# iris1997jiatong/I-DCCRN-VAE

Measured on AMD Instinct MI355X. Metric: 4s@16kHz utterances/sec fwd+SI-SNR, DCCRN-CL, 1/2/4/8 MI355X vs host CPU, higher is better.
Workload: dtype f32; 1 GPU; supervised DCCRN-CL forward(train=False) + final_ete_loss (weights 0/0/1); batch_per_gpu=64, utterance=4 s @ 16 kHz (64000 samples, 641 frames), parallelism=replicas x1, streams=1, input=resident in HBM

## Files before the change

i-dccrn-vae_amd/csrc/cgemm_tw.hip:

```cpp
#include <cstdint>
#include <cstdlib>
#include "cgemm.hpp"
#include "../../include/idccrn_hip.h"

namespace {

struct TwArgs {
    const float* x0;
    const float* x1;
    int C0, C1;
    int Fin, Fout;
    int J, Jp, Tp;
    const float* wfrag;
    int UP;
    const float* epi;
    int has_fold;
    const float* slope;
    float* out;
    int Cout, cotiles;
    int tshift, t_valid;
    double* stats;
    int stats_rep;
    const float* add;
    int add_div, add_Jp;
    int jtiles, ftiles;
    int xcd_split;
};

constexpr int TW_PACK_CI = 8;

template <int PH> __device__ __forceinline__ int tw_ra(int r) {
    if (PH == 0) return r == 0 ? 0 : (r == 2 ? 2 : 1);
    return r == 0 ? 1 : 2;
}
template <int PH> __device__ __forceinline__ int tw_rb(int r) {
    if (PH == 0) return r == 2 ? 1 : (r == 3 ? 3 : 2);
    return r == 0 ? 2 : 3;
}
template <int PH> __device__ __forceinline__ float tw_cb(int r) {
    if (PH == 0) return r == 1 ? 1.f : -1.f;
    return r == 1 ? 0.f : -1.f;
}
template <int PH> constexpr int tw_nr() { return PH == 0 ? 4 : 3; }
template <int PH> constexpr int tw_nt() { return tw_nr<PH>() * 9; }
template <int PH> constexpr int tw_ntp() { return PH == 0 ? 36 : 32; }
template <int PH> constexpr int tw_ntw() { return (tw_nt<PH>() + 3) / 4; }
__host__ __device__ inline int tw_tile(int ph, int w, int k) {
    if (ph == 0) return w * 9 + k;
    if (w < 3) return k < 6 ? w * 9 + k : w * 9 + 8;
    return k < 6 ? (k >> 1) * 9 + 6 + (k & 1) : -1;
}
template <int PH> constexpr int tw_wslots() { return PH == 0 ? 9 : 8; }

template <int PH, int CIK, bool LEFT, int DBG = 0, int RDW = 2, bool WVEC = true, bool STATS = false>
__global__ __launch_bounds__(256, 2) void cconv_tw_kernel(const TwArgs a) {
    constexpr int NR = tw_nr<PH>(), NT = tw_nt<PH>(), NTP = tw_ntp<PH>(), NTW = tw_ntw<PH>();
    constexpr int NRAW = PH == 0 ? 4 : 3, ROW0 = PH == 0 ? 0 : 1;
    constexpr int KS = CIK / 2;
    constexpr int RT = NRAW * 9 * 32;
    constexpr int NE = CIK * RT;
    constexpr int NBUF = 2;
    constexpr int NITEM = CIK * NRAW * 16;
    constexpr int NLD = (NITEM + 255) / 256;
    static_assert(KS % RDW == 0 && NLD <= 2, "weight ring slots are compile-time; at most two staging items per thread");
    static_assert(NT * 4 * 64 <= NBUF * NE, "the epilogue exchange fits the patch buffers");

    extern __shared__ __attribute__((aligned(16))) float smem[];

    const int tid = threadIdx.x;
    const int lane = tid & 63;
    const int wave = __builtin_amdgcn_readfirstlane(tid >> 6);
    const int half = lane >> 5, l31 = lane & 31;

    const int bid = blockIdx.x;
    const int xcd = bid & 7, slot = bid >> 3;
    int jt, ft, ct;
    if (a.xcd_split) {
        const int G = 8 / a.cotiles;
        ct = xcd % a.cotiles;
        jt = (slot / a.ftiles) * G + xcd / a.cotiles;
        ft = slot - (slot / a.ftiles) * a.ftiles;
    } else {
        const int per = a.cotiles * a.ftiles;
        jt = (slot / per) * 8 + xcd;
        const int rem = slot - (slot / per) * per;
        ft = rem / a.cotiles;
        ct = rem - ft * a.cotiles;
    }
    if (jt >= a.jtiles) return;
    const int j0 = jt * 64;
    const int m0 = 2 * ft;
    const int rbase = m0 - 1 + ROW0;

    const int Cin = a.C0 + a.C1;
    const int nchunk = (Cin + CIK - 1) / CIK;

    f32x16 acc[NTW];
#pragma unroll
    for (int k = 0; k < NTW; ++k)
#pragma unroll
        for (int r = 0; r < 16; ++r) acc[k][r] = 0.f;
    constexpr int NPAIR = (NTW - 1) / 2;
    constexpr bool UNI = PH == 0;
    int offA[UNI ? 1 : NPAIR + 1], offB[UNI ? 1 : NPAIR + 1];
    float cbj[UNI ? 1 : NPAIR + 1];
    if (UNI) {
        cbj[0] = tw_cb<PH>(wave);
        offA[0] = (tw_ra<PH>(wave) - ROW0) * 288;
        offB[0] = (tw_rb<PH>(wave) - ROW0) * 288;
    } else {
#pragma unroll
        for (int j = 0; j <= NPAIR; ++j) {
            int t = tw_tile(PH, wave, j < NPAIR ? 2 * j : NTW - 1);
            t = t < 0 ? 0 : t;
            const int r = t / 9, plane = t - r * 9;
            cbj[j] = tw_cb<PH>(r);
            const int po = plane == 8 ? 256 : (plane >> 1) * 64;
            offA[j] = (tw_ra<PH>(r) - ROW0) * 288 + po;
            offB[j] = cbj[j] != 0.f ? (tw_rb<PH>(r) - ROW0) * 288 + po : offA[j];
        }
    }

    f32x4 v_r[NLD], v_i[NLD];
    float e_r[NLD], e_i[NLD];
    unsigned off_v[NLD], off_e[NLD], ldsoff[NLD];
    unsigned okmask[NLD];
    int item_cl[NLD];
    bool interior[NLD];
#pragma unroll
    for (int i = 0; i < NLD; ++i) {
        const int e = tid + i * 256;
        const int c8 = e & 15;
        const int rl = (e >> 4) % NRAW, cl = e / (16 * NRAW);
        item_cl[i] = cl;
        const int f = rbase + rl;
        const int jc = j0 + 4 * c8;
        const int je = LEFT ? jc - 1 : jc + 4;
        const bool exists = e < NITEM;
        const bool okr = exists && f >= 0 && f < a.Fin;
        unsigned m = 0;
#pragma unroll
        for (int q = 0; q < 5; ++q) {
            const int c = jc + q + (LEFT ? -1 : 0);
            if (c >= 0 && c < a.J) m |= 1u << q;
        }
        if (okr) m |= 1u << 5;
        if (exists) m |= 1u << 7;
        const int jcv = jc + 3 < a.Jp ? jc : 0;
        const int jev = (je >= 0 && je < a.Jp) ? je : 0;
        off_v[i] = okr ? (unsigned)((cl * a.Fin + f) * a.Jp + jcv) : 0u;
        off_e[i] = okr ? (unsigned)((cl * a.Fin + f) * a.Jp + jev) : 0u;
        if (jc + 3 >= a.Jp) m &= ~0x1fu;
        if (!(je >= 0 && je < a.Jp)) m &= LEFT ? ~1u : ~(1u << 4);
        okmask[i] = m;
        interior[i] = __builtin_amdgcn_ballot_w64((m & 0xbfu) == 0xbfu) == ~0ull;
        ldsoff[i] = (unsigned)((cl * NRAW + rl) * 288 + 4 * c8);
    }
    auto stage_load = [&](int chunk, int i) {
        const int ci0 = chunk * CIK;
        const bool from0 = ci0 < a.C0;
        const float* br = from0 ? a.x0 + (size_t)ci0 * a.Fin * a.Jp : a.x1 + (size_t)(ci0 - a.C0) * a.Fin * a.Jp;
        const float* bi = from0 ? br + (size_t)a.C0 * a.Fin * a.Jp : br + (size_t)a.C1 * a.Fin * a.Jp;
        const int cvalid = (from0 ? a.C0 : Cin) - ci0;
        const bool dead = item_cl[i] >= cvalid;
        const unsigned ov = dead ? 0u : off_v[i], oe = dead ? 0u : off_e[i];
        v_r[i] = *(const f32x4*)(br + ov);
        v_i[i] = *(const f32x4*)(bi + ov);
        e_r[i] = br[oe];
        e_i[i] = bi[oe];
    };
    float fr[5], fi[5];
    auto stage_window = [&](int chunk, int i) {
        const int ci0s = chunk * CIK;
        const int cvalid = (ci0s < a.C0 ? a.C0 : Cin) - ci0s;
        constexpr bool left = LEFT;
        if (interior[i] && cvalid >= CIK) {
#pragma unroll
            for (int q = 0; q < 5; ++q) {
                fr[q] = left ? (q == 0 ? e_r[i] : v_r[i][q == 0 ? 0 : q - 1]) : (q == 4 ? e_r[i] : v_r[i][q == 4 ? 3 : q]);
                fi[q] = left ? (q == 0 ? e_i[i] : v_i[i][q == 0 ? 0 : q - 1]) : (q == 4 ? e_i[i] : v_i[i][q == 4 ? 3 : q]);
            }
            return;
        }
        unsigned m = okmask[i];
        if (item_cl[i] >= cvalid || !((m >> 5) & 1u)) m &= ~0x1fu;
#pragma unroll
        for (int q = 0; q < 5; ++q) {
            const float xr = left ? (q == 0 ? e_r[i] : v_r[i][q == 0 ? 0 : q - 1]) : (q == 4 ? e_r[i] : v_r[i][q == 4 ? 3 : q]);
            const float xi = left ? (q == 0 ? e_i[i] : v_i[i][q == 0 ? 0 : q - 1]) : (q == 4 ? e_i[i] : v_i[i][q == 4 ? 3 : q]);
            const bool cok = (m >> q) & 1u;
            fr[q] = cok ? xr : 0.f;
            fi[q] = cok ? xi : 0.f;
        }
    };
    auto plane_val = [&](int gt, int pr) -> float {
        const int g = gt / 3, tau = gt - g * 3;
        const int q0 = 2 * pr;
        const float xa_ = g == 0 ? fr[q0] + fi[q0] : (g == 1 ? fr[q0] : fi[q0]);
        const float xb_ = g == 0 ? fr[q0 + 1] + fi[q0 + 1] : (g == 1 ? fr[q0 + 1] : fi[q0 + 1]);
        const float xd_ = g == 0 ? fr[q0 + 2] + fi[q0 + 2] : (g == 1 ? fr[q0 + 2] : fi[q0 + 2]);
        return tau == 0 ? xa_ - xb_ : (tau == 1 ? xb_ : xb_ - xd_);
    };
    auto item_exists = [&](int i) -> bool { return NITEM >= (i + 1) * 256 || wave * 64 + i * 256 < NITEM; };
    auto stage_plane2 = [&](float* dst, int i, int j) {
        if (!item_exists(i)) return;
        if (j < 4) {
            f32x4 o = {plane_val(2 * j, 0), plane_val(2 * j + 1, 0), plane_val(2 * j, 1), plane_val(2 * j + 1, 1)};
            *(f32x4*)(dst + ldsoff[i] + j * 64) = o;
        } else {
            *(float2*)(dst + ldsoff[i] - 2 * (int)(tid & 15) + 256) = make_float2(plane_val(8, 0), plane_val(8, 1));
        }
    };
    auto stage_store = [&](float* dst, int chunk, int i) {
        stage_window(chunk, i);
#pragma unroll
        for (int j = 0; j < 5; ++j) stage_plane2(dst, i, j);
    };

    constexpr int WS = tw_wslots<PH>();
    const float* wbase = a.wfrag + ((size_t)(PH == 1 ? (size_t)a.cotiles * a.UP * tw_ntp<0>() : 0) + (size_t)ct * a.UP * NTP) * 64 +
                         (size_t)wave * WS * 64;
    const int total_ks = nchunk * KS;
    float a_w[RDW][NTW];
    auto load_w = [&](int g, float (&dst)[NTW]) {
        g = g < total_ks ? g : total_ks - 1;
        const float* ws = wbase + (size_t)g * NTP * 64;
        if (WVEC) {
            const f32x4 w0 = *(const f32x4*)(ws + lane * 4), w1 = *(const f32x4*)(ws + 256 + lane * 4);
#pragma unroll
            for (int k = 0; k < 4; ++k) {
                dst[k] = w0[k];
                if (4 + k < NTW) dst[4 + k] = w1[k];
            }
            if (NTW == 9) dst[NTW - 1] = ws[512 + lane];
        } else {
#pragma unroll
            for (int k = 0; k < NTW; ++k) dst[k] = ws[k * 64 + lane];
        }
    };
    float xa[NTW], xb[NTW];
    auto load_raw2 = [&](const float* base, int j) {
        if (j < NPAIR) {
            const int oa = UNI ? offA[0] + j * 64 : offA[UNI ? 0 : j], ob = UNI ? offB[0] + j * 64 : offB[UNI ? 0 : j];
            const float2 pa_ = *(const float2*)(base + oa + 2 * l31), pb_ = *(const float2*)(base + ob + 2 * l31);
            xa[2 * j] = pa_.x; xa[2 * j + 1] = pa_.y;
            xb[2 * j] = pb_.x; xb[2 * j + 1] = pb_.y;
        } else {
            xa[NTW - 1] = base[(UNI ? offA[0] + 256 : offA[UNI ? 0 : NPAIR]) + l31];
            xb[NTW - 1] = base[(UNI ? offB[0] + 256 : offB[UNI ? 0 : NPAIR]) + l31];
        }
    };
    auto load_raw_all = [&](const float* base) {
#pragma unroll
        for (int j = 0; j <= NPAIR; ++j) load_raw2(base, j);
    };

#pragma unroll
    for (int i = 0; i < NLD; ++i) stage_load(0, i);
#pragma unroll
    for (int u = 0; u < RDW; ++u) load_w(u, a_w[u]);
#pragma unroll
    for (int i = 0; i < NLD; ++i) stage_store(smem, 0, i);
#pragma unroll
    for (int i = 0; i < NLD; ++i) stage_load(nchunk > 1 ? 1 : 0, i);
    __syncthreads();

    load_raw_all(smem + (size_t)half * RT);
    for (int chunk = 0; chunk < nchunk; ++chunk) {
        const float* P = smem + (chunk & 1) * NE;
        float* Pn = smem + ((chunk + 1) & 1) * NE;
        const int nxt = chunk + 1 < nchunk ? chunk + 1 : chunk, nxt2 = chunk + 2 < nchunk ? chunk + 2 : nchunk - 1;
#pragma unroll
        for (int ul = 0; ul < KS; ++ul) {
            const float* bnext = ul + 1 < KS ? P + (size_t)(2 * (ul + 1) + half) * RT : Pn + (size_t)half * RT;
            const int si = ul - 1;
            const bool staging = !(DBG & 1) && si >= 0 && si < NLD;
#pragma unroll
            for (int k = 0; k < NTW; ++k) {
                const float b = xa[k] + cbj[UNI ? 0 : (k >> 1 < NPAIR ? k >> 1 : NPAIR)] * xb[k];
                acc[k] = __builtin_amdgcn_mfma_f32_32x32x2f32(a_w[ul % RDW][k], b, acc[k], 0, 0, 0);
                if (ul == KS - 1 && k == 0) {
                    __builtin_amdgcn_sched_barrier(0);
                    __syncthreads();
                }
                if ((k & 1) && (k >> 1) < NPAIR) load_raw2(bnext, k >> 1);
                if (k == NTW - 1) load_raw2(bnext, NPAIR);
                if (staging) {
                    if (k == 0) stage_window(nxt, si);
                    if ((k & 1) && k < 6) stage_plane2(Pn, si, k >> 1);
                    if (k == (NTW == 9 ? 7 : 6)) stage_plane2(Pn, si, 3);
                    if (k == NTW - 1) stage_plane2(Pn, si, 4);
                    if (k == NTW - 1) stage_load(nxt2, si);
                }
                __builtin_amdgcn_sched_barrier(0);
            }
            if (!(DBG & 2)) load_w(chunk * KS + ul + RDW, a_w[ul % RDW]);
        }
    }
    __syncthreads();

    const float slope = a.slope ? *a.slope : 1.0f;
    const bool has_act = a.slope != nullptr;
    float* E = smem;
    const int jA = j0 + 2 * l31;
    bool keep[2], inb[2];
    int ja[2];
#pragma unroll
    for (int q = 0; q < 2; ++q) {
        const int j = jA + q;
        const int bj = j / a.Tp, tp = j - bj * a.Tp;
        inb[q] = j < a.J;
        keep[q] = inb[q] && tp >= 1 && tp <= a.t_valid;
        ja[q] = j - (bj - bj / a.add_div) * a.Tp;
    }
#pragma unroll
    for (int s = 0; s < ((DBG & 4) ? 1 : 4); ++s) {
        if (s > 0) __syncthreads();
#pragma unroll
        for (int k = 0; k < NTW; ++k) {
            const int t = tw_tile(PH, wave, k);
            if (t >= 0) {
#pragma unroll
                for (int rr = 0; rr < 4; ++rr) E[(t * 4 + rr) * 64 + lane] = acc[k][4 * s + rr];
            }
        }
        __syncthreads();
        float v[NT];
#pragma unroll
        for (int t = 0; t < NT; ++t) v[t] = E[(t * 4 + wave) * 64 + lane];
        float pr[NR][2], pi[NR][2];
#pragma unroll
        for (int r = 0; r < NR; ++r) {
            float y[3][2];
#pragma unroll
            for (int g = 0; g < 3; ++g) {
                const float m1 = v[r * 9 + g * 3], m2 = v[r * 9 + g * 3 + 1], m3 = v[r * 9 + g * 3 + 2];
                y[g][0] = m1 + m2;
                y[g][1] = m2 - m3;
            }
#pragma unroll
            for (int q = 0; q < 2; ++q) {
                pr[r][q] = y[0][q] - y[2][q];
                pi[r][q] = y[0][q] + y[1][q];
            }
        }
        const int rg = 4 * s + wave;
        const int co = ct * 32 + (rg & 3) + 8 * (rg >> 2) + 4 * half;
        const bool cok = co < a.Cout;
        const f32x4 e0 = *(const f32x4*)(a.epi + (size_t)co * 8);
        const float e4 = a.epi[(size_t)co * 8 + 4], e5 = a.epi[(size_t)co * 8 + 5];
        float st[5] = {0.f, 0.f, 0.f, 0.f, 0.f};
#pragma unroll
        for (int rt = 0; rt < 2; ++rt) {
            const int fo = 2 * m0 + PH + 2 * rt;
            if (fo >= a.Fout) continue;
            float yr[2], yi[2];
#pragma unroll
            for (int q = 0; q < 2; ++q) {
                float re, im;
                if (PH == 0) {
                    re = rt == 0 ? pr[0][q] + pr[1][q] + pr[2][q] : pr[1][q] - pr[2][q] - pr[NR - 1][q];
                    im = rt == 0 ? pi[0][q] + pi[1][q] + pi[2][q] : pi[1][q] - pi[2][q] - pi[NR - 1][q];
                } else {
                    re = rt == 0 ? pr[0][q] + pr[1][q] : pr[1][q] - pr[2][q];
                    im = rt == 0 ? pi[0][q] + pi[1][q] : pi[1][q] - pi[2][q];
                }
                if (a.add && cok && inb[q]) {
                    re += a.add[((size_t)co * a.Fout + fo) * a.add_Jp + ja[q]];
                    im += a.add[((size_t)(a.Cout + co) * a.Fout + fo) * a.add_Jp + ja[q]];
                }
                float r_, i_;
                if (a.has_fold) {
                    r_ = e0[0] * re + e0[1] * im + e4;
                    i_ = e0[2] * re + e0[3] * im + e5;
                } else {
                    r_ = re + e4;
                    i_ = im + e5;
                }
                if (has_act) {
                    r_ = r_ >= 0.f ? r_ : slope * r_;
                    i_ = i_ >= 0.f ? i_ : slope * i_;
                }
                yr[q] = keep[q] ? r_ : 0.f;
                yi[q] = keep[q] ? i_ : 0.f;
                if (STATS && keep[q]) {
                    st[0] += yr[q];
                    st[1] += yi[q];
                    st[2] += yr[q] * yr[q];
                    st[3] += yi[q] * yi[q];
                    st[4] += yr[q] * yi[q];
                }
            }
            if (cok) {
                float* o_r = a.out + ((size_t)co * a.Fout + fo) * a.Jp + jA;
                float* o_i = a.out + ((size_t)(a.Cout + co) * a.Fout + fo) * a.Jp + jA;
                if (inb[1]) {
                    *(float2*)o_r = make_float2(yr[0], yr[1]);
                    *(float2*)o_i = make_float2(yi[0], yi[1]);
                } else if (inb[0]) {
                    o_r[0] = yr[0];
                    o_i[0] = yi[0];
                }
            }
        }
        if (STATS) {
#pragma unroll
            for (int q = 0; q < 5; ++q) {
                float tsum = st[q];
#pragma unroll
                for (int o = 16; o > 0; o >>= 1) tsum += __shfl_xor(tsum, o, 64);
                if (l31 == 0 && cok)
                    atomicAdd(&a.stats[((size_t)(a.stats_rep > 1 ? (blockIdx.x & (a.stats_rep - 1)) : 0) * a.Cout + co) * 5 + q], (double)tsum);
            }
        }
    }
}

__global__ void pack_cconv_tw_kernel(const float* __restrict__ wino, int cotiles, int UN, int UP, int vec, float* __restrict__ out) {
    const long long n0 = (long long)cotiles * UP * tw_ntp<0>() * 64, n1 = (long long)cotiles * UP * tw_ntp<1>() * 64;
    for (long long idx = blockIdx.x * (long long)blockDim.x + threadIdx.x; idx < n0 + n1; idx += (long long)gridDim.x * blockDim.x) {
        const int ph = idx >= n0;
        const long long i = ph ? idx - n0 : idx;
        const int ntp = ph ? tw_ntp<1>() : tw_ntp<0>(), nt = ph ? tw_nt<1>() : tw_nt<0>();
        const int lane = (int)(i & 63);
        long long t_ = i >> 6;
        const int t = (int)(t_ % ntp); t_ /= ntp;
        const int u = (int)(t_ % UP);
        const int ct = (int)(t_ / UP);
        float val = 0.f;
        const int ws_ = ph ? tw_wslots<1>() : tw_wslots<0>();
        const int pos = t * 64 + lane, w = pos / (ws_ * 64), q = pos % (ws_ * 64);
        const bool vec_ = (vec >> ph) & 1;
        const int k = !vec_ ? q >> 6 : (q < 512 ? (q >> 8) * 4 + (q & 3) : 8);
        const int ln = !vec_ ? q & 63 : (q < 512 ? (q & 255) >> 2 : q - 512);
        const int tt = k < (ph ? 7 : 9) ? tw_tile(ph, w, k) : -1;
        const int ci = 2 * u + (ln >> 5), co = ln & 31;
        if (tt >= 0 && ci * 3 < UN) {
            const int r = tt / 9, g = (tt % 9) / 3, tau = tt % 3;
            const float* src = wino + ((((size_t)ph * cotiles + ct) * UN + (size_t)ci * 3 + g) * 4 + r) * 64;
            const float w0 = src[co], w1 = src[32 + co];
            val = tau == 0 ? w0 : (tau == 1 ? w0 + w1 : w1);
        }
        out[idx] = val;
    }
}

template <int PH, int CIK, bool LEFT, int DBG, int RDW, bool WVEC = true, bool STATS = false>
int launch_tw_ph_l(const TwArgs& a, hipStream_t st);
inline int tw_wvec_mask() {
    static const int v = [] { const char* e = getenv("IDV_TW_WVEC"); return e ? atoi(e) : 1; }();
    return v;
}
template <int PH, int CIK, int DBG = 0, int RDW = 2>
int launch_tw_ph(const TwArgs& a, hipStream_t st) {
    const bool wv = (tw_wvec_mask() >> PH) & 1;
    if (DBG == 0 && RDW == 2 && a.stats) {
        constexpr bool WV = PH == 0;
        if (wv != WV) return IDV_EINVAL;
        return a.tshift ? launch_tw_ph_l<PH, CIK, true, 0, 2, WV, true>(a, st) : launch_tw_ph_l<PH, CIK, false, 0, 2, WV, true>(a, st);
    }
    if (DBG == 0 && RDW == 2 && !wv)
        return a.tshift ? launch_tw_ph_l<PH, CIK, true, 0, 2, false>(a, st) : launch_tw_ph_l<PH, CIK, false, 0, 2, false>(a, st);
    return a.tshift ? launch_tw_ph_l<PH, CIK, true, DBG, RDW>(a, st) : launch_tw_ph_l<PH, CIK, false, DBG, RDW>(a, st);
}
template <int PH, int CIK, bool LEFT, int DBG, int RDW, bool WVEC, bool STATS>
int launch_tw_ph_l(const TwArgs& a, hipStream_t st) {
    constexpr int NE = CIK * (PH == 0 ? 4 : 3) * 9 * 32;
    constexpr size_t smem = 2 * NE * sizeof(float);
    static_assert(smem * 2 <= 160 * 1024, "the patch buffers of two workgroups must fit the 160 KB of LDS");
    TwArgs b = a;
    b.jtiles = (a.J + 63) / 64;
    b.ftiles = PH == 1 ? a.Fin / 2 : (a.Fin + 1) / 2;
    if (b.ftiles == 0) return IDV_OK;
    static const int xsplit = [] { const char* e = getenv("IDV_TW_XCD_SPLIT"); return e ? atoi(e) : 1; }();
    b.xcd_split = (xsplit && (b.cotiles == 2 || b.cotiles == 4 || b.cotiles == 8)) ? 1 : 0;
    long long nblk = (long long)((b.jtiles + 7) / 8) * 8 * b.ftiles * b.cotiles;
    if (b.xcd_split) {
        const int G = 8 / b.cotiles;
        nblk = (long long)((b.jtiles + G - 1) / G) * b.ftiles * 8;
    }
    if (nblk > 0x7fffffffLL) return IDV_EINVAL;
    auto k = cconv_tw_kernel<PH, CIK, LEFT, DBG, RDW, WVEC, STATS>;
    static bool attr_set[64] = {};
    int dev = 0;
    if (hipGetDevice(&dev) != hipSuccess || dev < 0 || dev >= 64) return IDV_ELAUNCH;
    if (smem > 64 * 1024 && !attr_set[dev]) {
        if (hipFuncSetAttribute((const void*)k, hipFuncAttributeMaxDynamicSharedMemorySize, (int)smem) != hipSuccess) return IDV_ELAUNCH;
        attr_set[dev] = true;
    }
    hipLaunchKernelGGL(k, dim3((unsigned)nblk), dim3(256), smem, st, b);
    return idv_launch_status();
}

}

extern "C" int idv_cconv_tw_supported(int C0, int C1, int Cout, int Fin) {
    static const int min_cout = [] { const char* e = getenv("IDV_TW_MIN_COUT"); return e ? atoi(e) : 32; }();
    if (Cout < min_cout || Fin < 2) return 0;
    if (!idv_cconv_gauss_supported(C0, C1, Cout)) return 0;
    return (C1 == 0 || C0 % 8 == 0) ? 1 : 0;
}

extern "C" long long idv_cconv_tw_wfrag_floats(int Cout, int cin_used) {
    const long long cotiles = (Cout + 31) / 32, cpad = (cin_used + TW_PACK_CI - 1) / TW_PACK_CI * TW_PACK_CI;
    return cotiles * (cpad / 2) * (36 + 32) * 64;
}

extern "C" int idv_pack_cconv_tw(const float* wino_frag, int Cout, int cin_used, float* tw_frag, void* stream) {
    if (!wino_frag || !tw_frag || Cout <= 0 || cin_used <= 0) return IDV_EINVAL;
    const int cotiles = (Cout + 31) / 32;
    const int cpad = (cin_used + TW_PACK_CI - 1) / TW_PACK_CI * TW_PACK_CI;
    const long long n = idv_cconv_tw_wfrag_floats(Cout, cin_used);
    const unsigned blocks = (unsigned)((n + 255) / 256 > 4096 ? 4096 : (n + 255) / 256);
    hipLaunchKernelGGL(pack_cconv_tw_kernel, dim3(blocks), dim3(256), 0, (hipStream_t)stream, wino_frag, cotiles, cpad * 3, cpad / 2,
                       tw_wvec_mask(), tw_frag);
    return idv_launch_status();
}

extern "C" int idv_ctconv2d_tw_fwd(const float* x0, int C0, const float* x1, int C1, const float* wfrag, const float* epi, int has_fold,
                                   const float* prelu_slope, float* out, double* stats, double* stats_work, int stats_rep, int tshift,
                                   int Cout, int Fin, int B, int Tp, int Jp, int t_valid_out, const float* addend, int addend_div,
                                   int addend_Jp, void* stream) {
    if (!x0 || !wfrag || !epi || !out || C0 <= 0 || Cout <= 0 || Fin <= 0 || B <= 0 || Tp <= 1) return IDV_EINVAL;
    if (stats && stats_work && (stats_rep < 2 || (stats_rep & (stats_rep - 1)))) return IDV_EINVAL;
    if (addend && (addend_div < 1 || B % addend_div || addend_Jp < (B / addend_div) * Tp)) return IDV_EINVAL;
    if (C1 > 0 && !x1) return IDV_EINVAL;
    if (tshift != 0 && tshift != -1) return IDV_EINVAL;
    if (!idv_cconv_tw_supported(C0, C1, Cout, Fin)) return IDV_EINVAL;
    if ((Jp & 3) || (reinterpret_cast<uintptr_t>(x0) & 15) || (C1 > 0 && (reinterpret_cast<uintptr_t>(x1) & 15)) ||
        (reinterpret_cast<uintptr_t>(out) & 7))
        return IDV_EINVAL;
    TwArgs a{};
    a.x0 = x0; a.x1 = x1; a.C0 = C0; a.C1 = C1;
    a.Fin = Fin; a.Fout = 2 * Fin - 1;
    a.J = B * Tp; a.Jp = Jp; a.Tp = Tp;
    a.wfrag = wfrag; a.UP = (C0 + C1 + TW_PACK_CI - 1) / TW_PACK_CI * TW_PACK_CI / 2;
    a.epi = epi; a.has_fold = has_fold; a.slope = prelu_slope; a.out = out;
    a.Cout = Cout; a.cotiles = (Cout + 31) / 32;
    a.tshift = tshift; a.t_valid = t_valid_out;
    a.add = addend; a.add_div = addend ? addend_div : 1; a.add_Jp = addend_Jp;
    if (Jp < a.J) return IDV_EINVAL;
    if ((long long)8 * Fin * (long long)Jp >= 0xffffffffLL) return IDV_EINVAL;
    hipStream_t st = (hipStream_t)stream;
    a.stats = stats;
    if (stats && stats_work) { a.stats = stats_work; a.stats_rep = stats_rep; }
    int rc = 0;
#ifdef IDV_TW_EXPERIMENTS
    static const int dbg = [] { const char* e = getenv("IDV_TW_DBG"); return e ? atoi(e) : 0; }();
    static const int only = [] { const char* e = getenv("IDV_TW_ONLY"); return e ? atoi(e) : 0; }();
    if (dbg && !stats) {
        if (only != 2) rc = dbg == 1 ? launch_tw_ph<0, 8, 1>(a, st) : (dbg == 2 ? launch_tw_ph<0, 8, 2>(a, st) : launch_tw_ph<0, 8, 3>(a, st));
        if (rc) return rc;
        if (only != 1) rc = dbg == 1 ? launch_tw_ph<1, 8, 1>(a, st) : (dbg == 2 ? launch_tw_ph<1, 8, 2>(a, st) : launch_tw_ph<1, 8, 3>(a, st));
        return rc;
    }
    if (only) return only == 1 ? launch_tw_ph<0, 8>(a, st) : launch_tw_ph<1, 8>(a, st);
#endif
    rc = launch_tw_ph<0, 8>(a, st);
    if (!rc) rc = launch_tw_ph<1, 8>(a, st);
    if (rc || !(stats && stats_work)) return rc;
    return idv_launch_stats_collapse(stats_work, stats_rep, Cout * 5, stats, st);
}
```

i-dccrn-vae_amd/csrc/cgemm_tw2.hip:

```cpp
#include <cstdint>
#include <cstdlib>
#include <type_traits>
#include "cgemm.hpp"
#include "../../include/idccrn_hip.h"

namespace {

struct Tw2Args {
    const float* x0;
    int Cin;
    int Fin, Fout;
    int J, Jp, Tp;
    const float* wfrag;
    int UP;
    const float* epi;
    int has_fold;
    const float* slope;
    float* out;
    int Cout, cotiles;
    int tshift, t_valid;
    double* stats;
    int stats_rep;
    int jtiles, ftiles;
    int xcd_split;
};

constexpr int TW2_PACK_CI = 8;

__host__ __device__ constexpr int tw2_ra(int q) { return q == 0 ? 0 : (q == 1 ? 2 : (q == 2 ? 4 : (q == 3 ? 2 : (q == 4 ? 1 : 3)))); }
__host__ __device__ constexpr int tw2_rb(int q) { return q == 0 ? 4 : (q == 1 ? 4 : (q == 2 ? 2 : (q == 3 ? 6 : (q == 4 ? 3 : (q == 5 ? 3 : 5))))); }
__host__ __device__ constexpr float tw2_cb(int q) { return q == 1 ? 1.f : (q == 5 ? 0.f : -1.f); }
__host__ __device__ constexpr int tw2_qx(int a) { return a == 0 ? 0 : (a == 1 ? 1 : 3); }
__host__ __device__ constexpr int tw2_qy(int a) { return a == 0 ? 4 : (a == 1 ? 5 : 6); }
__host__ __device__ constexpr int tw2_main_acc(int w) { return w == 2 ? 3 : w; }
__host__ __device__ inline void tw2_slot(int w, int k, int& q, int& plane) {
    if (w < 3) {
        if (k < 14) { q = (k & 1) ? tw2_qy(tw2_main_acc(w)) : tw2_qx(tw2_main_acc(w)); plane = k >> 1; }
        else { q = 2; plane = 2 * w + (k - 14); }
    } else {
        if (k < 12) { const int a = tw2_main_acc(k >> 2); q = (k & 1) ? tw2_qy(a) : tw2_qx(a); plane = 7 + ((k >> 1) & 1); }
        else if (k < 15) { q = 2; plane = 6 + (k - 12); }
        else { q = -1; plane = 0; }
    }
}
__host__ __device__ inline int tw2_acc_tile(int w, int i) {
    if (w < 3) return i < 7 ? tw2_main_acc(w) * 9 + i : 2 * 9 + 2 * w + (i - 7);
    return i < 6 ? tw2_main_acc(i >> 1) * 9 + 7 + (i & 1) : 2 * 9 + 6 + (i - 6);
}

__device__ __forceinline__ int tw2_poff(int p, int l31) { return p < 8 ? (p >> 1) * 64 + 2 * l31 + (p & 1) : 256 + l31; }

template <bool LEFT, bool STATS, int DBG = 0>
__global__ __launch_bounds__(256, 2) void cconv_tw2_kernel(const Tw2Args a) {
    constexpr int NT = 36, NACC = 9, NSLOT = 16;
    constexpr int NRAW = 7, CIK = 4, KS = 2;
    constexpr int RT = NRAW * 288;
    constexpr int NE = CIK * RT;
    constexpr int NITEM = CIK * NRAW * 16;
    constexpr int NLD = 2;
    static_assert(NT * 4 * 64 <= 2 * NE, "the epilogue exchange fits the patch buffers");

    extern __shared__ __attribute__((aligned(16))) float smem[];

    const int tid = threadIdx.x;
    const int lane = tid & 63;
    const int wave = __builtin_amdgcn_readfirstlane(tid >> 6);
    const int half = lane >> 5, l31 = lane & 31;

    const int bid = blockIdx.x;
    const int xcd = bid & 7, slot = bid >> 3;
    int jt, ft, ct;
    if (a.xcd_split) {
        const int G = 8 / a.cotiles;
        ct = xcd % a.cotiles;
        jt = (slot / a.ftiles) * G + xcd / a.cotiles;
        ft = slot - (slot / a.ftiles) * a.ftiles;
    } else {
        const int per = a.cotiles * a.ftiles;
        jt = (slot / per) * 8 + xcd;
        const int rem = slot - (slot / per) * per;
        ft = rem / a.cotiles;
        ct = rem - ft * a.cotiles;
    }
    if (jt >= a.jtiles) return;
    const int j0 = jt * 64;
    const int m0 = 2 * ft;
    const int rbase = 2 * m0 - 2;

    const int Cin = a.Cin;
    const int nchunk = (Cin + CIK - 1) / CIK;

    f32x16 acc[NACC];
#pragma unroll
    for (int k = 0; k < NACC; ++k)
#pragma unroll
        for (int r = 0; r < 16; ++r) acc[k][r] = 0.f;

    f32x4 v_r[NLD], v_i[NLD];
    float e_r[NLD], e_i[NLD];
    unsigned off_v[NLD], ldsoff[NLD];
    unsigned okmask[NLD];
    bool interior[NLD];
    auto item_cl = [&](int i) -> int { return (tid + i * 256) / (16 * NRAW); };
#pragma unroll
    for (int i = 0; i < NLD; ++i) {
        const int e = tid + i * 256;
        const int c8 = e & 15;
        const int rl = (e >> 4) % NRAW, cl = e / (16 * NRAW);
        const int f = rbase + rl;
        const int jc = j0 + 4 * c8;
        const int je = LEFT ? jc - 1 : jc + 4;
        const bool exists = e < NITEM;
        const bool okr = exists && f >= 0 && f < a.Fin;
        unsigned m = 0;
#pragma unroll
        for (int q = 0; q < 5; ++q) {
            const int c = jc + q + (LEFT ? -1 : 0);
            if (c >= 0 && c < a.J) m |= 1u << q;
        }
        if (okr) m |= 1u << 5;
        const int jcv = jc + 3 < a.Jp ? jc : 0;
        off_v[i] = okr ? (unsigned)((cl * a.Fin + f) * a.Jp + jcv) : 4u;
        if (jc + 3 >= a.Jp) m &= ~0x1fu;
        if (!(je >= 0 && je < a.Jp)) m &= LEFT ? ~1u : ~(1u << 4);
        okmask[i] = m;
        interior[i] = __builtin_amdgcn_ballot_w64((m & 0x3fu) == 0x3fu) == ~0ull;
        ldsoff[i] = (unsigned)((cl * NRAW + rl) * 288 + 4 * c8);
    }
    auto item_exists = [&](int i) -> bool { return i == 0 || wave * 64 + 256 < NITEM; };
    auto stage_load = [&](int chunk, int i) {
        if (!item_exists(i)) return;
        const int ci0 = chunk * CIK;
        const float* br = a.x0 + (size_t)ci0 * a.Fin * a.Jp;
        const float* bi = br + (size_t)Cin * a.Fin * a.Jp;
        const bool dead = item_cl(i) >= Cin - ci0;
        const unsigned ov = dead ? 4u : off_v[i];
        v_r[i] = *(const f32x4*)(br + ov);
        v_i[i] = *(const f32x4*)(bi + ov);
        e_r[i] = (br + ov)[LEFT ? -1 : 4];
        e_i[i] = (bi + ov)[LEFT ? -1 : 4];
    };
    float fr[5], fi[5];
    auto stage_window = [&](int chunk, int i) {
        if (!item_exists(i)) return;
        const int cvalid = Cin - chunk * CIK;
        constexpr bool left = LEFT;
        if (interior[i] && cvalid >= CIK) {
#pragma unroll
            for (int q = 0; q < 5; ++q) {
                fr[q] = left ? (q == 0 ? e_r[i] : v_r[i][q == 0 ? 0 : q - 1]) : (q == 4 ? e_r[i] : v_r[i][q == 4 ? 3 : q]);
                fi[q] = left ? (q == 0 ? e_i[i] : v_i[i][q == 0 ? 0 : q - 1]) : (q == 4 ? e_i[i] : v_i[i][q == 4 ? 3 : q]);
            }
            return;
        }
        unsigned m = okmask[i];
        if (item_cl(i) >= cvalid || !((m >> 5) & 1u)) m &= ~0x1fu;
#pragma unroll
        for (int q = 0; q < 5; ++q) {
            const float xr = left ? (q == 0 ? e_r[i] : v_r[i][q == 0 ? 0 : q - 1]) : (q == 4 ? e_r[i] : v_r[i][q == 4 ? 3 : q]);
            const float xi = left ? (q == 0 ? e_i[i] : v_i[i][q == 0 ? 0 : q - 1]) : (q == 4 ? e_i[i] : v_i[i][q == 4 ? 3 : q]);
            const bool cok = (m >> q) & 1u;
            fr[q] = cok ? xr : 0.f;
            fi[q] = cok ? xi : 0.f;
        }
    };
    auto plane_val = [&](int gt, int pr) -> float {
        const int g = gt / 3, tau = gt - g * 3;
        const int q0 = 2 * pr;
        const float xa_ = g == 0 ? fr[q0] + fi[q0] : (g == 1 ? fr[q0] : fi[q0]);
        const float xb_ = g == 0 ? fr[q0 + 1] + fi[q0 + 1] : (g == 1 ? fr[q0 + 1] : fi[q0 + 1]);
        const float xd_ = g == 0 ? fr[q0 + 2] + fi[q0 + 2] : (g == 1 ? fr[q0 + 2] : fi[q0 + 2]);
        return tau == 0 ? xa_ - xb_ : (tau == 1 ? xb_ : xb_ - xd_);
    };
    auto stage_plane2 = [&](float* dst, int i, int j) {
        if (!item_exists(i)) return;
        if (j < 4) {
            f32x4 o = {plane_val(2 * j, 0), plane_val(2 * j + 1, 0), plane_val(2 * j, 1), plane_val(2 * j + 1, 1)};
            *(f32x4*)(dst + ldsoff[i] + j * 64) = o;
        } else {
            *(float2*)(dst + ldsoff[i] - 2 * (int)(tid & 15) + 256) = make_float2(plane_val(8, 0), plane_val(8, 1));
        }
    };
    auto stage_store = [&](float* dst, int chunk, int i) {
        stage_window(chunk, i);
#pragma unroll
        for (int j = 0; j < 5; ++j) stage_plane2(dst, i, j);
    };

    const float* wbase = a.wfrag + (((size_t)ct * a.UP) * 4 + wave) * 1024 + lane * 4;
    const int total_ks = nchunk * KS;
    float a_w[NSLOT];
    auto load_wg = [&](int g, int grp) {
        g = g < total_ks ? g : total_ks - 1;
        const f32x4 w4 = *(const f32x4*)(wbase + (size_t)g * 4096 + grp * 256);
#pragma unroll
        for (int k = 0; k < 4; ++k) a_w[grp * 4 + k] = w4[k];
    };

    const int am = tw2_main_acc(wave < 3 ? wave : 0);
    const int qxm = tw2_qx(am), qym = tw2_qy(am);
    const int rxa = tw2_ra(qxm) * 288, rxb = tw2_rb(qxm) * 288, rya = tw2_ra(qym) * 288, ryb = tw2_rb(qym) * 288;
    const float cbx = tw2_cb(qxm), cby = tw2_cb(qym);
    const int r2a = tw2_ra(2) * 288 + wave * 64, r2b = tw2_rb(2) * 288 + wave * 64;
    float xa[2][4], xb[2][4];
    auto load_grp_a = [&](const float* base, int g, float (&oa)[4], float (&ob)[4]) {
        if (g < 3) {
            const float2 xa_ = *(const float2*)(base + rxa + g * 64 + 2 * l31), xb_ = *(const float2*)(base + rxb + g * 64 + 2 * l31);
            const float2 ya_ = *(const float2*)(base + rya + g * 64 + 2 * l31), yb_ = *(const float2*)(base + ryb + g * 64 + 2 * l31);
            oa[0] = xa_.x; oa[2] = xa_.y; ob[0] = xb_.x; ob[2] = xb_.y;
            oa[1] = ya_.x; oa[3] = ya_.y; ob[1] = yb_.x; ob[3] = yb_.y;
        } else {
            oa[0] = base[rxa + 3 * 64 + 2 * l31]; ob[0] = base[rxb + 3 * 64 + 2 * l31];
            oa[1] = base[rya + 3 * 64 + 2 * l31]; ob[1] = base[ryb + 3 * 64 + 2 * l31];
            const float2 pa_ = *(const float2*)(base + r2a + 2 * l31), pb_ = *(const float2*)(base + r2b + 2 * l31);
            oa[2] = pa_.x; oa[3] = pa_.y; ob[2] = pb_.x; ob[3] = pb_.y;
        }
    };
    auto load_grp_b = [&](const float* base, int g, float (&oa)[4], float (&ob)[4]) {
#pragma unroll
        for (int s4 = 0; s4 < 4; ++s4) {
            int q, plane;
            tw2_slot(3, 4 * g + s4, q, plane);
            if (q < 0) continue;
            oa[s4] = base[tw2_ra(q) * 288 + tw2_poff(plane, l31)];
            ob[s4] = base[tw2_rb(q) * 288 + tw2_poff(plane, l31)];
        }
    };

#pragma unroll
    for (int i = 0; i < NLD; ++i) stage_load(0, i);
#pragma unroll
    for (int grp = 0; grp < 4; ++grp) load_wg(0, grp);
#pragma unroll
    for (int i = 0; i < NLD; ++i) stage_store(smem, 0, i);
#pragma unroll
    for (int i = 0; i < NLD; ++i) stage_load(nchunk > 1 ? 1 : 0, i);
    __syncthreads();
    if (wave < 3)
        load_grp_a(smem + (size_t)half * RT, 0, xa[0], xb[0]);
    else
        load_grp_b(smem + (size_t)half * RT, 0, xa[0], xb[0]);

    auto run = [&](auto role) {
        constexpr bool ROLE_B = decltype(role)::value;
        for (int chunk = 0; chunk < nchunk; ++chunk) {
            const float* P = smem + (chunk & 1) * NE;
            float* Pn = smem + ((chunk + 1) & 1) * NE;
            const int nxt = chunk + 1 < nchunk ? chunk + 1 : chunk, nxt2 = chunk + 2 < nchunk ? chunk + 2 : nchunk - 1;
#pragma unroll
            for (int ul = 0; ul < KS; ++ul) {
                const float* bnext = ul + 1 < KS ? P + (size_t)(2 * (ul + 1) + half) * RT : Pn + (size_t)half * RT;
                const bool staging = !(DBG & 1) && ul == 0;
#pragma unroll
                for (int k = 0; k < (ROLE_B ? NSLOT - 1 : NSLOT); ++k) {
                    const int g = k >> 2, s4 = k & 3;
                    float cb;
                    int ai;
                    if (ROLE_B) {
                        int q, plane;
                        tw2_slot(3, k, q, plane);
                        cb = tw2_cb(q);
                        ai = k < 12 ? k >> 1 : 6 + (k - 12);
                    } else {
                        cb = k < 14 ? ((k & 1) ? cby : cbx) : -1.f;
                        ai = k < 14 ? k >> 1 : 7 + (k - 14);
                    }
                    if (s4 == 0) {
                        const float* src = g < 3 ? P + (size_t)(2 * ul + half) * RT : bnext;
                        if (!(ul == KS - 1 && g == 3)) {
                            if (ROLE_B) load_grp_b(src, (g + 1) & 3, xa[(g + 1) & 1], xb[(g + 1) & 1]);
                            else load_grp_a(src, (g + 1) & 3, xa[(g + 1) & 1], xb[(g + 1) & 1]);
                        }
                    }
                    const float b = xa[g & 1][s4] + cb * xb[g & 1][s4];
                    acc[ai] = __builtin_amdgcn_mfma_f32_32x32x2f32(a_w[k], b, acc[ai], 0, 0, 0);
                    if (ul == KS - 1 && k == 0) {
                        __builtin_amdgcn_sched_barrier(0);
                        __syncthreads();
                    }
                    if (ul == KS - 1 && k == 12) {
                        if (ROLE_B) load_grp_b(bnext, 0, xa[0], xb[0]);
                        else load_grp_a(bnext, 0, xa[0], xb[0]);
                    }
                    if (((k & 3) == 3 || (ROLE_B && k == NSLOT - 2)) && !(DBG & 2)) load_wg(chunk * KS + ul + 1, k >> 2);
                    if (staging) {
                        if (k == 0) stage_window(nxt, 0);
                        if (k >= 1 && k <= 5) stage_plane2(Pn, 0, k - 1);
                        if (k == 5) stage_load(nxt2, 0);
                        if (!ROLE_B) {
                            if (k == 8) stage_window(nxt, 1);
                            if (k >= 9 && k <= 13) stage_plane2(Pn, 1, k - 9);
                            if (k == 13) stage_load(nxt2, 1);
                        }
                    }
                    __builtin_amdgcn_sched_barrier(0);
                }
            }
        }
    };
    if (wave < 3)
        run(std::false_type{});
    else
        run(std::true_type{});
    __syncthreads();

    const float slope = a.slope ? *a.slope : 1.0f;
    const bool has_act = a.slope != nullptr;
    float* E = smem;
    const int jA = j0 + 2 * l31;
    bool keep[2], inb[2];
#pragma unroll
    for (int q = 0; q < 2; ++q) {
        const int j = jA + q;
        const int tp = j % a.Tp;
        inb[q] = j < a.J;
        keep[q] = inb[q] && tp >= 1 && tp <= a.t_valid;
    }
#pragma unroll
    for (int s = 0; s < 4; ++s) {
        if (s > 0) __syncthreads();
#pragma unroll
        for (int k = 0; k < NACC; ++k) {
            const int t = tw2_acc_tile(wave, k);
#pragma unroll
            for (int rr = 0; rr < 4; ++rr) E[(t * 4 + rr) * 64 + lane] = acc[k][4 * s + rr];
        }
        __syncthreads();
        float v[NT];
#pragma unroll
        for (int t = 0; t < NT; ++t) v[t] = E[(t * 4 + wave) * 64 + lane];
        float pr[4][2], pi[4][2];
#pragma unroll
        for (int r = 0; r < 4; ++r) {
            float y[3][2];
#pragma unroll
            for (int g = 0; g < 3; ++g) {
                const float m1 = v[r * 9 + g * 3], m2 = v[r * 9 + g * 3 + 1], m3 = v[r * 9 + g * 3 + 2];
                y[g][0] = m1 + m2;
                y[g][1] = m2 - m3;
            }
#pragma unroll
            for (int q = 0; q < 2; ++q) {
                pr[r][q] = y[0][q] - y[2][q];
                pi[r][q] = y[0][q] + y[1][q];
            }
        }
        const int rg = 4 * s + wave;
        const int co = ct * 32 + (rg & 3) + 8 * (rg >> 2) + 4 * half;
        const bool cok = co < a.Cout;
        const f32x4 e0 = *(const f32x4*)(a.epi + (size_t)co * 8);
        const float e4 = a.epi[(size_t)co * 8 + 4], e5 = a.epi[(size_t)co * 8 + 5];
        float st[5] = {0.f, 0.f, 0.f, 0.f, 0.f};
#pragma unroll
        for (int rt = 0; rt < 2; ++rt) {
            const int fo = m0 + rt;
            if (fo >= a.Fout) continue;
            float yr[2], yi[2];
#pragma unroll
            for (int q = 0; q < 2; ++q) {
                const float re = rt == 0 ? pr[0][q] + pr[1][q] + pr[2][q] : pr[1][q] - pr[2][q] - pr[3][q];
                const float im = rt == 0 ? pi[0][q] + pi[1][q] + pi[2][q] : pi[1][q] - pi[2][q] - pi[3][q];
                float r_, i_;
                if (a.has_fold) {
                    r_ = e0[0] * re + e0[1] * im + e4;
                    i_ = e0[2] * re + e0[3] * im + e5;
                } else {
                    r_ = re + e4;
                    i_ = im + e5;
                }
                if (has_act) {
                    r_ = r_ >= 0.f ? r_ : slope * r_;
                    i_ = i_ >= 0.f ? i_ : slope * i_;
                }
                yr[q] = keep[q] ? r_ : 0.f;
                yi[q] = keep[q] ? i_ : 0.f;
                if (STATS && keep[q]) {
                    st[0] += yr[q];
                    st[1] += yi[q];
                    st[2] += yr[q] * yr[q];
                    st[3] += yi[q] * yi[q];
                    st[4] += yr[q] * yi[q];
                }
            }
            if (cok) {
                float* o_r = a.out + ((size_t)co * a.Fout + fo) * a.Jp + jA;
                float* o_i = a.out + ((size_t)(a.Cout + co) * a.Fout + fo) * a.Jp + jA;
                if (inb[1]) {
                    *(float2*)o_r = make_float2(yr[0], yr[1]);
                    *(float2*)o_i = make_float2(yi[0], yi[1]);
                } else if (inb[0]) {
                    o_r[0] = yr[0];
                    o_i[0] = yi[0];
                }
            }
        }
        if (STATS) {
#pragma unroll
            for (int q = 0; q < 5; ++q) {
                float tsum = st[q];
#pragma unroll
                for (int o = 16; o > 0; o >>= 1) tsum += __shfl_xor(tsum, o, 64);
                if (l31 == 0 && cok)
                    atomicAdd(&a.stats[((size_t)(a.stats_rep > 1 ? (blockIdx.x & (a.stats_rep - 1)) : 0) * a.Cout + co) * 5 + q], (double)tsum);
            }
        }
    }
}

__global__ void pack_cconv_tw2_kernel(const float* __restrict__ wino, int cotiles, int UN, int UP, float* __restrict__ out) {
    const long long n = (long long)cotiles * UP * 4096;
    for (long long idx = blockIdx.x * (long long)blockDim.x + threadIdx.x; idx < n; idx += (long long)gridDim.x * blockDim.x) {
        const int kk = (int)(idx & 3), ln = (int)((idx >> 2) & 63), grp = (int)((idx >> 8) & 3), w = (int)((idx >> 10) & 3);
        const long long t_ = idx >> 12;
        const int u = (int)(t_ % UP), ct = (int)(t_ / UP);
        int q, plane;
        tw2_slot(w, grp * 4 + kk, q, plane);
        float val = 0.f;
        const int ci = 2 * u + (ln >> 5), co = ln & 31;
        if (q >= 0 && ci * 3 < UN) {
            const int g = plane / 3, tau = plane % 3;
            const float* src = wino + ((((size_t)ct * UN + (size_t)ci * 3 + g) * 8 + q)) * 64;
            const float w0 = src[co], w1 = src[32 + co];
            val = tau == 0 ? w0 : (tau == 1 ? w0 + w1 : w1);
        }
        out[idx] = val;
    }
}

template <bool LEFT, bool STATS, int DBG>
int launch_tw2(const Tw2Args& a, hipStream_t st) {
    constexpr size_t smem = 2 * 4 * 7 * 288 * sizeof(float);
    static_assert(smem * 2 <= 160 * 1024, "the patch buffers of two workgroups must fit the 160 KB of LDS");
    Tw2Args b = a;
    b.jtiles = (a.J + 63) / 64;
    b.ftiles = (a.Fout + 1) / 2;
    static const int xsplit = [] { const char* e = getenv("IDV_TW_XCD_SPLIT"); return e ? atoi(e) : 1; }();
    b.xcd_split = (xsplit && (b.cotiles == 2 || b.cotiles == 4 || b.cotiles == 8)) ? 1 : 0;
    long long nblk = (long long)((b.jtiles + 7) / 8) * 8 * b.ftiles * b.cotiles;
    if (b.xcd_split) {
        const int G = 8 / b.cotiles;
        nblk = (long long)((b.jtiles + G - 1) / G) * b.ftiles * 8;
    }
    if (nblk > 0x7fffffffLL) return IDV_EINVAL;
    auto k = cconv_tw2_kernel<LEFT, STATS, DBG>;
    static bool attr_set[64] = {};
    int dev = 0;
    if (hipGetDevice(&dev) != hipSuccess || dev < 0 || dev >= 64) return IDV_ELAUNCH;
    if (smem > 64 * 1024 && !attr_set[dev]) {
        if (hipFuncSetAttribute((const void*)k, hipFuncAttributeMaxDynamicSharedMemorySize, (int)smem) != hipSuccess) return IDV_ELAUNCH;
        attr_set[dev] = true;
    }
    hipLaunchKernelGGL(k, dim3((unsigned)nblk), dim3(256), smem, st, b);
    return idv_launch_status();
}

}

extern "C" int idv_cconv_tw2_supported(int Cin, int Cout, int Fin) {
    static const int min_cout = [] { const char* e = getenv("IDV_TW2_MIN_COUT"); return e ? atoi(e) : 32; }();
    static const int min_cin = [] { const char* e = getenv("IDV_TW2_MIN_CIN"); return e ? atoi(e) : 64; }();
    if (Cout < min_cout || Cin < min_cin || (Fin - 1) / 2 + 1 < 2) return 0;
    return idv_cconv_gauss_supported(Cin, 0, Cout);
}

extern "C" long long idv_cconv_tw2_wfrag_floats(int Cout, int cin_used) {
    const long long cotiles = (Cout + 31) / 32, cpad = (cin_used + TW2_PACK_CI - 1) / TW2_PACK_CI * TW2_PACK_CI;
    return cotiles * (cpad / 2) * 4096;
}

extern "C" int idv_pack_cconv_tw2(const float* wino_frag, int Cout, int cin_used, float* tw_frag, void* stream) {
    if (!wino_frag || !tw_frag || Cout <= 0 || cin_used <= 0) return IDV_EINVAL;
    const int cotiles = (Cout + 31) / 32;
    const int cpad = (cin_used + TW2_PACK_CI - 1) / TW2_PACK_CI * TW2_PACK_CI;
    const long long n = idv_cconv_tw2_wfrag_floats(Cout, cin_used);
    const unsigned blocks = (unsigned)((n + 255) / 256 > 4096 ? 4096 : (n + 255) / 256);
    hipLaunchKernelGGL(pack_cconv_tw2_kernel, dim3(blocks), dim3(256), 0, (hipStream_t)stream, wino_frag, cotiles, cpad * 3, cpad / 2,
                       tw_frag);
    return idv_launch_status();
}

extern "C" int idv_cconv2d_tw_fwd(const float* x0, int Cin, const float* wfrag, const float* epi, int has_fold, const float* prelu_slope,
                                  float* out, double* stats, double* stats_work, int stats_rep, int tshift, int Cout, int Fin, int B, int Tp,
                                  int Jp, int t_valid_out, void* stream) {
    if (!x0 || !wfrag || !epi || !out || Cin <= 0 || Cout <= 0 || Fin <= 0 || B <= 0 || Tp <= 1) return IDV_EINVAL;
    if (stats && stats_work && (stats_rep < 2 || (stats_rep & (stats_rep - 1)))) return IDV_EINVAL;
    if (tshift != 0 && tshift != -1) return IDV_EINVAL;
    if (!idv_cconv_tw2_supported(Cin, Cout, Fin)) return IDV_EINVAL;
    if ((Jp & 3) || (reinterpret_cast<uintptr_t>(x0) & 15) || (reinterpret_cast<uintptr_t>(out) & 7)) return IDV_EINVAL;
    Tw2Args a{};
    a.x0 = x0; a.Cin = Cin;
    a.Fin = Fin; a.Fout = (Fin - 1) / 2 + 1;
    a.J = B * Tp; a.Jp = Jp; a.Tp = Tp;
    a.wfrag = wfrag; a.UP = (Cin + TW2_PACK_CI - 1) / TW2_PACK_CI * TW2_PACK_CI / 2;
    a.epi = epi; a.has_fold = has_fold; a.slope = prelu_slope; a.out = out;
    a.Cout = Cout; a.cotiles = (Cout + 31) / 32;
    a.tshift = tshift; a.t_valid = t_valid_out;
    if (Jp < a.J) return IDV_EINVAL;
    if ((long long)4 * Fin * (long long)Jp >= 0xffffffffLL) return IDV_EINVAL;
    hipStream_t st = (hipStream_t)stream;
    a.stats = stats;
    if (stats && stats_work) { a.stats = stats_work; a.stats_rep = stats_rep; }
    int rc;
#ifdef IDV_TW_EXPERIMENTS
    static const int dbg = [] { const char* e = getenv("IDV_TW_DBG"); return e ? atoi(e) : 0; }();
    if (!stats && dbg == 1) return tshift ? launch_tw2<true, false, 1>(a, st) : launch_tw2<false, false, 1>(a, st);
    if (!stats && dbg == 2) return tshift ? launch_tw2<true, false, 2>(a, st) : launch_tw2<false, false, 2>(a, st);
    if (!stats && dbg == 3) return tshift ? launch_tw2<true, false, 3>(a, st) : launch_tw2<false, false, 3>(a, st);
#endif
    if (stats)
        rc = tshift ? launch_tw2<true, true, 0>(a, st) : launch_tw2<false, true, 0>(a, st);
    else
        rc = tshift ? launch_tw2<true, false, 0>(a, st) : launch_tw2<false, false, 0>(a, st);
    if (rc || !(stats && stats_work)) return rc;
    return idv_launch_stats_collapse(stats_work, stats_rep, Cout * 5, stats, st);
}
```

i-dccrn-vae_amd/csrc/cgemm_wino.hip:

```cpp
#include <cstdlib>
#include "cgemm.hpp"
#include "../../include/idccrn_hip.h"

namespace {

struct WinoArgs {
    const float* x0;
    const float* x1;
    int C0, C1;
    int Fin, Fout;
    int J, Jp, Tp;
    const float* wfrag;
    int UN;
    const float* epi;
    int has_fold;
    const float* slope;
    float* out;
    int Cout, cotiles;
    int tshift, t_valid;
    double* stats;
    int stats_rep;
    const float* add;
    int add_div, add_Jp;
    int jtiles, ftiles, mblocks;
    int xcd_split;
};

constexpr int WCIK = 8;
template <int PH> __device__ __forceinline__ int wino_ra(int tq) {
    if (PH == 0) return tq == 0 ? 0 : (tq == 2 ? 2 : 1);
    if (PH == 1) return tq == 0 ? 1 : 2;
    return tq == 0 ? 0 : (tq == 1 ? 2 : (tq == 2 ? 4 : (tq == 3 ? 2 : (tq == 4 ? 1 : 3))));
}
template <int PH> __device__ __forceinline__ int wino_rb(int tq) {
    if (PH == 0) return tq == 2 ? 1 : (tq == 3 ? 3 : 2);
    if (PH == 1) return tq == 0 ? 2 : 3;
    return tq == 0 ? 4 : (tq == 1 ? 4 : (tq == 2 ? 2 : (tq == 3 ? 6 : (tq == 4 ? 3 : 5))));
}
template <int PH> __device__ __forceinline__ float wino_cb(int tq) {
    if (PH == 0) return tq == 1 ? 1.f : -1.f;
    if (PH == 1) return tq == 1 ? 0.f : -1.f;
    return tq == 1 ? 1.f : (tq == 5 ? 0.f : -1.f);
}
template <int PH> constexpr int wino_tr() { return PH == 0 ? 4 : (PH == 1 ? 3 : 7); }
template <int PH> constexpr int wino_nacc() { return PH == 1 ? 3 : 4; }
template <int PH> constexpr int wino_slots() { return PH == 2 ? 8 : 4; }
constexpr int wino_acc2(int q) { return q < 4 ? q : (q == 4 ? 0 : (q == 5 ? 1 : 3)); }

template <int PH, int WM, int WN, int CIK, int NBUF, bool STATS, int OCC = 1, int RDP = 0>
__global__ __launch_bounds__(WM* WN * 64, OCC) void cconv_wino_kernel(const WinoArgs a) {
    constexpr int NT = WM * WN * 64;
    constexpr int TR = wino_tr<PH>();
    constexpr int NP = TR, NACC = wino_nacc<PH>(), SL = wino_slots<PH>();
    constexpr int JT = 32 * WN;
    constexpr int PS = JT + 8;
    constexpr int COL0 = 4;
    constexpr int PS4 = PS / 4;
    constexpr int NS = CIK * TR * PS4;
    constexpr int NLD = (NS + NT - 1) / NT;
    constexpr int NE = CIK * 3 * TR * PS;
    constexpr int UNITS = CIK * 3;
    static_assert(NLD <= 8, "staging registers");

    extern __shared__ __attribute__((aligned(16))) float smem[];

    const int tid = threadIdx.x;
    const int lane = tid & 63;
    const int wave = __builtin_amdgcn_readfirstlane(tid >> 6);
    const int wm = wave / WN, wn = wave % WN;

    const int MB = a.mblocks, FTn = a.ftiles;
    const int bid = blockIdx.x;
    int jt, ft, mblk;
    if (a.xcd_split) {
        const int xcd = bid & 7, slot = bid >> 3;
        const int G = 8 / MB;
        mblk = xcd % MB;
        jt = (slot / FTn) * G + xcd / MB;
        ft = slot - (slot / FTn) * FTn;
    } else {
        const int per = 8 * MB * FTn;
        const int sg = bid / per, rem = bid - sg * per;
        const int v = rem >> 3;
        jt = sg * 8 + (rem & 7);
        ft = v / MB;
        mblk = v - (v / MB) * MB;
    }
    if (jt >= a.jtiles) return;
    const int j0 = jt * JT;
    const int ct = mblk * WM + wm;
    const bool ct_ok = ct < a.cotiles;
    const int m0 = 2 * ft;
    const int rbase = PH == 2 ? 2 * m0 - 2 : m0 - 1;
    const bool half_tile = PH != 1 && m0 + 1 >= (PH == 2 ? a.Fout : a.Fin);

    const int Cin = a.C0 + a.C1;
    const int nchunk = (Cin + CIK - 1) / CIK;

    f32x16 acc[NACC][3];
#pragma unroll
    for (int w = 0; w < NACC; ++w)
#pragma unroll
        for (int p3 = 0; p3 < 3; ++p3)
#pragma unroll
            for (int r = 0; r < 16; ++r) acc[w][p3][r] = 0.f;

    f32x4 sar[NLD], sai[NLD], sbr[NLD], sbi[NLD];
    unsigned voffa[NLD], voffb[NLD];
    unsigned long long okbits = 0;
    unsigned ldsoff[NLD];
    float cbv[NLD];
#pragma unroll
    for (int i = 0; i < NLD; ++i) {
        const int e = tid + i * NT;
        const int row = e / PS4, c4 = e - row * PS4;
        const int cil = row / TR, tq = row - cil * TR;
        const int fa = rbase + wino_ra<PH>(tq), fb = rbase + wino_rb<PH>(tq);
        const int jv = j0 - 4 + 4 * c4;
        const bool oka = (e < NS) && fa >= 0 && fa < a.Fin;
        const bool okb = (e < NS) && wino_cb<PH>(tq) != 0.f && fb >= 0 && fb < a.Fin;
        unsigned ba = 0, bb = 0;
#pragma unroll
        for (int q = 0; q < 4; ++q) {
            const bool cok = jv + q >= 0 && jv + q < a.J;
            if (oka && cok) ba |= 1u << q;
            if (okb && cok) bb |= 1u << q;
        }
        okbits |= (unsigned long long)(ba | (bb << 4)) << (8 * i);
        voffa[i] = ba ? (unsigned)((cil * a.Fin + fa) * a.Jp + jv) : 0u;
        voffb[i] = bb ? (unsigned)((cil * a.Fin + fb) * a.Jp + jv) : 0u;
        cbv[i] = wino_cb<PH>(tq);
        ldsoff[i] = (unsigned)(((cil * 3) * TR + tq) * PS + 4 * c4);
    }
    auto stage_load = [&](int chunk) {
        const int ci0 = chunk * CIK;
        const bool from0 = ci0 < a.C0;
        const float* br = from0 ? a.x0 + (size_t)ci0 * a.Fin * a.Jp : a.x1 + (size_t)(ci0 - a.C0) * a.Fin * a.Jp;
        const float* bi = from0 ? br + (size_t)a.C0 * a.Fin * a.Jp : br + (size_t)a.C1 * a.Fin * a.Jp;
        const int cvalid = (from0 ? a.C0 : Cin) - ci0;
#pragma unroll
        for (int i = 0; i < NLD; ++i) {
            const bool dead = (tid + i * NT) / (TR * PS4) >= cvalid;
            const unsigned oa = dead ? 0u : voffa[i], ob = dead ? 0u : voffb[i];
            sar[i] = *(const f32x4*)(br + oa);
            sai[i] = *(const f32x4*)(bi + oa);
            sbr[i] = *(const f32x4*)(br + ob);
            sbi[i] = *(const f32x4*)(bi + ob);
        }
    };
    auto stage_store = [&](float* dst, int chunk) {
        const int ci0s = chunk * CIK;
        const int cvalid = (ci0s < a.C0 ? a.C0 : Cin) - ci0s;
#pragma unroll
        for (int i = 0; i < NLD; ++i) asm volatile("" ::"v"(sar[i]), "v"(sai[i]), "v"(sbr[i]), "v"(sbi[i]));
#pragma unroll
        for (int i = 0; i < NLD; ++i) {
            const int e = tid + i * NT;
            unsigned bits = (unsigned)(okbits >> (8 * i)) & 255u;
            if (e / (TR * PS4) >= cvalid) bits = 0u;
            f32x4 vr, vi, vs;
#pragma unroll
            for (int q = 0; q < 4; ++q) {
                const float ar = (bits >> q) & 1u ? sar[i][q] : 0.f, ai = (bits >> q) & 1u ? sai[i][q] : 0.f;
                const float br_ = (bits >> (4 + q)) & 1u ? sbr[i][q] : 0.f, bi_ = (bits >> (4 + q)) & 1u ? sbi[i][q] : 0.f;
                vr[q] = ar + cbv[i] * br_;
                vi[q] = ai + cbv[i] * bi_;
                vs[q] = vr[q] + vi[q];
            }
            if (e < NS) {
                float* d = dst + ldsoff[i];
                *(f32x4*)d = vs;
                *(f32x4*)(d + TR * PS) = vr;
                *(f32x4*)(d + 2 * TR * PS) = vi;
            }
        }
    };

    constexpr int RD = RDP ? RDP : UNITS;
    static_assert(UNITS % RD == 0, "ring slots are compile-time");
    const float* wbase = a.wfrag + (((size_t)(PH == 1 ? a.cotiles : 0) + (ct_ok ? ct : 0)) * a.UN) * SL * 64 + lane;
    const int total_units = nchunk * UNITS;
    float a_w[RD][NP];

    const int bcol = wn * 32 + (lane & 31) + (lane >> 5) + COL0 + a.tshift;
    auto load_b = [&](const float* P, int u, float (&dst)[TR]) {
#pragma unroll
        for (int tq = 0; tq < TR; ++tq) dst[tq] = P[(u * TR + tq) * PS + bcol];
    };

    stage_load(0);
#pragma unroll
    for (int u = 0; u < RD; ++u)
#pragma unroll
        for (int q = 0; q < NP; ++q) a_w[u][q] = wbase[(size_t)(u * SL + q) * 64];
    stage_store(smem, 0);
#pragma unroll
    for (int u = 0; u < RD; ++u)
#pragma unroll
        for (int q = 0; q < NP; ++q) asm volatile("" : "+v"(a_w[u][q]));
    __syncthreads();

    constexpr int UMID = UNITS / 2;
    float b_cur[TR], b_nxt[TR];
    int ibuf = 0;
    if (NBUF == 3) load_b(smem, 0, b_cur);
    for (int chunk = 0; chunk < nchunk; ++chunk) {
        const float* P = smem + ibuf * NE;
        const int inext = (ibuf + 1 == NBUF) ? 0 : ibuf + 1;
        float* Pn = smem + inext * NE;
        const int nxt = (chunk + 1 < nchunk) ? chunk + 1 : chunk;
        if (NBUF == 2) load_b(P, 0, b_cur);
#pragma unroll
        for (int u = 0; u < UNITS; ++u) {
            const int p3 = u % 3;
            acc[0][p3] = __builtin_amdgcn_mfma_f32_32x32x2f32(a_w[u % RD][0], b_cur[0], acc[0][p3], 0, 0, 0);
            __builtin_amdgcn_sched_barrier(0);
            if (NBUF == 3 && u == UNITS - 1) __syncthreads();
            if (u + 1 < UNITS)
                load_b(P, u + 1, b_nxt);
            else if (NBUF == 3)
                load_b(Pn, 0, b_nxt);
            __builtin_amdgcn_sched_barrier(0);
            if (u == 0) stage_load(nxt);
            if (u == (NBUF == 3 ? UMID : UNITS - 1)) stage_store(Pn, nxt);
#pragma unroll
            for (int q = 1; q < NP; ++q) {
                constexpr int dummy = 0;
                (void)dummy;
                const int ai = PH == 2 ? wino_acc2(q) : q;
                if (ai == 3 && half_tile) continue;
                acc[ai][p3] = __builtin_amdgcn_mfma_f32_32x32x2f32(a_w[u % RD][q], b_cur[q], acc[ai][p3], 0, 0, 0);
            }
            __builtin_amdgcn_sched_barrier(0);
            {
                int gl = chunk * UNITS + u - 1 + RD;
                gl = gl < total_units ? gl : total_units - 1;
                const float* ws = wbase + (size_t)gl * SL * 64;
#pragma unroll
                for (int q = 0; q < NP; ++q) a_w[(u + RD - 1) % RD][q] = ws[q * 64];
            }
            if (u + 1 < UNITS || NBUF == 3) {
#pragma unroll
                for (int tq = 0; tq < TR; ++tq) b_cur[tq] = b_nxt[tq];
            }
        }
        if (NBUF == 2) __syncthreads();
        ibuf = inext;
    }

    if (!ct_ok) return;
    const float slope = a.slope ? *a.slope : 1.0f;
    const bool has_act = a.slope != nullptr;
    const int half = lane >> 5, l31 = lane & 31;
    const int j = j0 + wn * 32 + l31;
    const int bj = j / a.Tp, tp = j - bj * a.Tp;
    const bool keep = (tp >= 1) && (tp <= a.t_valid);
    const bool inb = j < a.J;
    const int ja = j - (bj - bj / a.add_div) * a.Tp;
#pragma unroll
    for (int r = 0; r < 16; ++r) {
        const int co = ct * 32 + (r & 3) + 8 * (r >> 2) + 4 * half;
        const f32x4 e0 = *(const f32x4*)(a.epi + (size_t)co * 8);
        const float e4 = a.epi[(size_t)co * 8 + 4], e5 = a.epi[(size_t)co * 8 + 5];
        const bool cok = co < a.Cout;
        float st[5] = {0.f, 0.f, 0.f, 0.f, 0.f};
        float t[2][3];
#pragma unroll
        for (int p3 = 0; p3 < 3; ++p3) {
            if (PH != 1) {
                const float M1 = acc[0][p3][r], M2 = acc[1][p3][r], M3 = acc[2][p3][r], M4 = acc[NACC - 1][p3][r];
                t[0][p3] = M1 + M2 + M3;
                t[1][p3] = M2 - M3 - M4;
            } else {
                const float N1 = acc[0][p3][r], N2 = acc[1][p3][r], N3 = acc[2][p3][r];
                t[0][p3] = N1 + N2;
                t[1][p3] = N2 - N3;
            }
        }
#pragma unroll
        for (int rt = 0; rt < 2; ++rt) {
            const int fo = PH == 2 ? m0 + rt : 2 * m0 + PH + 2 * rt;
            if (fo >= a.Fout) continue;
            float re = t[rt][0] - t[rt][2], im = t[rt][0] + t[rt][1];
            if (a.add && cok && inb) {
                re += a.add[((size_t)co * a.Fout + fo) * a.add_Jp + ja];
                im += a.add[((size_t)(a.Cout + co) * a.Fout + fo) * a.add_Jp + ja];
            }
            float yr, yi;
            if (a.has_fold) {
                yr = e0[0] * re + e0[1] * im + e4;
                yi = e0[2] * re + e0[3] * im + e5;
            } else {
                yr = re + e4;
                yi = im + e5;
            }
            if (has_act) {
                yr = yr >= 0.f ? yr : slope * yr;
                yi = yi >= 0.f ? yi : slope * yi;
            }
            yr = keep ? yr : 0.f;
            yi = keep ? yi : 0.f;
            if (cok && inb) {
                a.out[((size_t)co * a.Fout + fo) * a.Jp + j] = yr;
                a.out[((size_t)(a.Cout + co) * a.Fout + fo) * a.Jp + j] = yi;
            }
            if (STATS && inb && keep) {
                st[0] += yr;
                st[1] += yi;
                st[2] += yr * yr;
                st[3] += yi * yi;
                st[4] += yr * yi;
            }
        }
        if (STATS) {
#pragma unroll
            for (int q = 0; q < 5; ++q) {
                float tsum = st[q];
#pragma unroll
                for (int o = 16; o > 0; o >>= 1) tsum += __shfl_xor(tsum, o, 64);
                if (l31 == 0 && cok)
                    atomicAdd(&a.stats[((size_t)(a.stats_rep > 1 ? (blockIdx.x & (a.stats_rep - 1)) : 0) * a.Cout + co) * 5 + q], (double)tsum);
            }
        }
    }
}

__global__ void pack_cconv_wino_kernel(const float* __restrict__ w_re, const float* __restrict__ w_im, int Cout, int Cin_total,
                                       int Cin_used, int transposed, int conj, int UN, int cotiles, float* __restrict__ wfrag) {
    const long long n = 2LL * cotiles * UN * 64;
    for (long long idx = blockIdx.x * (long long)blockDim.x + threadIdx.x; idx < n; idx += (long long)gridDim.x * blockDim.x) {
        const int lane = (int)(idx & 63);
        long long t = idx >> 6;
        int unit, ct, hf;
        if (transposed) {
            unit = (int)(t % UN); t /= UN;
            ct = (int)(t % cotiles);
            hf = (int)(t / cotiles);
        } else {
            hf = (int)(t & 1); t >>= 1;
            unit = (int)(t % UN);
            ct = (int)(t / UN);
        }
        const int h = lane >> 5, co = ct * 32 + (lane & 31);
        const int ci = unit / 3, p3 = unit % 3;
        float W[5] = {0.f, 0.f, 0.f, 0.f, 0.f};
        if (co < Cout && ci < Cin_used) {
            const int kt = transposed ? 1 - h : h;
#pragma unroll
            for (int kf = 0; kf < 5; ++kf) {
                const size_t off = transposed ? (((size_t)ci * Cout + co) * 5 + kf) * 2 + kt
                                              : (((size_t)co * Cin_total + ci) * 5 + kf) * 2 + kt;
                const float wr = w_re[off], wi = conj ? -w_im[off] : w_im[off];
                W[kf] = p3 == 0 ? wr : (p3 == 1 ? wi - wr : wr + wi);
            }
        }
        float o[4];
        if (transposed) {
            if (hf == 0) {
                o[0] = W[4]; o[1] = 0.5f * (W[4] + W[2] + W[0]); o[2] = 0.5f * (W[4] - W[2] + W[0]); o[3] = W[0];
            } else {
                o[0] = W[3]; o[1] = W[3] + W[1]; o[2] = W[1]; o[3] = 0.f;
            }
        } else {
            if (hf == 0) {
                o[0] = W[0]; o[1] = 0.5f * (W[0] + W[2] + W[4]); o[2] = 0.5f * (W[0] - W[2] + W[4]); o[3] = W[4];
            } else {
                o[0] = W[1]; o[1] = W[1] + W[3]; o[2] = W[3]; o[3] = 0.f;
            }
        }
        float* dst = wfrag + ((idx >> 6) * 4) * 64 + lane;
#pragma unroll
        for (int q = 0; q < 4; ++q) dst[q * 64] = o[q];
    }
}

template <int PH, int WM, int WN, int CIK, bool STATS, int OCC = 1, int RD = 0>
int launch_wino_ph(const WinoArgs& a, hipStream_t st) {
    static_assert(WCIK % CIK == 0, "a K chunk never straddles the pack granularity (nor, with it, the two sources)");
    constexpr int TR = wino_tr<PH>();
    constexpr int JT = 32 * WN;
    constexpr int NE = CIK * 3 * TR * (JT + 8);
    constexpr int NBUF = (3 * NE * sizeof(float) * OCC <= 156 * 1024) ? 3 : 2;
    constexpr size_t smem = NBUF * NE * sizeof(float);
    static_assert(smem * OCC <= 160 * 1024, "the patch buffers of OCC workgroups must fit the 160 KB of LDS");
    WinoArgs b = a;
    b.jtiles = (a.J + JT - 1) / JT;
    b.ftiles = PH == 2 ? (a.Fout + 1) / 2 : (PH == 1 ? a.Fin / 2 : (a.Fin + 1) / 2);
    b.mblocks = (a.cotiles + WM - 1) / WM;
    if (b.ftiles == 0) return IDV_OK;
    static const int xsplit = [] { const char* e = getenv("IDV_WINO_XCD_SPLIT"); return e ? atoi(e) : 1; }();
    b.xcd_split = (xsplit && (b.mblocks == 2 || b.mblocks == 4 || b.mblocks == 8)) ? 1 : 0;
    long long nblk = (long long)((b.jtiles + 7) / 8) * 8 * b.ftiles * b.mblocks;
    if (b.xcd_split) {
        const int G = 8 / b.mblocks;
        nblk = (long long)((b.jtiles + G - 1) / G) * b.ftiles * 8;
    }
    if (nblk > 0x7fffffffLL) return IDV_EINVAL;
    auto k = cconv_wino_kernel<PH, WM, WN, CIK, NBUF, STATS, OCC, RD>;
    const size_t smem_req = OCC == 1 ? (smem > 84 * 1024 ? smem : 84 * 1024) : smem;
    if (smem_req > 64 * 1024 &&
        hipFuncSetAttribute((const void*)k, hipFuncAttributeMaxDynamicSharedMemorySize, (int)smem_req) != hipSuccess) return IDV_ELAUNCH;
    hipLaunchKernelGGL(k, dim3((unsigned)nblk), dim3(WM * WN * 64), smem_req, st, b);
    return idv_launch_status();
}

template <int WM, int WN, int CIK, bool STATS>
int launch_wino_s(const WinoArgs& a, int transposed, hipStream_t st) {
    if (!transposed) {
        if constexpr (CIK == 2) return launch_wino_ph<2, WM, WN, 2, STATS, 2, 3>(a, st);
        else return launch_wino_ph<2, WM, WN, CIK, STATS, 1, (CIK * 3) / 2>(a, st);
    }
    if constexpr (CIK == 2) return IDV_EINVAL;
    else {
    static const int ph1 = [] { const char* e = getenv("IDV_WINO_PH1"); return e ? atoi(e) : 1; }();
    static const int ph0 = [] { const char* e = getenv("IDV_WINO_PH0"); return e ? atoi(e) : 2; }();
    if (ph0 == 2 && WM == 4 && WN == 1) {
        if (int rc = launch_wino_ph<0, 4, 1, 4, STATS, 2, 4>(a, st)) return rc;
    } else if (ph0 == 2 && WM == 2 && WN == 2) {
        if (int rc = launch_wino_ph<0, 2, 2, 2, STATS, 2, 3>(a, st)) return rc;
    } else if (ph0 == 2 && WM == 1 && WN == 4) {
        if (int rc = launch_wino_ph<0, 1, 4, 2, STATS, 2, 3>(a, st)) return rc;
    } else if (int rc = launch_wino_ph<0, WM, WN, CIK, STATS>(a, st)) return rc;
    if (ph1 == 0) return launch_wino_ph<1, WM, WN, CIK, STATS>(a, st);
    return launch_wino_ph<1, WM, WN, CIK, STATS, 2, (CIK * 3) % 8 == 0 ? 8 : 6>(a, st);
    }
}
template <int WM, int WN, int CIK>
int launch_wino(const WinoArgs& a, int transposed, hipStream_t st) {
    return a.stats ? launch_wino_s<WM, WN, CIK, true>(a, transposed, st) : launch_wino_s<WM, WN, CIK, false>(a, transposed, st);
}

const bool USE_WINO = [] { const char* e = getenv("IDV_WINO"); return !e || e[0] != '0'; }();
const bool USE_WINO_CONV = [] { const char* e = getenv("IDV_WINO_CONV"); return !e || e[0] != '0'; }();

}

extern "C" int idv_cconv_wino_supported(int transposed, int C0, int C1, int Cout, int Fin) {
    static const int min_cout = [] { const char* e = getenv("IDV_WINO_MIN_COUT"); return e ? atoi(e) : 33; }();
    static const int conv_min = [] { const char* e = getenv("IDV_WINO_CONV_MINC"); return e ? atoi(e) : 32; }();
    if (!USE_WINO || (!transposed && !USE_WINO_CONV) || Cout < min_cout) return 0;
    static const int conv_mincout = [] { const char* e = getenv("IDV_WINO_CONV_MINCOUT"); return e ? atoi(e) : 64; }();
    if (transposed ? Fin < 2 : ((Fin - 1) / 2 + 1 < 2 || Cout < conv_mincout || C0 + C1 < conv_min)) return 0;
    return idv_cconv_gauss_supported(C0, C1, Cout);
}

extern "C" long long idv_cconv_wino_wfrag_floats(int transposed, int Cout, int cin_used) {
    (void)transposed;
    const long long cotiles = (Cout + 31) / 32, cpad = (cin_used + WCIK - 1) / WCIK * WCIK;
    return cotiles * cpad * 3 * 8 * 64;
}

extern "C" int idv_cconv_wino_config(int transposed, int Cin, int Cout) {
    (void)Cin;
    if (!transposed) return Cout >= 128 ? 412 : 222;
    return Cout >= 128 ? 418 : (Cout > 32 ? 228 : 144);
}

extern "C" int idv_pack_cconv_wino(const float* w_re, const float* w_im, int Cout, int Cin_total, int Cin_used, int transposed,
                                   int conj, float* wfrag, void* stream) {
    if (!w_re || !w_im || !wfrag || Cout <= 0 || Cin_used <= 0 || Cin_used > Cin_total) return IDV_EINVAL;
    const int cotiles = (Cout + 31) / 32;
    const int UN = (Cin_used + WCIK - 1) / WCIK * WCIK * 3;
    const long long n = 2LL * cotiles * UN * 64;
    const unsigned blocks = (unsigned)((n + 255) / 256 > 4096 ? 4096 : (n + 255) / 256);
    hipLaunchKernelGGL(pack_cconv_wino_kernel, dim3(blocks), dim3(256), 0, (hipStream_t)stream, w_re, w_im, Cout, Cin_total, Cin_used,
                       transposed, conj, UN, cotiles, wfrag);
    return idv_launch_status();
}

extern "C" int idv_cconv2d_wino_fwd(const float* x0, int C0, const float* x1, int C1, const float* wfrag, const float* epi, int has_fold,
                                    const float* prelu_slope, float* out, double* stats, double* stats_work, int stats_rep,
                                    int transposed, int tshift, int Cout, int Fin, int B, int Tp, int Jp, int t_valid_out,
                                    const float* addend, int addend_div, int addend_Jp, void* stream) {
    if (!x0 || !wfrag || !epi || !out || C0 <= 0 || Cout <= 0 || Fin <= 0 || B <= 0 || Tp <= 1) return IDV_EINVAL;
    if (stats && stats_work && (stats_rep < 2 || (stats_rep & (stats_rep - 1)))) return IDV_EINVAL;
    if (addend && (addend_div < 1 || B % addend_div || addend_Jp < (B / addend_div) * Tp)) return IDV_EINVAL;
    if (C1 > 0 && !x1) return IDV_EINVAL;
    if (tshift != 0 && tshift != -1) return IDV_EINVAL;
    if (!idv_cconv_wino_supported(transposed, C0, C1, Cout, Fin)) return IDV_EINVAL;
    if ((Jp & 3) || (reinterpret_cast<uintptr_t>(x0) & 15) || (C1 > 0 && (reinterpret_cast<uintptr_t>(x1) & 15))) return IDV_EINVAL;
    WinoArgs a{};
    a.x0 = x0; a.x1 = x1; a.C0 = C0; a.C1 = C1;
    a.Fin = Fin; a.Fout = transposed ? 2 * Fin - 1 : (Fin - 1) / 2 + 1;
    a.J = B * Tp; a.Jp = Jp; a.Tp = Tp;
    a.wfrag = wfrag; a.UN = (C0 + C1 + WCIK - 1) / WCIK * WCIK * 3; a.epi = epi; a.has_fold = has_fold; a.slope = prelu_slope; a.out = out;
    a.Cout = Cout; a.cotiles = (Cout + 31) / 32;
    a.tshift = tshift; a.t_valid = t_valid_out;
    a.add = addend; a.add_div = addend ? addend_div : 1; a.add_Jp = addend_Jp;
    if (Jp < a.J) return IDV_EINVAL;
    if ((long long)WCIK * Fin * (long long)Jp >= 0xffffffffLL) return IDV_EINVAL;
    hipStream_t st = (hipStream_t)stream;
    a.stats = stats;
    if (stats && stats_work) { a.stats = stats_work; a.stats_rep = stats_rep; }
    int rc;
    static const int xcfg = [] { const char* e = getenv("IDV_WINO_CFG"); return e ? atoi(e) : 0; }();
    static const int xccfg = [] { const char* e = getenv("IDV_WINO_CCFG"); return e ? atoi(e) : 0; }();
    int cfg = transposed ? xcfg : xccfg;
    if (!cfg) cfg = idv_cconv_wino_config(transposed, C0 + C1, Cout);
    if (C1 > 0 && C0 % (cfg % 10)) cfg = cfg / 10 * 10 + 4;
    if (transposed && cfg % 10 == 2) return IDV_EINVAL;
    switch (cfg) {
        case 412: rc = launch_wino<4, 1, 2>(a, transposed, st); break;
        case 414: rc = launch_wino<4, 1, 4>(a, transposed, st); break;
        case 418: rc = launch_wino<4, 1, 8>(a, transposed, st); break;
        case 222: rc = launch_wino<2, 2, 2>(a, transposed, st); break;
        case 224: rc = launch_wino<2, 2, 4>(a, transposed, st); break;
        case 228: rc = launch_wino<2, 2, 8>(a, transposed, st); break;
        case 144: rc = launch_wino<1, 4, 4>(a, transposed, st); break;
        default: return IDV_EINVAL;
    }
    if (rc || !(stats && stats_work)) return rc;
    return idv_launch_stats_collapse(stats_work, stats_rep, Cout * 5, stats, st);
}
```

i-dccrn-vae_amd/csrc/common.hpp:

```cpp
#pragma once
#include <hip/hip_runtime.h>
#include <stdint.h>

#define IDV_SLACK 256

typedef float f32x16 __attribute__((ext_vector_type(16)));
typedef float f32x4 __attribute__((ext_vector_type(4)));

#define IDV_OK 0
#define IDV_EINVAL (-1)
#define IDV_ELAUNCH (-2)

static inline int idv_launch_status() {
    hipError_t e = hipGetLastError();
    return e == hipSuccess ? IDV_OK : IDV_ELAUNCH;
}

__device__ __forceinline__ float wave_sum(float v) {
#pragma unroll
    for (int o = 32; o > 0; o >>= 1) v += __shfl_xor(v, o, 64);
    return v;
}
__device__ __forceinline__ double wave_sum_d(double v) {
#pragma unroll
    for (int o = 32; o > 0; o >>= 1) v += __shfl_xor(v, o, 64);
    return v;
}

__device__ __forceinline__ float sigmoidf_(float x) {
    return __builtin_amdgcn_rcpf(1.0f + __builtin_amdgcn_exp2f(-1.44269504088896341f * x));
}
__device__ __forceinline__ float tanhf_(float x) {
    return 2.0f * __builtin_amdgcn_rcpf(1.0f + __builtin_amdgcn_exp2f(-2.88539008177792681f * x)) - 1.0f;
}

int idv_launch_stats_collapse(const double* work, int rep, int n, double* stats, hipStream_t st);
```

i-dccrn-vae_amd/ops.py:

```python
from __future__ import annotations

import os
from typing import Optional, Sequence

import torch

from . import _lib as L
from ._lib import call, p, i, f, d, ll, stream_ptr

SLACK = 256

PRECISION = os.environ.get("IDV_PRECISION", "fp32")


def set_precision(mode: str):
    global PRECISION
    if mode not in ("fp32", "bf16x3"):
        raise ValueError("precision must be 'fp32' or 'bf16x3'")
    PRECISION = mode


def bucket(n: int) -> int:
    if n <= 4096:
        return n
    step = 1 << (n.bit_length() - 4)
    return (n + step - 1) // step * step


class Planar:

    __slots__ = ("buf", "C", "F", "B", "T", "Tp", "Jp", "lengths")

    def __init__(self, buf, C, F, B, T, Tp, Jp, lengths=None):
        self.buf, self.C, self.F, self.B, self.T, self.Tp, self.Jp, self.lengths = buf, C, F, B, T, Tp, Jp, lengths

    @staticmethod
    def jp_for(B: int, Tp: int) -> int:
        return (B * Tp + 3) // 4 * 4

    @classmethod
    def empty(cls, C, F, B, T, Tp, device, zero=False):
        Jp = cls.jp_for(B, Tp)
        n = bucket(2 * C * F * Jp + 2 * SLACK)
        buf = (torch.zeros if zero else torch.empty)(n, dtype=torch.float32, device=device)
        return cls(buf, C, F, B, T, Tp, Jp)

    @property
    def data(self) -> torch.Tensor:
        return self.buf[SLACK:SLACK + 2 * self.C * self.F * self.Jp]

    def ptr(self, plane_offset: int = 0):
        return L._P(self.buf.data_ptr() + 4 * (SLACK + plane_offset * self.F * self.Jp))

    def planes(self) -> torch.Tensor:
        return torch.as_strided(self.buf, (2, self.C, self.F, self.B, self.Tp),
                                (self.C * self.F * self.Jp, self.F * self.Jp, self.Jp, self.Tp, 1), SLACK)

    def tensor5(self) -> torch.Tensor:
        return self.planes()[..., 1:1 + self.T].permute(3, 1, 2, 4, 0)

    def tensor4(self) -> torch.Tensor:
        return self.tensor5()[:, 0]

    def channel_slice(self, c0: int, c1: int) -> torch.Tensor:
        assert self.F == 1
        return self.planes()[:, c0:c1, 0, :, 1:1 + self.T].permute(2, 3, 1, 0)

    @classmethod
    def from_tensor5(cls, x: torch.Tensor, Tp: Optional[int] = None):
        B, C, F, T, _ = x.shape
        Tp = Tp or T + 1
        out = cls.empty(C, F, B, T, Tp, x.device, zero=True)
        out.tensor5().copy_(x)
        return out


IMG_SLACK = 4096
IMAGE_PATH = os.environ.get("IDV_IMAGE_PATH", "1") != "0"
IMAGE_TRAIN = os.environ.get("IDV_IMAGE_TRAIN", "1") != "0"


class Image:

    __slots__ = ("buf", "C", "F", "B", "T", "Tp", "Jp", "lo_off")

    def __init__(self, buf, C, F, B, T, Tp, Jp, lo_off):
        self.buf, self.C, self.F, self.B, self.T, self.Tp, self.Jp, self.lo_off = buf, C, F, B, T, Tp, Jp, lo_off

    @classmethod
    def empty(cls, C, F, B, T, Tp, device):
        Jp = Planar.jp_for(B, Tp)
        plane = (2 * C + 7) // 8 * F * Jp * 8
        lo_off = plane + IMG_SLACK
        buf = torch.empty(bucket(2 * IMG_SLACK + lo_off + plane), dtype=torch.int16, device=device)
        return cls(buf, C, F, B, T, Tp, Jp, lo_off)

    def ptr(self):
        return L._P(self.buf.data_ptr() + 2 * IMG_SLACK)

    @property
    def lo_slots(self) -> int:
        return self.lo_off // 8


def to_image(x: Planar) -> Image:
    out = Image.empty(x.C, x.F, x.B, x.T, x.Tp, x.buf.device)
    call("idv_planar_to_image", x.ptr(), i(x.C), i(x.F), i(x.B * x.Tp), i(x.Jp), out.ptr(), ll(out.lo_off), stream_ptr())
    return out


def to_image_repeat(x: Planar, n: int) -> Image:
    out = Image.empty(x.C, x.F, x.B * n, x.T, x.Tp, x.buf.device)
    call("idv_planar_to_image_repeat", x.ptr(), i(x.C), i(x.F), i(x.B), i(x.Tp), i(x.Jp), i(n), out.ptr(), ll(out.lo_off),
         i(out.Jp), stream_ptr())
    return out


def to_planar(x: Image) -> Planar:
    out = Planar.empty(x.C, x.F, x.B, x.T, x.Tp, x.buf.device)
    call("idv_image_to_planar", x.ptr(), ll(x.lo_off), i(x.C), i(x.F), i(x.B * x.Tp), i(x.Jp), out.ptr(), stream_ptr())
    return out


class KImage:

    __slots__ = ("buf", "nplanes", "Jp", "lo_off")

    def __init__(self, nplanes: int, Jp: int, device):
        assert nplanes % 8 == 0
        plane = nplanes // 8 * Jp * 8
        self.nplanes, self.Jp, self.lo_off = nplanes, Jp, plane + IMG_SLACK
        self.buf = torch.empty(bucket(2 * IMG_SLACK + self.lo_off + plane), dtype=torch.int16, device=device)

    def ptr(self, octet: int = 0):
        return L._P(self.buf.data_ptr() + 2 * IMG_SLACK + 16 * octet * self.Jp)

    @property
    def lo_slots(self) -> int:
        return self.lo_off // 8

    @classmethod
    def from_planes(cls, x_ptr, nvalid: int, J: int, Jp: int, device, pad_to: int = 8):
        nplanes = (nvalid + pad_to - 1) // pad_to * pad_to
        out = cls(nplanes, Jp, device)
        call("idv_planar_to_kimage", x_ptr, i(nvalid), i(nplanes), i(J), i(Jp), out.ptr(), ll(out.lo_off), stream_ptr())
        return out


def pack_pw_bf16(w):
    M, K = w.shape
    L.lib().idv_pw_bf16_wfrag_bytes.restype = L._L
    wf = torch.empty(int(L.lib().idv_pw_bf16_wfrag_bytes(i(M), i(K))), dtype=torch.uint8, device=w.device)
    call("idv_pack_pw_bf16", p(w.contiguous()), i(M), i(K), p(wf), stream_ptr())
    return wf


def pw_bf16x3(kimg: KImage, octet0: int, K: int, wfrag16, bias, M: int, B: int, Tp: int, t_valid: int, out_ptr):
    call("idv_pw_bf16x3", kimg.ptr(octet0), ll(kimg.lo_slots), i(K), p(wfrag16), p(bias), out_ptr, i(M), i(B), i(Tp), i(kimg.Jp),
         i(t_valid), stream_ptr())


def pw_bf16x3_rows(kimg: KImage, K: int, wfrag16, bias, M: int, ldo: int, B: int, T: int, Tp: int, out_ptr):
    call("idv_pw_bf16x3_rows", kimg.ptr(), ll(kimg.lo_slots), i(K), p(wfrag16), p(bias), out_ptr, i(M), i(ldo), i(B), i(T), i(Tp),
         i(kimg.Jp), stream_ptr())


def _dev_scratch(n: int, device, dtype=torch.float32, zero=False):
    return (torch.zeros if zero else torch.empty)(n, dtype=dtype, device=device)


def mtiles_alloc(M: int) -> int:
    return (M + 127) // 128 * 4


def cbn_fold(moments, g_rr, g_ri, g_ii, b_r, b_i):
    C = g_rr.numel()
    fold = torch.empty(C, 6, dtype=torch.float32, device=g_rr.device)
    call("idv_cbn_fold", p(moments), p(g_rr), p(g_ri), p(g_ii), p(b_r), p(b_i), i(C), p(fold), stream_ptr())
    return fold


def pack_cconv(w_re, w_im, b_re, b_im, fold, cin_used: Optional[int] = None, transposed=False):
    if transposed:
        cin_total, cout = w_re.shape[0], w_re.shape[1]
    else:
        cout, cin_total = w_re.shape[0], w_re.shape[1]
    cin_used = cin_total if cin_used is None else cin_used
    cck = L.lib().idv_cconv_cck(cin_used)
    ccp = (2 * cin_used + cck - 1) // cck * cck
    mt = mtiles_alloc(2 * cout)
    wfrag = torch.empty(mt * ccp * 5 * 64, dtype=torch.float32, device=w_re.device)
    bias = torch.empty(mt * 32, dtype=torch.float32, device=w_re.device)
    call("idv_pack_cconv", p(w_re.contiguous()), p(w_im.contiguous()), p(b_re.contiguous()), p(b_im.contiguous()),
         p(fold), i(cout), i(cin_total), i(cin_used), i(1 if transposed else 0), p(wfrag), p(bias), stream_ptr())
    return wfrag, bias


SKIP_ONCE = os.environ.get("IDV_SKIP_ONCE", "1") != "0"
GAUSS_FWD = os.environ.get("IDV_GAUSS_FWD", "1") != "0"
GAUSS_BWD = os.environ.get("IDV_GAUSS_BWD", "1") != "0"


def gauss_supported(c0: int, c1: int, cout: int, bwd: bool = False) -> bool:
    if not (GAUSS_BWD if bwd else GAUSS_FWD):
        return False
    return bool(L.lib().idv_cconv_gauss_supported(i(c0), i(c1), i(cout)))


def pack_cconv_gauss(w_re, w_im, b_re, b_im, fold, cin_used: Optional[int] = None, transposed=False, *, adjoint_of=None):
    if adjoint_of is not None:
        cout, cin_total, cin_used, transposed = adjoint_of
    else:
        if transposed:
            cin_total, cout = w_re.shape[0], w_re.shape[1]
        else:
            cout, cin_total = w_re.shape[0], w_re.shape[1]
        cin_used = cin_total if cin_used is None else cin_used
    lib = L.lib()
    lib.idv_cconv_gauss_wfrag_floats.restype = L._L
    wfrag = torch.empty(int(lib.idv_cconv_gauss_wfrag_floats(i(cout), i(cin_used))), dtype=torch.float32, device=w_re.device)
    epi = torch.empty(int(lib.idv_cconv_gauss_epi_rows(i(cout))) * 8, dtype=torch.float32, device=w_re.device)
    if adjoint_of is not None:
        call("idv_pack_cconv_gauss", p(w_re), p(w_im), p(None), p(None), p(None), i(cout), i(cin_total), i(cin_used),
             i(1 if transposed else 0), i(1), p(wfrag), p(epi), stream_ptr())
        return (wfrag, epi, 0) + _pack_wino_tw(w_re, w_im, cout, cin_total, cin_used, transposed, 1)
    w_re, w_im = w_re.contiguous(), w_im.contiguous()
    call("idv_pack_cconv_gauss", p(w_re), p(w_im), p(b_re.contiguous()), p(b_im.contiguous()), p(fold),
         i(cout), i(cin_total), i(cin_used), i(1 if transposed else 0), i(0), p(wfrag), p(epi), stream_ptr())
    return (wfrag, epi, (1 if fold is not None else 0)) + _pack_wino_tw(w_re, w_im, cout, cin_total, cin_used, transposed, 0)


WINO = os.environ.get("IDV_WINO", "1") != "0"
WINO_CFG = 4000000


def _pack_wino(w_re, w_im, cout: int, cin_total: int, cin_used: int, transposed: bool, conj: int):
    if not WINO:
        return None
    n = int(_ll_fn("idv_cconv_wino_wfrag_floats")(i(1 if transposed else 0), i(cout), i(cin_used)))
    wf = torch.empty(n, dtype=torch.float32, device=w_re.device)
    call("idv_pack_cconv_wino", p(w_re), p(w_im), i(cout), i(cin_total), i(cin_used), i(1 if transposed else 0), i(conj), p(wf),
         stream_ptr())
    return wf


TW = os.environ.get("IDV_TW", "1") != "0"
TW_CONV = os.environ.get("IDV_TW_CONV", "1") != "0"
TW_CFG = 5000000


def _pack_wino_tw(w_re, w_im, cout: int, cin_total: int, cin_used: int, transposed: bool, conj: int):
    wf = _pack_wino(w_re, w_im, cout, cin_total, cin_used, transposed, conj)
    if wf is None or not TW or (not transposed and not TW_CONV):
        return wf, None
    if transposed:
        tw = torch.empty(int(_ll_fn("idv_cconv_tw_wfrag_floats")(i(cout), i(cin_used))), dtype=torch.float32, device=w_re.device)
        call("idv_pack_cconv_tw", p(wf), i(cout), i(cin_used), p(tw), stream_ptr())
    else:
        tw = torch.empty(int(_ll_fn("idv_cconv_tw2_wfrag_floats")(i(cout), i(cin_used))), dtype=torch.float32, device=w_re.device)
        call("idv_pack_cconv_tw2", p(wf), i(cout), i(cin_used), p(tw), stream_ptr())
    return wf, tw


def _tw2_ok(gauss, x: Planar, c1: int, cout: int) -> bool:
    return (gauss is not None and TW and TW_CONV and WINO and c1 == 0 and len(gauss) > 4 and gauss[4] is not None and x.Jp % 4 == 0
            and bool(L.lib().idv_cconv_tw2_supported(i(x.C), i(cout), i(x.F))))


def _tw_ok(gauss, x: Planar, c1: int, cout: int, skip_jp: Optional[int]) -> bool:
    return (gauss is not None and TW and WINO and len(gauss) > 4 and gauss[4] is not None and x.Jp % 4 == 0
            and (skip_jp is None or skip_jp == x.Jp) and bool(L.lib().idv_cconv_tw_supported(i(x.C), i(c1), i(cout), i(x.F))))


def _wino_ok(gauss, transposed: bool, x: Planar, c1: int, cout: int, skip_jp: Optional[int]) -> bool:
    return (gauss is not None and WINO and len(gauss) > 3 and gauss[3] is not None and x.Jp % 4 == 0
            and (skip_jp is None or skip_jp == x.Jp)
            and bool(L.lib().idv_cconv_wino_supported(i(1 if transposed else 0), i(x.C), i(c1), i(cout), i(x.F))))


def pack_cconv_gauss_skip_part(w_re, w_im, c0: int):
    wr, wi = w_re[c0:].contiguous(), w_im[c0:].contiguous()
    cin, cout = wr.shape[0], wr.shape[1]
    lib = L.lib()
    lib.idv_cconv_gauss_wfrag_floats.restype = L._L
    wfrag = torch.empty(int(lib.idv_cconv_gauss_wfrag_floats(i(cout), i(cin))), dtype=torch.float32, device=wr.device)
    epi = torch.empty(int(lib.idv_cconv_gauss_epi_rows(i(cout))) * 8, dtype=torch.float32, device=wr.device)
    call("idv_pack_cconv_gauss", p(wr), p(wi), p(None), p(None), p(None), i(cout), i(cin), i(cin), i(1), i(0), p(wfrag), p(epi),
         stream_ptr())
    return (wfrag, epi, 0) + _pack_wino_tw(wr, wi, cout, cin, cin, True, 0)


def bf16_supported(transposed: bool, c0: int, c1: int, skip_div: int, cout: int) -> bool:
    return bool(L.lib().idv_cconv_bf16_supported(i(1 if transposed else 0), i(c0), i(c1), i(skip_div), i(cout)))


def pack_cconv_bf16(w_re, w_im, fold, cin_used: Optional[int] = None, transposed=False):
    if transposed:
        cin_total, cout = w_re.shape[0], w_re.shape[1]
    else:
        cout, cin_total = w_re.shape[0], w_re.shape[1]
    cin_used = cin_total if cin_used is None else cin_used
    L.lib().idv_cconv_bf16_wfrag_bytes.restype = L._L
    nbytes = L.lib().idv_cconv_bf16_wfrag_bytes(i(cout), i(cin_used))
    wfrag = torch.empty(int(nbytes), dtype=torch.uint8, device=w_re.device)
    call("idv_pack_cconv_bf16", p(w_re.contiguous()), p(w_im.contiguous()), p(fold), i(cout), i(cin_total), i(cin_used),
         i(1 if transposed else 0), p(wfrag), stream_ptr())
    return wfrag


def pack_ctconv_c1(w_re, w_im, fold, cin_used: Optional[int] = None):
    cin_total = w_re.shape[0]
    cin_used = cin_total if cin_used is None else cin_used
    L.lib().idv_ctconv_c1_wfrag_bytes.restype = L._L
    wfrag = torch.empty(int(L.lib().idv_ctconv_c1_wfrag_bytes(i(cin_used))), dtype=torch.uint8, device=w_re.device)
    call("idv_pack_ctconv_c1_bf16", p(w_re.contiguous()), p(w_im.contiguous()), p(fold), i(cin_total), i(cin_used), p(wfrag),
         stream_ptr())
    return wfrag


def ctconv_c1(x, wfrag_c1, bias, *, slope=None, skip=None) -> Planar:
    out = Planar.empty(1, 2 * x.F - 1, x.B, x.T, x.Tp, x.buf.device)
    c1 = skip.C if skip is not None else 0
    if LAUNCH_LOG is not None:
        macs = 4 * (x.C + c1) * 10 * x.B * x.T * x.F
        ev0, ev1 = torch.cuda.Event(enable_timing=True), torch.cuda.Event(enable_timing=True)
        ev0.record()
    if isinstance(x, Image):
        if skip is not None and not isinstance(skip, Image):
            raise RuntimeError("ctconv_c1: x and skip must have the same format")
        call("idv_ctconv_c1_img_fwd", x.ptr(), ll(x.lo_slots), i(x.C), skip.ptr() if skip is not None else p(None),
             ll(skip.lo_slots if skip is not None else 0), i(c1), p(wfrag_c1), p(bias), p(slope), out.ptr(), i(x.F), i(x.B),
             i(x.Tp), i(x.Jp), i(x.T), stream_ptr())
    else:
        call("idv_ctconv_c1_bf16x3_fwd", x.ptr(), i(x.C), skip.ptr() if skip is not None else p(None), i(c1),
             i(skip.Jp if skip is not None else 0), p(wfrag_c1), p(bias), p(slope), out.ptr(), i(x.F), i(x.B), i(x.Tp), i(x.Jp),
             i(x.T), stream_ptr())
    if LAUNCH_LOG is not None:
        ev1.record()
        LAUNCH_LOG.append((-98 if isinstance(x, Image) else -99, macs, ev0, ev1))
    return out


def pack_pw(w, bias):
    M, K = w.shape
    mt = mtiles_alloc(M)
    ks = (K + 7) // 8 * 4
    wfrag = torch.empty(mt * ks * 64, dtype=torch.float32, device=w.device)
    bout = torch.empty(mt * 32, dtype=torch.float32, device=w.device)
    call("idv_pack_pw", p(w.contiguous()), p(None if bias is None else bias.contiguous()), i(M), i(K), p(wfrag),
         p(bout), stream_ptr())
    return wfrag, bout


LAUNCH_LOG = None

STREAM_SPLIT = int(os.environ.get("IDV_STREAM_SPLIT", "1"))
CONCURRENT = os.environ.get("IDV_CONCURRENT", "0") != "0"
STREAM_STAGGER = os.environ.get("IDV_STREAM_STAGGER", "1") != "0"
STREAM_STAGGER_BELOW = 1 << 30
STREAM_SPLIT_MIN_BATCH = 16
_SIDE_STREAMS = {}


def stream_split(batch: int) -> int:
    n = max(1, STREAM_SPLIT)
    while n > 1 and batch < n * STREAM_SPLIT_MIN_BATCH:
        n -= 1
    return n


def side_streams(n: int, device):
    key = (torch.device(device).index or 0)
    pool = _SIDE_STREAMS.setdefault(key, [])
    while len(pool) < n:
        pool.append(torch.cuda.Stream(device=device))
    return pool[:n]


def repeat_batch(x: Planar, n: int) -> Planar:
    out = Planar.empty(x.C, x.F, x.B * n, x.T, x.Tp, x.buf.device)
    dst = torch.as_strided(out.buf, (2, x.C, x.F, x.B, n, x.Tp),
                           (x.C * x.F * out.Jp, x.F * out.Jp, out.Jp, n * x.Tp, x.Tp, 1), SLACK)
    dst.copy_(x.planes().unsqueeze(4).expand(2, x.C, x.F, x.B, n, x.Tp))
    return out


def concurrent(fns, device=None):
    if not CONCURRENT:
        return [fn() for fn in fns]
    device = torch.device("cuda", torch.cuda.current_device()) if device is None else device
    main = torch.cuda.current_stream(device)
    streams = side_streams(len(fns), device)
    ready = torch.cuda.Event()
    ready.record(main)
    outs = []
    for fn, st in zip(fns, streams):
        st.wait_event(ready)
        with torch.cuda.stream(st):
            outs.append(fn())
    for st in streams:
        main.wait_stream(st)
    hand_over(outs, main)
    return outs


def hand_over(obj, stream):
    if isinstance(obj, torch.Tensor):
        if obj.is_cuda:
            obj.record_stream(stream)
        pl = getattr(obj, "_idv", None)
        if pl is not None and isinstance(getattr(pl, "buf", None), torch.Tensor) and pl.buf.is_cuda:
            pl.buf.record_stream(stream)
    elif isinstance(obj, (Planar, Image)):
        obj.buf.record_stream(stream)
    elif isinstance(obj, (tuple, list)):
        for o in obj:
            hand_over(o, stream)


class CoopTimeout(RuntimeError):
    """A cooperative (spin-synchronised) recurrence ran into its spin bound: its outputs are NaN-poisoned."""


def coop_check(sync: bool = True, clear: bool = True) -> None:
    if sync:
        torch.cuda.current_stream().synchronize()
    if L.lib().idv_coop_last_status(1 if clear else 0) != 0:
        raise CoopTimeout("a cooperative LSTM recurrence timed out on this device (a sibling workgroup never became resident, e.g. "
                          "a CU-masked or shared GPU): results computed since the last check are NaN-poisoned"
                          + ("" if clear else "; cooperative launches are refused until ops.coop_clear()"))


def coop_clear() -> bool:
    return L.lib().idv_coop_last_status(1) != 0


STATS_REP = int(os.environ.get("IDV_STATS_REP", "32"))


def _stats_work(stats, cout: int):
    if stats is None or STATS_REP < 2:
        return None
    return torch.zeros(STATS_REP, cout, 5, dtype=torch.float64, device=stats.device)


def cconv2d(x: Planar, wfrag, bias, cout: int, *, transposed=False, causal=True, slope=None, skip: Optional[Planar] = None,
            skip_div: int = 1, stats: Optional[torch.Tensor] = None, out: Optional[Planar] = None,
            wfrag_bf16: Optional[torch.Tensor] = None, image: str = "", adjoint_time: bool = False, gauss=None,
            addend: Optional[Planar] = None, addend_div: int = 1):
    Fout = 2 * x.F - 1 if transposed else (x.F - 1) // 2 + 1
    if causal:
        t_out = x.T
    else:
        t_out = x.T + 1 if transposed else x.T - 1
    tshift = -1 if (causal or transposed) else 0
    if adjoint_time:
        assert transposed and causal
        tshift = 0
    if out is None and image != "only":
        out = Planar.empty(cout, Fout, x.B, t_out, x.Tp, x.buf.device)
    c1 = skip.C if skip is not None else 0
    if image:
        assert stats is None and skip_div == 1 and wfrag_bf16 is None
        img = Image.empty(cout, Fout, x.B, t_out, x.Tp, x.buf.device)
        call("idv_cconv2d_fwd_img", x.ptr(), i(x.C), skip.ptr() if skip is not None else p(None), i(c1),
             i(skip.Jp if skip is not None else 0), p(wfrag), p(bias), p(slope), out.ptr() if out is not None else p(None),
             img.ptr(), ll(img.lo_off), i(1 if transposed else 0), i(tshift), i(cout), i(x.F), i(x.B), i(x.Tp), i(x.Jp),
             i(t_out), stream_ptr())
        return out, img
    if LAUNCH_LOG is not None:
        cfg = L.lib().idv_cconv_config(i(1 if transposed else 0), i(x.C + c1), i(cout), i(x.F))
        pos = x.B * x.T * (x.F if transposed else Fout)
        macs = 4 * (x.C + c1) * cout * 10 * pos
        ev0, ev1 = torch.cuda.Event(enable_timing=True), torch.cuda.Event(enable_timing=True)
        ev0.record()
    if wfrag_bf16 is not None:
        if LAUNCH_LOG is not None:
            cfg = -(1000000 + L.lib().idv_cconv_bf16_config(i(1 if transposed else 0), i(cout), i(x.F)))
        swork = _stats_work(stats, cout)
        call("idv_cconv2d_bf16x3_fwd", x.ptr(), i(x.C), skip.ptr() if skip is not None else p(None), i(c1),
             i(skip.Jp if skip is not None else 0), i(skip_div), p(wfrag_bf16), p(bias), p(slope), out.ptr(), p(stats), p(swork),
             i(STATS_REP), i(1 if transposed else 0), i(tshift), i(cout), i(x.F), i(x.B), i(x.Tp), i(x.Jp), i(t_out), stream_ptr())
        if LAUNCH_LOG is not None:
            ev1.record()
            LAUNCH_LOG.append((cfg, macs, ev0, ev1))
        return out
    if transposed and skip_div == 1 and _tw_ok(gauss, x, c1, cout, skip.Jp if skip is not None else None):
        if LAUNCH_LOG is not None:
            cfg = TW_CFG + (1 if tshift else 0)
        swork = _stats_work(stats, cout)
        call("idv_ctconv2d_tw_fwd", x.ptr(), i(x.C), skip.ptr() if skip is not None else p(None), i(c1), p(gauss[4]), p(gauss[1]),
             i(gauss[2]), p(slope), out.ptr(), p(stats), p(swork), i(STATS_REP), i(tshift), i(cout), i(x.F), i(x.B), i(x.Tp), i(x.Jp),
             i(t_out), addend.ptr() if addend is not None else p(None), i(addend_div), i(addend.Jp if addend is not None else 0),
             stream_ptr())
    elif not transposed and addend is None and _tw2_ok(gauss, x, c1, cout):
        if LAUNCH_LOG is not None:
            cfg = TW_CFG + 2 + (1 if tshift else 0)
        swork = _stats_work(stats, cout)
        call("idv_cconv2d_tw_fwd", x.ptr(), i(x.C), p(gauss[4]), p(gauss[1]), i(gauss[2]), p(slope), out.ptr(), p(stats), p(swork),
             i(STATS_REP), i(tshift), i(cout), i(x.F), i(x.B), i(x.Tp), i(x.Jp), i(t_out), stream_ptr())
    elif skip_div == 1 and _wino_ok(gauss, transposed, x, c1, cout, skip.Jp if skip is not None else None):
        if LAUNCH_LOG is not None:
            cfg = WINO_CFG + (1000 if transposed else 0) + L.lib().idv_cconv_wino_config(i(1 if transposed else 0), i(x.C + c1), i(cout))
        swork = _stats_work(stats, cout)
        call("idv_cconv2d_wino_fwd", x.ptr(), i(x.C), skip.ptr() if skip is not None else p(None), i(c1), p(gauss[3]), p(gauss[1]),
             i(gauss[2]), p(slope), out.ptr(), p(stats), p(swork), i(STATS_REP), i(1 if transposed else 0), i(tshift), i(cout), i(x.F),
             i(x.B), i(x.Tp), i(x.Jp), i(t_out), addend.ptr() if addend is not None else p(None), i(addend_div),
             i(addend.Jp if addend is not None else 0), stream_ptr())
    elif gauss is not None:
        if LAUNCH_LOG is not None:
            cfg = L.lib().idv_cconv_gauss_config(i(1 if transposed else 0), i(x.C + c1), i(cout), i(x.F))
        swork = _stats_work(stats, cout)
        call("idv_cconv2d_gauss_fwd", x.ptr(), i(x.C), skip.ptr() if skip is not None else p(None), i(c1),
             i(skip.Jp if skip is not None else 0), i(skip_div), p(gauss[0]), p(gauss[1]), i(gauss[2]), p(slope), out.ptr(),
             p(stats), p(swork), i(STATS_REP), i(1 if transposed else 0), i(tshift), i(cout), i(x.F), i(x.B), i(x.Tp), i(x.Jp), i(t_out),
             addend.ptr() if addend is not None else p(None), i(addend_div), i(addend.Jp if addend is not None else 0), stream_ptr())
    else:
        swork = _stats_work(stats, cout)
        call("idv_cconv2d_fwd", x.ptr(), i(x.C), skip.ptr() if skip is not None else p(None), i(c1),
             i(skip.Jp if skip is not None else 0), i(skip_div), p(wfrag), p(bias), p(slope), out.ptr(), p(stats), p(swork),
             i(STATS_REP), i(1 if transposed else 0), i(tshift), i(cout), i(x.F), i(x.B), i(x.Tp), i(x.Jp), i(t_out), stream_ptr())
    if LAUNCH_LOG is not None:
        ev1.record()
        LAUNCH_LOG.append((cfg, macs, ev0, ev1))
    return out


def cconv2d_img(x, wfrag_bf16, bias, cout: int, *, transposed=False, causal=True, slope=None, skip=None,
                want_planar=False, want_image=True, adjoint=False):
    src_img = isinstance(x, Image)
    if skip is not None and isinstance(skip, Image) != src_img:
        raise RuntimeError("cconv2d_img: x and skip must have the same format")
    Fout = 2 * x.F - 1 if transposed else (x.F - 1) // 2 + 1
    t_out = x.T if causal else (x.T + 1 if transposed else x.T - 1)
    tshift = -1 if (causal or transposed) else 0
    if adjoint:
        assert causal
        tshift, t_out = 0, x.T
    dev = x.buf.device
    outp = Planar.empty(cout, Fout, x.B, t_out, x.Tp, dev) if want_planar else None
    outi = Image.empty(cout, Fout, x.B, t_out, x.Tp, dev) if want_image else None
    c1 = skip.C if skip is not None else 0
    if LAUNCH_LOG is not None:
        cfg = -(100000000 + L.lib().idv_cconv_img_config(i(1 if src_img else 0), i(1 if transposed else 0), i(x.C + c1),
                                                          i(cout), i(x.F)))
        pos = x.B * x.T * (x.F if transposed else Fout)
        macs = 4 * (x.C + c1) * cout * 10 * pos
        ev0, ev1 = torch.cuda.Event(enable_timing=True), torch.cuda.Event(enable_timing=True)
        ev0.record()
    call("idv_cconv2d_img_fwd", i(1 if src_img else 0), x.ptr(), ll(x.lo_slots if src_img else 0), i(x.C),
         skip.ptr() if skip is not None else p(None), ll(skip.lo_slots if (skip is not None and src_img) else 0), i(c1),
         p(wfrag_bf16), p(bias), p(slope), outp.ptr() if outp is not None else p(None),
         outi.ptr() if outi is not None else p(None), ll(outi.lo_off if outi is not None else 0),
         i(1 if transposed else 0), i(tshift), i(cout), i(x.F), i(x.B), i(x.Tp), i(x.Jp), i(t_out), stream_ptr())
    if LAUNCH_LOG is not None:
        ev1.record()
        LAUNCH_LOG.append((cfg, macs, ev0, ev1))
    return outp, outi


def cconv2d_img_train(x: Image, wfrag_bf16, bias, cout: int, stats, *, transposed=False, skip: Optional[Image] = None) -> Planar:
    Fout = 2 * x.F - 1 if transposed else (x.F - 1) // 2 + 1
    out = Planar.empty(cout, Fout, x.B, x.T, x.Tp, x.buf.device)
    c1 = skip.C if skip is not None else 0
    if LAUNCH_LOG is not None:
        cfg = -(100000000 + L.lib().idv_cconv_img_config(i(1), i(1 if transposed else 0), i(x.C + c1), i(cout), i(x.F)))
        macs = 4 * (x.C + c1) * cout * 10 * x.B * x.T * (x.F if transposed else Fout)
        ev0, ev1 = torch.cuda.Event(enable_timing=True), torch.cuda.Event(enable_timing=True)
        ev0.record()
    swork = _stats_work(stats, cout)
    call("idv_cconv2d_img_train_fwd", x.ptr(), ll(x.lo_slots), i(x.C), skip.ptr() if skip is not None else p(None),
         ll(skip.lo_slots if skip is not None else 0), i(c1), p(wfrag_bf16), p(bias), out.ptr(), p(stats), p(swork), i(STATS_REP),
         i(1 if transposed else 0), i(cout), i(x.F), i(x.B), i(x.Tp), i(x.Jp), i(x.T), stream_ptr())
    if LAUNCH_LOG is not None:
        ev1.record()
        LAUNCH_LOG.append((cfg, macs, ev0, ev1))
    return out


def pw_gemm(x_ptr, K: int, wfrag, bias, M: int, B: int, Tp: int, Jp: int, t_valid: int, out_ptr, *, slope=None,
            swap=False, ldo=0):
    call("idv_pw_gemm", x_ptr, i(K), p(wfrag), p(bias), p(slope), out_ptr, i(M), i(B), i(Tp), i(Jp), i(t_valid),
         i(1 if swap else 0), i(ldo), stream_ptr())


def pack_lstm(sd_get, H: int, K: int, layer: int, device):
    g = lambda n: sd_get(n).contiguous()
    l = layer
    M = 8 * H
    mt = mtiles_alloc(M)
    ks = (K + 7) // 8 * 4
    wih = torch.empty(mt * ks * 64, dtype=torch.float32, device=device)
    bih = torch.empty(mt * 32, dtype=torch.float32, device=device)
    call("idv_pack_lstm_ih", p(g(f"lstm_re.weight_ih_l{l}")), p(g(f"lstm_re.bias_ih_l{l}")), p(g(f"lstm_re.bias_hh_l{l}")),
         p(g(f"lstm_im.weight_ih_l{l}")), p(g(f"lstm_im.bias_ih_l{l}")), p(g(f"lstm_im.bias_hh_l{l}")), i(H), i(K),
         p(wih), p(bih), stream_ptr())
    whh = torch.empty(4 * 4 * H * H, dtype=torch.float32, device=device)
    call("idv_pack_lstm_hh", p(g(f"lstm_re.weight_hh_l{l}")), p(g(f"lstm_im.weight_hh_l{l}")), i(H), p(whh), stream_ptr())
    wih16 = None
    if L.lib().idv_lstm_proj_bf16_supported(i(H), i(K)) and (layer == 0 or (4 * H) % 256 == 0):
        L.lib().idv_lstm_ih_bf16_bytes.restype = L._L
        wih16 = torch.empty(int(L.lib().idv_lstm_ih_bf16_bytes(i(H), i(K))), dtype=torch.uint8, device=device)
        call("idv_pack_lstm_ih_bf16", p(g(f"lstm_re.weight_ih_l{l}")), p(g(f"lstm_im.weight_ih_l{l}")), i(H), i(K), p(wih16),
             stream_ptr())
    wih_hh = None
    if layer == 1 and K == H and H == 128:
        wih_hh = torch.empty(4 * 4 * H * H, dtype=torch.float32, device=device)
        call("idv_pack_lstm_hh", p(g(f"lstm_re.weight_ih_l{l}")), p(g(f"lstm_im.weight_ih_l{l}")), i(H), p(wih_hh), stream_ptr())
    return wih, bih, whh, wih16, wih_hh


LSTM_PERSISTENT = os.environ.get("IDV_LSTM_PERSISTENT", "1") != "0"
LSTM_STACK2 = os.environ.get("IDV_LSTM_STACK2", "1") != "0"


def clstm(x: Planar, packed0, packed1, H: int) -> Planar:
    K = x.C * x.F
    out = Planar.empty(H, 1, x.B, x.T, x.Tp, x.buf.device)
    nwork = L.lib().idv_clstm_work_floats(i(H), i(x.B), i(x.T), i(x.Jp))
    work = torch.empty(bucket(int(nwork)), dtype=torch.float32, device=x.buf.device)
    flags = 1 if PRECISION == "bf16x3" else 0
    if not LSTM_PERSISTENT:
        flags |= 8
    if (flags & 1) and packed0[3] is not None:
        kimg = KImage.from_planes(x.ptr(), 2 * K, x.B * x.Tp, x.Jp, x.buf.device)
        call("idv_lstm_proj_bf16x3", kimg.ptr(), ll(kimg.lo_slots), i(K), p(packed0[3]), p(packed0[1]), p(work), i(H), i(x.B),
             i(x.T), i(x.Tp), i(x.Jp), stream_ptr())
        flags |= 2
    call("idv_clstm_fwd2", x.ptr(), i(K), p(packed0[0]), p(packed0[1]), p(packed0[2]), p(packed1[0]), p(packed1[1]),
         p(packed1[2]), p(packed1[4] if (LSTM_STACK2 and len(packed1) > 4) else None), i(H), i(x.B), i(x.T), i(x.Tp), i(x.Jp), p(work), out.ptr(),
         i(flags), p(packed1[3] if (flags & 1) else None), stream_ptr())
    return out


def cdense(x: Planar, packed_r, packed_i, M: int, C_out: int, F_out: int) -> Planar:
    K = x.C * x.F
    out = Planar.empty(C_out, F_out, x.B, x.T, x.Tp, x.buf.device)
    if PRECISION == "bf16x3" and K % 64 == 0 and len(packed_r) > 2 and packed_r[2] is not None:
        kimg = KImage.from_planes(x.ptr(), 2 * K, x.B * x.Tp, x.Jp, x.buf.device)
        for ri, pk in enumerate((packed_r, packed_i)):
            pw_bf16x3(kimg, ri * K // 8, K, pk[2], pk[1], M, x.B, x.Tp, x.T, out.ptr(ri * C_out))
        return out
    for ri, pk in enumerate((packed_r, packed_i)):
        pw_gemm(x.ptr(ri * x.C), K, pk[0], pk[1], M, x.B, x.Tp, x.Jp, x.T, out.ptr(ri * C_out))
    return out


class DftPlan:

    def __init__(self, n_fft, win, hop, T, device):
        self.n_fft, self.win, self.hop, self.T = n_fft, win, hop, T
        self.F = n_fft // 2 + 1
        F = self.F
        w_fwd = torch.empty(2 * F, win, dtype=torch.float32, device=device)
        w_inv = torch.empty(win, 2 * F, dtype=torch.float32, device=device)
        self.env_inv = torch.empty(n_fft + hop * (T - 1), dtype=torch.float32, device=device)
        call("idv_make_dft", i(n_fft), i(win), i(hop), i(T), p(w_fwd), p(w_inv), p(self.env_inv), stream_ptr())
        self.fwd = pack_pw(w_fwd, None)
        self.inv = pack_pw(w_inv, None)
        self.fwd16 = pack_pw_bf16(w_fwd)
        self.inv16 = pack_pw_bf16(w_inv)
        self._w_fwd, self._w_inv = w_fwd, w_inv
        self._fwd_T = self._inv_T = None

    def fwd_T(self):
        if self._fwd_T is None:
            self._fwd_T = pack_pw(self._w_fwd.t().contiguous(), None)
        return self._fwd_T

    def inv_T(self):
        if self._inv_T is None:
            self._inv_T = pack_pw(self._w_inv.t().contiguous(), None)
        return self._inv_T


def check_lengths(lengths, B: int, L: int, n_fft: Optional[int]) -> list:
    if isinstance(lengths, Lengths):
        lengths = lengths.host
    if isinstance(lengths, torch.Tensor):
        if lengths.is_cuda:
            raise ValueError("lengths must be a python sequence or a CPU integer tensor: they size the batch on the host, and "
                             "a GPU tensor would have to be fetched with a synchronisation")
        if lengths.dim() != 1 or lengths.is_floating_point() or lengths.is_complex() or lengths.dtype == torch.bool:
            raise ValueError("lengths must be a 1-D integer tensor")
        lengths = lengths.tolist()
    elif isinstance(lengths, (str, bytes)) or not isinstance(lengths, Sequence):
        raise ValueError("lengths must be a python sequence or a CPU integer tensor")
    if any(isinstance(v, bool) or not isinstance(v, int) for v in lengths):
        raise ValueError("lengths must be integers (sample counts)")
    if len(lengths) != B:
        raise ValueError(f"{len(lengths)} lengths for a batch of {B} utterances")
    for b, v in enumerate(lengths):
        if n_fft is None and v <= 0:
            raise ValueError(f"lengths[{b}] = {v}: a length must be positive")
        if n_fft is not None and v <= n_fft // 2:
            raise ValueError(f"lengths[{b}] = {v}: torch.stft's reflect padding needs more than n_fft/2 = {n_fft // 2} samples")
        if v > L:
            raise ValueError(f"lengths[{b}] = {v} exceeds the {L} samples per row of the padded batch")
    return list(lengths)


class Lengths:

    __slots__ = ("host", "dev")

    def __init__(self, host, device, dev=None):
        self.host = list(host)
        self.dev = torch.tensor(self.host, dtype=torch.int32, device=device) if dev is None else dev

    def __len__(self):
        return len(self.host)

    def part(self, b0: int, b1: int) -> "Lengths":
        return Lengths(self.host[b0:b1], None, self.dev[b0:b1])

    def outputs(self, hop: int) -> "Lengths":
        return Lengths([hop * (v // hop) for v in self.host], self.dev.device)


def _ragged_rows(x: torch.Tensor) -> torch.Tensor:
    if x.dtype != torch.float32 or x.stride(1) != 1 or x.stride(0) < x.shape[1]:
        x = x.float().contiguous()
    return x


def stft(x: torch.Tensor, plan: DftPlan, Tp: Optional[int] = None, lengths=None) -> Planar:
    if lengths is not None:
        return _stft_ragged(x, plan, Tp, lengths)
    B, Lx = x.shape
    T = 1 + Lx // plan.hop
    assert T == plan.T, "DftPlan built for another length"
    Tp = Tp or T + 1
    x = x.contiguous()
    if PRECISION == "bf16x3":
        Jp = Planar.jp_for(B, Tp)
        kimg = KImage((plan.win + 63) // 64 * 64, Jp, x.device)
        call("idv_stft_frames_kimage", p(x), i(B), i(Lx), i(plan.n_fft), i(plan.win), i(plan.hop), i(T), kimg.ptr(),
             ll(kimg.lo_off), i(Tp), i(Jp), stream_ptr())
        out = Planar.empty(1, plan.F, B, T, Tp, x.device)
        pw_bf16x3(kimg, 0, plan.win, plan.fwd16, None, 2 * plan.F, B, Tp, T, out.ptr())
        return out
    fr = Planar.empty(1, plan.win // 2, B, T, Tp, x.device)
    assert plan.win % 2 == 0
    call("idv_stft_frames", p(x), i(B), i(Lx), i(plan.n_fft), i(plan.win), i(plan.hop), i(T), fr.ptr(), i(Tp), i(fr.Jp),
         stream_ptr())
    out = Planar.empty(1, plan.F, B, T, Tp, x.device)
    pw_gemm(fr.ptr(), plan.win, plan.fwd[0], plan.fwd[1], 2 * plan.F, B, Tp, fr.Jp, T, out.ptr())
    return out


def _stft_ragged(x: torch.Tensor, plan: DftPlan, Tp: Optional[int], lengths) -> Planar:
    B, Lx = x.shape
    T = 1 + Lx // plan.hop
    assert T == plan.T, "DftPlan built for another length"
    host = check_lengths(lengths, B, Lx, plan.n_fft)
    if not isinstance(lengths, Lengths):
        lengths = Lengths(host, x.device)
    Tp = Tp or T + 1
    x = _ragged_rows(x)
    assert plan.win % 2 == 0
    out = Planar.empty(1, plan.F, B, T, Tp, x.device)
    out.lengths = lengths
    if PRECISION == "bf16x3":
        kimg = KImage((plan.win + 63) // 64 * 64, out.Jp, x.device)
        call("idv_stft_frames_kimage_ragged", p(x), ll(x.stride(0)), p(lengths.dev), i(B), i(plan.n_fft), i(plan.win), i(plan.hop),
             i(T), kimg.ptr(), ll(kimg.lo_off), i(Tp), i(out.Jp), stream_ptr())
        pw_bf16x3(kimg, 0, plan.win, plan.fwd16, None, 2 * plan.F, B, Tp, T, out.ptr())
        return out
    fr = Planar.empty(1, plan.win // 2, B, T, Tp, x.device)
    call("idv_stft_frames_ragged", p(x), ll(x.stride(0)), p(lengths.dev), i(B), i(plan.n_fft), i(plan.win), i(plan.hop), i(T),
         fr.ptr(), i(Tp), i(fr.Jp), stream_ptr())
    pw_gemm(fr.ptr(), plan.win, plan.fwd[0], plan.fwd[1], 2 * plan.F, B, Tp, fr.Jp, T, out.ptr())
    return out


def istft(spec: Planar, plan: DftPlan, lengths=None) -> torch.Tensor:
    B, T = spec.B, spec.T
    if lengths is not None:
        nl = len(lengths)
        if nl < 1 or B % nl:
            raise ValueError(f"{nl} lengths for {B} rows: the row count must be a multiple of the number of lengths")
        if not isinstance(lengths, Lengths):
            lengths = Lengths(check_lengths(lengths, nl, plan.hop * T + plan.hop - 1, plan.n_fft), spec.buf.device)
        if max(lengths.host) // plan.hop + 1 > T:
            raise ValueError("a length needs more frames than the spectrum holds")
    fr = Planar.empty(1, plan.win // 2, B, T, spec.Tp, spec.buf.device)
    if PRECISION == "bf16x3":
        kimg = KImage.from_planes(spec.ptr(), 2 * plan.F, B * spec.Tp, spec.Jp, spec.buf.device, pad_to=64)
        pw_bf16x3(kimg, 0, 2 * plan.F, plan.inv16, None, plan.win, B, spec.Tp, T, fr.ptr())
    else:
        pw_gemm(spec.ptr(), 2 * plan.F, plan.inv[0], plan.inv[1], plan.win, B, spec.Tp, spec.Jp, T, fr.ptr())
    y = torch.empty(B, plan.hop * (T - 1), dtype=torch.float32, device=spec.buf.device)
    if lengths is not None:
        call("idv_istft_ola_ragged", fr.ptr(), p(lengths.dev), i(B // len(lengths)), i(B), i(plan.n_fft), i(plan.win), i(plan.hop),
             i(T), i(spec.Tp), i(fr.Jp), p(y), ll(y.stride(0)), stream_ptr())
        return y
    call("idv_istft_ola", fr.ptr(), p(plan.env_inv), i(B), i(plan.n_fft), i(plan.win), i(plan.hop), i(T), i(spec.Tp),
         i(fr.Jp), p(y), stream_ptr())
    return y


def mask_apply(mask: Planar, X: Planar, x_div: int = 1):
    B, F, T = mask.B, mask.F, mask.T
    pred = Planar.empty(1, F, B, T, mask.Tp, mask.buf.device)
    pc = torch.empty(B, F, T, 2, dtype=torch.float32, device=mask.buf.device)
    call("idv_mask_apply", mask.ptr(), X.ptr(), i(x_div), i(X.Jp), pred.ptr(), p(pc), i(F), i(B), i(T), i(mask.Tp),
         i(mask.Jp), stream_ptr())
    return pred, torch.view_as_complex(pc)


def msd(a: Planar, ca0: int, b: Planar, cb0: int, C: int) -> torch.Tensor:
    work = torch.empty(3, dtype=torch.float64, device=a.buf.device)
    out = torch.empty(1, dtype=torch.float32, device=a.buf.device)
    call("idv_msd", a.ptr(), i(a.C), i(ca0), i(a.Jp), b.ptr(), i(b.C), i(cb0), i(b.Jp), i(C), i(a.F), i(a.B), i(a.Tp), i(a.T),
         p(work), p(out), stream_ptr())
    return out[0]


def planar_to_complex(act: Planar) -> torch.Tensor:
    pc = torch.empty(act.B, act.F, act.T, 2, dtype=torch.float32, device=act.buf.device)
    call("idv_planar_to_complex", act.ptr(), p(pc), i(act.F), i(act.B), i(act.T), i(act.Tp), i(act.Jp), stream_ptr())
    return torch.view_as_complex(pc)


def cbn_train(act: Planar, stats: torch.Tensor, bn, slope, first_call: bool, momentum: float = 0.9):
    C = act.C
    dev = act.buf.device
    moments = torch.empty(5, C, dtype=torch.float32, device=dev)
    fold = torch.empty(C, 6, dtype=torch.float32, device=dev)
    count = float(act.B) * act.F * act.T
    if BN_SYNC is not None:
        count = count * BN_SYNC(stats)
    call("idv_cbn_finalize", p(stats), d(count), p(bn.gamma_rr), p(bn.gamma_ri), p(bn.gamma_ii), p(bn.beta_r), p(bn.beta_i),
         i(C), i(1 if first_call else 0), f(momentum), p(bn.running_mean_real), p(bn.running_mean_imag), p(bn.Vrr), p(bn.Vri),
         p(bn.Vii), p(moments), p(fold), stream_ptr())
    call("idv_cbn_apply_prelu", act.ptr(), p(fold), p(slope), i(C), i(act.F), i(act.B), i(act.Tp), i(act.Jp), i(act.T),
         stream_ptr())
    return moments


def reparam(lat: Planar, off, zdim: int, eps_r, eps_i, ns: int) -> Planar:
    B, T = lat.B, lat.T
    z = Planar.empty(zdim, 1, B * ns, T, lat.Tp, lat.buf.device)
    call("idv_reparam", lat.ptr(), i(lat.C), i(off[0]), i(off[1]), i(off[2]), i(zdim), p(eps_r.contiguous()),
         p(eps_i.contiguous()), i(ns), i(B), i(T), i(lat.Tp), i(lat.Jp), z.ptr(), i(z.Jp), stream_ptr())
    return z


def check_dev_f32(t: torch.Tensor, name: str, device=None):
    if not isinstance(t, torch.Tensor) or not t.is_cuda:
        raise L.IdvError(f"{name}: expected a CUDA (ROCm) tensor, got {type(t).__name__} on "
                         f"{getattr(t, 'device', '?')}; the HIP hot path has no CPU fallback")
    if device is not None and t.device != torch.device(device):
        raise L.IdvError(f"{name}: on {t.device}, expected {device}")


def sisnr(source: torch.Tensor, est: torch.Tensor, src_div: int = 1) -> torch.Tensor:
    B, Ln = est.shape
    check_dev_f32(source, "source", est.device)
    if source.dtype != torch.float32 or est.dtype != torch.float32 or source.shape[-1] < Ln:
        raise L.IdvError("sisnr: float32 tensors with source length >= estimate length expected")
    assert source.stride(-1) == 1 and est.stride(-1) == 1
    work = torch.empty(3 * B, dtype=torch.float64, device=est.device)
    out = torch.empty(1, dtype=torch.float32, device=est.device)
    call("idv_sisnr", p(source), i(source.stride(0)), i(src_div), p(est), i(est.stride(0)), i(B), i(Ln), p(work), p(out),
         stream_ptr())
    return out[0]


def recon_loss(pred_c: torch.Tensor, ori: torch.Tensor, ori_div: int = 1):
    pr = torch.view_as_real(pred_c)
    assert pr.is_contiguous()
    check_dev_f32(ori, "ori_cpx_stft", pr.device)
    if ori.dtype != torch.float32:
        raise L.IdvError("recon_loss: float32 STFT expected")
    B, F, T, _ = pr.shape
    if tuple(ori.shape[1:]) != (F, T, 2):
        raise L.IdvError(f"recon_loss: STFT shape {tuple(ori.shape)} does not match the prediction {tuple(pr.shape)}")
    work = torch.empty(3, dtype=torch.float64, device=pr.device)
    out = torch.empty(2, dtype=torch.float32, device=pr.device)
    sb, sf, st, sr = ori.stride()
    call("idv_recon_loss", p(pr), p(ori), ll(sb), ll(sf), ll(st), ll(sr), i(ori_div), i(B), i(F), i(T), p(work), p(out),
         stream_ptr())
    return out[0], out[1]


def ckl(q1: Planar, off1, q2: Optional[Planar], off2, zdim: int, eps: float) -> torch.Tensor:
    work = torch.empty(3, dtype=torch.float64, device=q1.buf.device)
    out = torch.empty(1, dtype=torch.float32, device=q1.buf.device)
    o2 = off2 if q2 is not None else (0, 0, 0)
    call("idv_ckl", q1.ptr(), i(q1.C), i(q1.Jp), i(off1[0]), i(off1[1]), i(off1[2]),
         q2.ptr() if q2 is not None else p(None), i(q2.C if q2 is not None else 0), i(q2.Jp if q2 is not None else 0),
         i(o2[0]), i(o2[1]), i(o2[2]), i(zdim), f(eps), i(q1.B), i(q1.T), i(q1.Tp), p(work), p(out), stream_ptr())
    return out[0]


def mi_estimate(lat: Planar, off, z: Planar, zdim: int, ns: int, eps: float):
    lib = L.lib()
    lib.idv_mi_work_floats.restype = L._L
    if (z.C, z.B, z.T, z.Tp) != (zdim, lat.B * ns, lat.T, lat.Tp):
        raise ValueError(f"mutual_information: samples {(z.C, z.B, z.T)} do not belong to a posterior {(zdim, lat.B, lat.T)} x {ns}")
    work = torch.empty(int(lib.idv_mi_work_floats(i(lat.B), i(ns), i(lat.T), i(zdim))), dtype=torch.float32, device=lat.buf.device)
    acc = torch.empty(1, dtype=torch.float64, device=lat.buf.device)
    out = torch.empty(1, dtype=torch.float32, device=lat.buf.device)
    call("idv_mi_fwd", lat.ptr(), i(lat.C), i(lat.Jp), i(off[0]), i(off[1]), i(off[2]), z.ptr(), i(z.Jp), i(zdim), i(ns), i(lat.B),
         i(lat.T), i(lat.Tp), f(eps), p(work), p(acc), p(out), stream_ptr())
    return out[0], work


def mi_bwd(lat: Planar, off, z: Planar, zdim: int, ns: int, eps: float, work, gout, dlat: Optional[Planar], dz: Optional[Planar]):
    call("idv_mi_bwd", lat.ptr(), i(lat.C), i(lat.Jp), i(off[0]), i(off[1]), i(off[2]), z.ptr(), i(z.Jp), i(zdim), i(ns), i(lat.B),
         i(lat.T), i(lat.Tp), f(eps), p(work), p(gout), dlat.ptr() if dlat is not None else p(None),
         dz.ptr() if dz is not None else p(None), stream_ptr())


def miu_dist(q1: Planar, off1: int, q2: Planar, off2: int, zdim: int) -> torch.Tensor:
    work = torch.empty(3 * 2 * zdim, dtype=torch.float64, device=q1.buf.device)
    out = torch.empty(1, dtype=torch.float32, device=q1.buf.device)
    call("idv_miu_dist", q1.ptr(), i(q1.C), i(q1.Jp), i(off1), q2.ptr(), i(q2.C), i(q2.Jp), i(off2), i(zdim), i(q1.B), i(q1.T),
         i(q1.Tp), p(work), p(out), stream_ptr())
    return out[0]


def cbn_stats(act: Planar) -> torch.Tensor:
    stats = torch.zeros(act.C, 5, dtype=torch.float64, device=act.buf.device)
    call("idv_cbn_stats", act.ptr(), i(act.C), i(act.F), i(act.B), i(act.Tp), i(act.Jp), i(act.T), p(stats), stream_ptr())
    return stats


def cbn_apply(act: Planar, fold: torch.Tensor, slope=None):
    call("idv_cbn_apply_prelu", act.ptr(), p(fold), p(slope), i(act.C), i(act.F), i(act.B), i(act.Tp), i(act.Jp), i(act.T),
         stream_ptr())
    return act


_LL = L._L


def _ll_fn(name):
    fn = getattr(L.lib(), name)
    fn.restype = _LL
    return fn


def like(x: Planar, C: Optional[int] = None, F: Optional[int] = None, zero=False) -> Planar:
    return Planar.empty(x.C if C is None else C, x.F if F is None else F, x.B, x.T, x.Tp, x.buf.device, zero=zero)


def rewrap(buf: torch.Tensor, x: Planar, C: Optional[int] = None, F: Optional[int] = None) -> Planar:
    return Planar(buf, x.C if C is None else C, x.F if F is None else F, x.B, x.T, x.Tp, x.Jp)


def pack_cconv_adjoint(w_re, w_im, cout: int, cin_total: int, cin_used: int, transposed: bool):
    cck = L.lib().idv_cconv_cck(cin_used)
    ccp = (2 * cin_used + cck - 1) // cck * cck
    mt = mtiles_alloc(2 * cout)
    wfrag = torch.empty(mt * ccp * 5 * 64, dtype=torch.float32, device=w_re.device)
    bias = torch.empty(mt * 32, dtype=torch.float32, device=w_re.device)
    call("idv_pack_cconv_adjoint", p(w_re), p(w_im), i(cout), i(cin_total), i(cin_used), i(1 if transposed else 0), p(wfrag),
         p(bias), stream_ptr())
    return wfrag, bias


def pack_cconv_bf16_adjoint(w_re, w_im, cout: int, cin_total: int, cin_used: int, transposed: bool):
    L.lib().idv_cconv_bf16_wfrag_bytes.restype = L._L
    wfrag = torch.empty(int(L.lib().idv_cconv_bf16_wfrag_bytes(i(cout), i(cin_used))), dtype=torch.uint8, device=w_re.device)
    call("idv_pack_cconv_bf16_adjoint", p(w_re), p(w_im), i(cout), i(cin_total), i(cin_used), i(1 if transposed else 0),
         p(wfrag), stream_ptr())
    return wfrag


_ZBIAS = {}


def zero_bias(cout: int, device):
    key = (mtiles_alloc(2 * cout), str(device))
    if key not in _ZBIAS:
        _ZBIAS[key] = torch.zeros(key[0] * 32, dtype=torch.float32, device=device)
        torch.cuda.current_stream(device).synchronize()
    return _ZBIAS[key]


def cconv_dgrad(dy: Planar, wfrag, bias, cout_adj: int, fwd_transposed: bool, causal: bool, wfrag_bf16=None, gauss=None) -> Planar:
    adj_transposed = not fwd_transposed
    Fout = 2 * dy.F - 1 if adj_transposed else (dy.F - 1) // 2 + 1
    if causal:
        tshift_adj, t_out = 0, dy.T
    elif adj_transposed:
        tshift_adj, t_out = -1, dy.T + 1
    else:
        tshift_adj, t_out = 0, dy.T - 1
    if t_out + 1 > dy.Tp:
        raise RuntimeError("cconv_dgrad: the input of the block had more frames than the buffer's columns per utterance")
    out = Planar.empty(cout_adj, Fout, dy.B, t_out, dy.Tp, dy.buf.device)
    if LAUNCH_LOG is not None:
        cfg = L.lib().idv_cconv_config(i(1 if adj_transposed else 0), i(dy.C), i(cout_adj), i(dy.F))
        macs = 4 * dy.C * cout_adj * 10 * dy.B * dy.T * (dy.F if adj_transposed else Fout)
        ev0, ev1 = torch.cuda.Event(enable_timing=True), torch.cuda.Event(enable_timing=True)
        if wfrag_bf16 is not None:
            cfg = -(1000000 + L.lib().idv_cconv_bf16_config(i(1 if adj_transposed else 0), i(cout_adj), i(dy.F)))
        ev0.record()
    if wfrag_bf16 is None and adj_transposed and _tw_ok(gauss, dy, 0, cout_adj, None):
        if LAUNCH_LOG is not None:
            cfg = TW_CFG + (1 if tshift_adj else 0)
        call("idv_ctconv2d_tw_fwd", dy.ptr(), i(dy.C), p(None), i(0), p(gauss[4]), p(gauss[1]), i(0), p(None), out.ptr(), p(None), p(None),
             i(0), i(tshift_adj), i(cout_adj), i(dy.F), i(dy.B), i(dy.Tp), i(dy.Jp), i(t_out), p(None), i(1), i(0), stream_ptr())
    elif wfrag_bf16 is None and not adj_transposed and _tw2_ok(gauss, dy, 0, cout_adj):
        if LAUNCH_LOG is not None:
            cfg = TW_CFG + 2 + (1 if tshift_adj else 0)
        call("idv_cconv2d_tw_fwd", dy.ptr(), i(dy.C), p(gauss[4]), p(gauss[1]), i(0), p(None), out.ptr(), p(None), p(None), i(0),
             i(tshift_adj), i(cout_adj), i(dy.F), i(dy.B), i(dy.Tp), i(dy.Jp), i(t_out), stream_ptr())
    elif wfrag_bf16 is None and _wino_ok(gauss, adj_transposed, dy, 0, cout_adj, None):
        if LAUNCH_LOG is not None:
            cfg = WINO_CFG + (1000 if adj_transposed else 0) + L.lib().idv_cconv_wino_config(i(1 if adj_transposed else 0), i(dy.C), i(cout_adj))
        call("idv_cconv2d_wino_fwd", dy.ptr(), i(dy.C), p(None), i(0), p(gauss[3]), p(gauss[1]), i(0), p(None), out.ptr(), p(None), p(None),
             i(0), i(1 if adj_transposed else 0), i(tshift_adj), i(cout_adj), i(dy.F), i(dy.B), i(dy.Tp), i(dy.Jp), i(t_out), p(None), i(1),
             i(0), stream_ptr())
    elif gauss is not None and wfrag_bf16 is None:
        if LAUNCH_LOG is not None:
            cfg = L.lib().idv_cconv_gauss_config(i(1 if adj_transposed else 0), i(dy.C), i(cout_adj), i(dy.F))
        call("idv_cconv2d_gauss_fwd", dy.ptr(), i(dy.C), p(None), i(0), i(0), i(1), p(gauss[0]), p(gauss[1]), i(0), p(None),
             out.ptr(), p(None), p(None), i(0), i(1 if adj_transposed else 0), i(tshift_adj), i(cout_adj), i(dy.F), i(dy.B), i(dy.Tp),
             i(dy.Jp), i(t_out), p(None), i(1), i(0), stream_ptr())
    elif wfrag_bf16 is not None:
        call("idv_cconv2d_bf16x3_fwd", dy.ptr(), i(dy.C), p(None), i(0), i(0), i(1), p(wfrag_bf16), p(bias), p(None), out.ptr(), p(None),
             p(None), i(0), i(1 if adj_transposed else 0), i(tshift_adj), i(cout_adj), i(dy.F), i(dy.B), i(dy.Tp), i(dy.Jp), i(t_out),
             stream_ptr())
    else:
        call("idv_cconv2d_fwd", dy.ptr(), i(dy.C), p(None), i(0), i(0), i(1), p(wfrag), p(bias), p(None), out.ptr(), p(None), p(None),
             i(0), i(1 if adj_transposed else 0), i(tshift_adj), i(cout_adj), i(dy.F), i(dy.B), i(dy.Tp), i(dy.Jp), i(t_out), stream_ptr())
    if LAUNCH_LOG is not None:
        ev1.record()
        LAUNCH_LOG.append((cfg, macs, ev0, ev1))
    return out


_WORK = {}
WGRAD_BF16_CFG = -96
WGRAD_BF16 = os.environ.get("IDV_WGRAD_BF16", "1") != "0"
WGRAD_GAUSS_CFG = -95
WGRAD_CFG = -97


def _scratch(n: int, device, tag="w") -> torch.Tensor:
    key = (str(device), torch.cuda.current_stream().cuda_stream, tag)
    t = _WORK.get(key)
    if t is None or t.numel() < n:
        t = torch.empty(bucket(n), dtype=torch.float32, device=device)
        _WORK[key] = t
    return t


def cconv_wgrad(x: Planar, ci_off: int, dy: Planar, cout: int, cin_total: int, transposed: bool, causal: bool, dw_re, dw_im):
    tshift = -1 if (causal or transposed) else 0
    cs, cl = (x.C, cout) if transposed else (cout, x.C)
    bf16 = PRECISION == "bf16x3" and WGRAD_BF16 and 2 * cs >= 32 and 2 * cl >= 32
    gauss = not bf16 and bool(L.lib().idv_cconv_wgrad_gauss_supported(i(cs), i(cl)))
    if gauss:
        n = int(_ll_fn("idv_cconv_wgrad_gauss_work_floats")(i(x.C), i(cout), i(1 if transposed else 0), i(x.F), i(x.B), i(x.Tp),
                                                            i(x.Jp), i(dy.Jp)))
    else:
        n = int(_ll_fn("idv_cconv_wgrad_bf16_work_floats" if bf16 else "idv_cconv_wgrad_work_floats")(i(cs), i(cl), i(x.B), i(x.Tp)))
    work = _scratch(n, x.buf.device)
    if LAUNCH_LOG is not None:
        macs = 4 * x.C * cout * 10 * x.B * x.T * (x.F if transposed else dy.F)
        ev0, ev1 = torch.cuda.Event(enable_timing=True), torch.cuda.Event(enable_timing=True)
        ev0.record()
    call("idv_cconv2d_bwd_weight_bf16x3" if bf16 else ("idv_cconv2d_bwd_weight_gauss" if gauss else "idv_cconv2d_bwd_weight"),
         x.ptr(), i(x.C), i(ci_off), dy.ptr(), i(cout), i(cin_total), i(1 if transposed else 0),
         i(tshift), i(x.F), i(x.B), i(x.Tp), i(x.Jp), i(dy.Jp), p(work), ll(work.numel()), p(dw_re), p(dw_im), stream_ptr())
    if LAUNCH_LOG is not None:
        ev1.record()
        LAUNCH_LOG.append((WGRAD_BF16_CFG if bf16 else (WGRAD_GAUSS_CFG if gauss else WGRAD_CFG), macs, ev0, ev1))


def cconv_bias_grad(dy: Planar):
    stats = cbn_stats(dy)
    db_re = torch.empty(dy.C, dtype=torch.float32, device=dy.buf.device)
    db_im = torch.empty_like(db_re)
    call("idv_cconv2d_bwd_bias", p(stats), i(dy.C), p(db_re), p(db_im), stream_ptr())
    return db_re, db_im


def train_image_ok(C: int) -> bool:
    return PRECISION == "bf16x3" and IMAGE_TRAIN and C % 8 == 0 and 2 * C >= 64


def cbn_apply_to(y: Planar, fold, slope, want_image: bool = False):
    out = like(y)
    if want_image:
        img = Image.empty(y.C, y.F, y.B, y.T, y.Tp, y.buf.device)
        call("idv_cbn_apply_prelu_to_img", y.ptr(), p(fold), p(slope), i(y.C), i(y.F), i(y.B), i(y.Tp), i(y.Jp), i(y.T), out.ptr(),
             img.ptr(), ll(img.lo_off), stream_ptr())
        return out, img
    call("idv_cbn_apply_prelu_to", y.ptr(), p(fold), p(slope), i(y.C), i(y.F), i(y.B), i(y.Tp), i(y.Jp), i(y.T), out.ptr(),
         stream_ptr())
    return out


BN_SYNC = None


def cbn_bwd(dz: Planar, y: Planar, fold, moments, bn, slope, count: float, want_image: bool = False):
    C, dev = y.C, y.buf.device
    sums = torch.empty(C, 8, dtype=torch.float64, device=dev)
    call("idv_cbn_bwd_reduce", dz.ptr(), y.ptr(), p(fold), p(slope), i(C), i(y.F), i(y.B), i(y.Tp), i(y.Jp), i(y.T), p(sums),
         stream_ptr())
    world = 1
    if BN_SYNC is not None:
        world = BN_SYNC(sums)
        count = count * world
    coef = torch.empty(C, 12, dtype=torch.float32, device=dev)
    g = [torch.empty(C, dtype=torch.float32, device=dev) for _ in range(5)]
    dslope = torch.zeros(1, dtype=torch.float32, device=dev)
    call("idv_cbn_bwd_finalize", p(sums), d(count), p(moments), p(bn[0]), p(bn[1]), p(bn[2]), i(C), p(coef), p(g[0]), p(g[1]),
         p(g[2]), p(g[3]), p(g[4]), p(dslope if slope is not None else None), f(1.0 / world), stream_ptr())
    dy = like(y)
    if want_image:
        img = Image.empty(y.C, y.F, y.B, y.T, y.Tp, dev)
        call("idv_cbn_bwd_apply_img", dz.ptr(), y.ptr(), p(fold), p(coef), p(slope), i(C), i(y.F), i(y.B), i(y.Tp), i(y.Jp), i(y.T),
             dy.ptr(), img.ptr(), ll(img.lo_off), stream_ptr())
        return ((dy, img), *g, dslope)
    call("idv_cbn_bwd_apply", dz.ptr(), y.ptr(), p(fold), p(coef), p(slope), i(C), i(y.F), i(y.B), i(y.Tp), i(y.Jp), i(y.T),
         dy.ptr(), stream_ptr())
    return (dy, *g, dslope)


def cbn_finalize(stats, count: float, bn_mod, first_call: bool, momentum: float, update_running: bool = True):
    C = bn_mod.C
    dev = stats.device
    if BN_SYNC is not None:
        count = count * BN_SYNC(stats)
    moments = torch.empty(5, C, dtype=torch.float32, device=dev)
    fold = torch.empty(C, 6, dtype=torch.float32, device=dev)
    rb = (bn_mod.running_mean_real, bn_mod.running_mean_imag, bn_mod.Vrr, bn_mod.Vri, bn_mod.Vii) if update_running else (None,) * 5
    call("idv_cbn_finalize", p(stats), d(count), p(bn_mod.gamma_rr), p(bn_mod.gamma_ri), p(bn_mod.gamma_ii), p(bn_mod.beta_r),
         p(bn_mod.beta_i), i(C), i(1 if first_call else 0), f(momentum), p(rb[0]), p(rb[1]), p(rb[2]), p(rb[3]), p(rb[4]),
         p(moments), p(fold), stream_ptr())
    return moments, fold


def pw_wgrad(dout_ptr, M: int, Jp_d: int, x_ptr, K: int, Jp_x: int, J: int, dw: torch.Tensor, *, shift=0, rowmap=0, H=0,
             accumulate=False):
    n = int(_ll_fn("idv_pw_wgrad_work_floats")(i(M), i(K), i(J)))
    work = _scratch(n, dw.device)
    bf16 = PRECISION == "bf16x3" and WGRAD_BF16 and M >= 64 and K >= 64
    call("idv_pw_bwd_weight_bf16x3" if bf16 else "idv_pw_bwd_weight", dout_ptr, i(M), i(Jp_d), x_ptr, i(K), i(Jp_x), i(J), i(shift), p(work), ll(work.numel()), p(dw),
         i(dw.stride(0)), i(rowmap), i(H), i(1 if accumulate else 0), stream_ptr())


def planar_rowsum(x_ptr, M: int, Jp: int, J: int, out: torch.Tensor, accumulate=False):
    call("idv_planar_rowsum", x_ptr, i(M), i(Jp), i(J), i(1 if accumulate else 0), p(out), stream_ptr())


def mask_apply_bwd(mask: Planar, X: Planar, x_div: int, dpred: Optional[Planar], dpred_c, want_dx: bool = False):
    dm = like(mask)
    dX = like(X) if want_dx else None
    call("idv_mask_apply_bwd", mask.ptr(), X.ptr(), i(x_div), i(X.Jp), dpred.ptr() if dpred is not None else p(None),
         p(dpred_c), i(mask.F), i(mask.B), i(mask.T), i(mask.Tp), i(mask.Jp), dm.ptr(), dX.ptr() if dX is not None else p(None),
         stream_ptr())
    return dm, dX


def complex_to_planar(xc: torch.Tensor, Tp: Optional[int] = None) -> Planar:
    B, F, T, _ = xc.shape
    out = Planar.empty(1, F, B, T, Tp or T + 1, xc.device)
    call("idv_complex_to_planar", p(xc.contiguous()), out.ptr(), i(F), i(B), i(T), i(out.Tp), i(out.Jp), stream_ptr())
    return out


def istft_bwd(dy: torch.Tensor, spec: Planar, plan: "DftPlan") -> Planar:
    B, T = spec.B, spec.T
    dfr = Planar.empty(1, plan.win // 2, B, T, spec.Tp, dy.device)
    call("idv_istft_ola_bwd", p(dy.contiguous()), p(plan.env_inv), i(B), i(plan.n_fft), i(plan.win), i(plan.hop), i(T),
         i(spec.Tp), i(dfr.Jp), dfr.ptr(), stream_ptr())
    out = like(spec)
    wT = plan.inv_T()
    pw_gemm(dfr.ptr(), plan.win, wT[0], wT[1], 2 * plan.F, B, spec.Tp, dfr.Jp, T, out.ptr())
    return out


def stft_bwd(dX: Planar, plan: "DftPlan", Lx: int) -> torch.Tensor:
    B, T = dX.B, dX.T
    dfr = Planar.empty(1, plan.win // 2, B, T, dX.Tp, dX.buf.device)
    wT = plan.fwd_T()
    pw_gemm(dX.ptr(), 2 * plan.F, wT[0], wT[1], plan.win, B, dX.Tp, dX.Jp, T, dfr.ptr())
    dx = torch.empty(B, Lx, dtype=torch.float32, device=dX.buf.device)
    call("idv_stft_frames_bwd", dfr.ptr(), i(B), i(Lx), i(plan.n_fft), i(plan.win), i(plan.hop), i(T), i(dX.Tp), i(dfr.Jp),
         p(dx), stream_ptr())
    return dx


def reparam_bwd(lat: Planar, off, zdim: int, eps_r, eps_i, ns: int, dz: Planar, dlat: Planar):
    call("idv_reparam_bwd", lat.ptr(), i(lat.C), i(off[0]), i(off[1]), i(off[2]), i(zdim), p(eps_r), p(eps_i), i(ns), i(lat.B),
         i(lat.T), i(lat.Tp), i(lat.Jp), dz.ptr(), i(dz.Jp), dlat.ptr(), stream_ptr())
```

include/idccrn_hip.h:

```cpp
#ifndef IDCCRN_HIP_H
#define IDCCRN_HIP_H

#ifdef __cplusplus
extern "C" {
#endif

#define IDV_ABI_VERSION 9
#define IDV_SLACK_FLOATS 256

int idv_abi_version(void);

int idv_coop_last_status(int clear);
int idv_coop_max_workgroups(void);


int idv_cconv_cck(int cin_used);
int idv_cconv_config(int transposed, int cin_used, int Cout, int Fin);

int idv_cbn_fold(const float* moments, const float* gamma_rr, const float* gamma_ri, const float* gamma_ii,
                 const float* beta_r, const float* beta_i, int C, float* fold, void* stream);

int idv_pack_cconv(const float* w_re, const float* w_im, const float* b_re, const float* b_im, const float* fold,
                   int Cout, int Cin_total, int Cin_used, int transposed, float* wfrag, float* bias_out, void* stream);

int idv_pack_pw(const float* w, const float* bias, int M, int K, float* wfrag, float* bias_out, void* stream);

int idv_pack_lstm_ih(const float* w_ih_re, const float* b_ih_re, const float* b_hh_re, const float* w_ih_im,
                     const float* b_ih_im, const float* b_hh_im, int H, int K, float* wfrag, float* bias_out,
                     void* stream);
int idv_pack_lstm_hh(const float* w_hh_re, const float* w_hh_im, int H, float* whh_frag, void* stream);

int idv_make_dft(int n_fft, int win, int hop, int T, float* w_fwd, float* w_inv, float* env_inv, void* stream);


int idv_cconv2d_fwd(const float* x0, int C0, const float* x1, int C1, int Jp1, int x1_div, const float* wfrag,
                    const float* bias, const float* prelu_slope, float* out, double* stats, double* stats_work, int stats_rep,
                    int transposed, int tshift, int Cout, int Fin, int B, int Tp, int Jp, int t_valid_out, void* stream);

int idv_cconv_gauss_supported(int C0, int C1, int Cout);
long long idv_cconv_gauss_wfrag_floats(int Cout, int cin_used);
int idv_cconv_gauss_epi_rows(int Cout);
int idv_cconv_gauss_config(int transposed, int Cin, int Cout, int Fin);
int idv_pack_cconv_gauss(const float* w_re, const float* w_im, const float* b_re, const float* b_im, const float* fold, int Cout,
                         int Cin_total, int Cin_used, int transposed, int conj, float* wfrag, float* epi, void* stream);
int idv_cconv2d_gauss_fwd(const float* x0, int C0, const float* x1, int C1, int Jp1, int x1_div, const float* wfrag,
                          const float* epi, int has_fold, const float* prelu_slope, float* out, double* stats, double* stats_work,
                          int stats_rep, int transposed, int tshift, int Cout, int Fin, int B, int Tp, int Jp, int t_valid_out,
                          const float* addend, int addend_div, int addend_Jp, void* stream);

long long idv_cconv_bf16_wfrag_bytes(int Cout, int cin_used);
int idv_cconv_bf16_supported(int transposed, int C0, int C1, int x1_div, int Cout);
int idv_cconv_bf16_config(int transposed, int Cout, int Fin);
int idv_pack_cconv_bf16(const float* w_re, const float* w_im, const float* fold, int Cout, int Cin_total, int Cin_used,
                        int transposed, void* wfrag, void* stream);
int idv_cconv2d_bf16x3_fwd(const float* x0, int C0, const float* x1, int C1, int Jp1, int x1_div, const void* wfrag_bf16,
                           const float* bias, const float* prelu_slope, float* out, double* stats, double* stats_work,
                           int stats_rep, int transposed, int tshift, int Cout, int Fin, int B, int Tp, int Jp, int t_valid_out,
                           void* stream);

int idv_cconv2d_fwd_img(const float* x0, int C0, const float* x1, int C1, int Jp1, const float* wfrag, const float* bias,
                        const float* prelu_slope, float* out_planar, void* out_img, long long out_lo_off_elems,
                        int transposed, int tshift, int Cout, int Fin, int B, int Tp, int Jp, int t_valid_out,
                        void* stream);
int idv_cconv2d_img_train_fwd(const void* x0_img, long long lo_off0, int C0, const void* x1_img, long long lo_off1, int C1,
                              const void* wfrag_bf16, const float* bias, float* out_planar, double* stats, double* stats_work,
                              int stats_rep, int transposed, int Cout, int Fin, int B, int Tp, int Jp, int t_valid_out, void* stream);
int idv_cconv_img_config(int src_is_image, int transposed, int Cin, int Cout, int Fin);
int idv_planar_to_image(const float* x, int C, int F, int J, int Jp, void* img, long long lo_off_elems, void* stream);
int idv_planar_to_image_repeat(const float* x, int C, int F, int B, int Tp, int Jp_in, int rep, void* img, long long lo_off_elems,
                               int Jp, void* stream);
int idv_image_to_planar(const void* img, long long lo_off_elems, int C, int F, int J, int Jp, float* x, void* stream);
int idv_cconv2d_img_fwd(int src_is_image , const void* x0_img, long long lo_off0_slots, int C0, const void* x1_img, long long lo_off1_slots,
                        int C1, const void* wfrag_bf16, const float* bias, const float* prelu_slope, float* out_planar,
                        void* out_img, long long out_lo_off_elems, int transposed, int tshift,
                        int Cout, int Fin, int B, int Tp, int Jp, int t_valid_out, void* stream);

long long idv_ctconv_c1_wfrag_bytes(int cin_used);
int idv_pack_ctconv_c1_bf16(const float* w_re, const float* w_im, const float* fold, int Cin_total, int Cin_used,
                            void* wfrag, void* stream);
int idv_ctconv_c1_bf16x3_fwd(const float* x0, int C0, const float* x1, int C1, int Jp1, const void* wfrag,
                             const float* bias, const float* prelu_slope, float* out, int Fin, int B, int Tp, int Jp,
                             int t_valid_out, void* stream);
int idv_ctconv_c1_img_fwd(const void* x0_img, long long lo_off0_slots, int C0, const void* x1_img, long long lo_off1_slots,
                          int C1, const void* wfrag, const float* bias, const float* prelu_slope, float* out, int Fin, int B,
                          int Tp, int Jp, int t_valid_out, void* stream);

int idv_pw_gemm(const float* x, int K, const float* wfrag, const float* bias, const float* prelu_slope, float* out,
                int M, int B, int Tp, int Jp, int t_valid, int swap, int ldo, void* stream);

int idv_cbn_finalize(const double* stats, double count, const float* gamma_rr, const float* gamma_ri,
                     const float* gamma_ii, const float* beta_r, const float* beta_i, int C, int first_call,
                     float momentum, float* running_mean_r, float* running_mean_i, float* Vrr, float* Vri,
                     float* Vii, float* moments, float* fold, void* stream);
int idv_cbn_stats(const float* act, int C, int F, int B, int Tp, int Jp, int t_valid, double* stats, void* stream);
int idv_cbn_apply_prelu(float* act, const float* fold, const float* prelu_slope, int C, int F, int B, int Tp, int Jp,
                        int t_valid, void* stream);

int idv_stft_frames(const float* x, int B, int L, int n_fft, int win, int hop, int T, float* frames, int Tp, int Jp,
                    void* stream);
int idv_istft_ola(const float* frames, const float* env_inv, int B, int n_fft, int win, int hop, int T, int Tp,
                  int Jp, float* y, void* stream);

int idv_mask_apply(const float* mask, const float* X, int x_div, int JpX, float* pred, float* pred_c, int F, int B,
                   int T, int Tp, int Jp, void* stream);
int idv_datanorm(const float* X, const float* mean, const float* stdv, int F, int B, int T, int Tp, int Jp, float* out, void* stream);
int idv_datadenorm(const float* P, const float* mean, const float* stdv, int F, int B, int T, int Tp, int Jp, float* out,
                   float* out_c, void* stream);
int idv_datanorm_bwd(const float* dout, const float* stdv, int F, int B, int T, int Tp, int Jp, float* dX, void* stream);
int idv_datadenorm_bwd(const float* dout, const float* dout_c, const float* stdv, int F, int B, int T, int Tp, int Jp, float* dP,
                       void* stream);
int idv_outtype_estimate(const float* speech_c, const float* noise_c, const float* X, long long sb, long long sf, long long st,
                         long long sr, int mode, int ns, int B, int F, int T, int Tp, int Jp, float* out, float* out_c,
                         void* stream);
int idv_planar_to_complex(const float* act, float* out_c, int F, int B, int T, int Tp, int Jp, void* stream);

long long idv_clstm_work_floats(int H, int B, int T, int Jp);
int idv_lstm_pers_supported(int H, int B);
long long idv_lstm_pers_work_bytes(int H, int B);
int idv_lstm_rec_pers(const float* g, long long g_run_z, long long g_run_s, int ldg, const float* whh_frag, float* hout, int H,
                      int B, int T, void* work, void* kimg, long long kimg_lo_slots, int Tp, int Jp, float* gsave, float* csave,
                      void* stream);
int idv_lstm_proj1_bf16x3(const void* himg, long long lo_off_slots, const void* wfrag_bf16, const float* bias, float* G1, int H,
                          int B, int T, int Tp, int Jp, void* stream);
int idv_lstm_coop_f32_supported(int H, int B);
long long idv_lstm_coop_f32_work_bytes(int H, int B);
int idv_lstm_rec_coop_f32(const float* g, long long g_run_z, long long g_run_s, int ldg, const float* whh_frag, float* hout, int H,
                          int B, int T, void* work, float* gsave, float* csave, void* stream);
int idv_lstm_pers_f32_supported(int H, int B);
long long idv_lstm_pers_f32_work_bytes(int H, int B);
int idv_lstm_rec_pers_f32(const float* g, long long g_run_z, long long g_run_s, int ldg, const float* whh_frag, float* hout, int H,
                          int B, int T, void* work, float* gsave, float* csave, void* stream);
void idv_lstm_pers_set_profile(unsigned long long* prof_cycles);
long long idv_clstm_train_work_floats(int H, int B, int T, int Jp);
int idv_clstm_fwd(const float* x, int K, const float* wih0, const float* bih0, const float* whh0, const float* wih1,
                  const float* bih1, const float* whh1, int H, int B, int T, int Tp, int Jp, float* work, float* out,
                  int flags, const void* wih1_bf16, void* stream);

int idv_lstm_stack2_f32_supported(int H, int B);
long long idv_lstm_stack2_f32_work_bytes(int H, int B);
int idv_lstm_stack2_f32(const float* g, long long g_run_z, long long g_run_s, int ldg, const float* whh0, const float* wih1_hh,
                        const float* whh1, const float* bias1, float* h0, float* hout, int H, int B, int T, void* work,
                        float* gsave1, float* csave0, float* csave1, void* stream);
int idv_clstm_fwd2(const float* x, int K, const float* wih0, const float* bih0, const float* whh0, const float* wih1,
                   const float* bih1, const float* whh1, const float* wih1_hh, int H, int B, int T, int Tp, int Jp, float* work,
                   float* out, int flags, const void* wih1_bf16, void* stream);

long long idv_lstm_ih_bf16_bytes(int H, int K);
int idv_lstm_proj_bf16_supported(int H, int K);
int idv_pack_lstm_ih_bf16(const float* w_ih_re, const float* w_ih_im, int H, int K, void* wfrag, void* stream);
int idv_planar_to_kimage(const float* x, int nvalid, int nplanes, int J, int Jp, void* img, long long lo_off_elems, void* stream);
int idv_pw_bf16x3_rows(const void* ximg, long long lo_off_slots, int K, const void* wfrag_bf16, const float* bias, float* out_rows,
                       int M, int ldo, int B, int T, int Tp, int Jp, void* stream);
long long idv_pw_bf16_wfrag_bytes(int M, int K);
int idv_pack_pw_bf16(const float* w, int M, int K, void* wfrag, void* stream);
int idv_pw_bf16x3(const void* ximg, long long lo_off_slots, int K, const void* wfrag_bf16, const float* bias, float* out, int M,
                  int B, int Tp, int Jp, int t_valid, void* stream);
int idv_stft_frames_kimage(const float* x, int B, int L, int n_fft, int win, int hop, int T, void* img, long long lo_off_elems,
                           int Tp, int Jp, void* stream);
int idv_lstm_proj_bf16x3(const void* ximg, long long lo_off_slots, int K, const void* wfrag_bf16, const float* bias, float* G,
                         int H, int B, int T, int Tp, int Jp, void* stream);

int idv_reparam(const float* lat, int Hl, int off_miu, int off_ls, int off_dl, int zdim, const float* eps_r,
                const float* eps_i, int ns, int B, int T, int Tp, int Jp, float* z, int Jpz, void* stream);


int idv_sisnr(const float* source, int src_ld, int src_div, const float* est, int est_ld, int B, int L, double* work,
              float* out, void* stream);
int idv_sisdr(const float* ref, int ref_ld, const float* est, int est_ld, int B, int L, double* work, float* out, void* stream);
int idv_mean_over_samples(const float* x, int ns, int B, int L, float* out, void* stream);
int idv_recon_loss(const float* pred_c, const float* ori, long long sb, long long sf, long long st, long long sr,
                   int ori_div, int B, int F, int T, double* work, float* out, void* stream);
int idv_ckl(const float* q1, int H1, int Jp1, int o1_miu, int o1_ls, int o1_dl, const float* q2, int H2, int Jp2,
            int o2_miu, int o2_ls, int o2_dl, int zdim, float eps, int B, int T, int Tp, double* work, float* out,
            void* stream);
int idv_msd(const float* a, int Ca, int ca0, int JpA, const float* b, int Cb, int cb0, int JpB, int C, int F, int B, int Tp,
            int t_valid, double* work, float* out, void* stream);
long long idv_mi_work_floats(int B, int ns, int T, int zdim);
int idv_mi_fwd(const float* lat, int H, int Jp, int o_miu, int o_ls, int o_dl, const float* z, int Jpz, int zdim, int ns, int B,
               int T, int Tp, float eps, float* work, double* acc, float* out, void* stream);
int idv_mi_bwd(const float* lat, int H, int Jp, int o_miu, int o_ls, int o_dl, const float* z, int Jpz, int zdim, int ns, int B,
               int T, int Tp, float eps, const float* work, const float* gout, float* dlat, float* dz, void* stream);
int idv_miu_dist(const float* q1, int H1, int Jp1, int off1, const float* q2, int H2, int Jp2, int off2, int zdim,
                 int B, int T, int Tp, double* work, float* out, void* stream);


int idv_pack_cconv_adjoint(const float* w_re, const float* w_im, int Cout, int Cin_total, int Cin_used, int transposed,
                           float* wfrag, float* bias_out, void* stream);
int idv_pack_cconv_bf16_adjoint(const float* w_re, const float* w_im, int Cout, int Cin_total, int Cin_used, int transposed,
                                void* wfrag, void* stream);

long long idv_cconv_wgrad_work_floats(int Cs, int Cl, int B, int Tp);
int idv_cconv2d_bwd_weight(const float* x, int Cx, int ci_off, const float* dy, int Cout, int Cin_total, int transposed,
                           int tshift, int Fin, int B, int Tp, int Jp_x, int Jp_dy, float* work, long long work_floats,
                           float* dw_re, float* dw_im, void* stream);
long long idv_cconv_wgrad_bf16_work_floats(int Cs, int Cl, int B, int Tp);
int idv_cconv2d_bwd_weight_bf16x3(const float* x, int Cx, int ci_off, const float* dy, int Cout, int Cin_total, int transposed,
                                  int tshift, int Fin, int B, int Tp, int Jp_x, int Jp_dy, float* work, long long work_floats,
                                  float* dw_re, float* dw_im, void* stream);
int idv_cconv_wgrad_gauss_supported(int Cs, int Cl);
long long idv_cconv_wgrad_gauss_work_floats(int Cx, int Cout, int transposed, int Fin, int B, int Tp, int Jp_x, int Jp_dy);
int idv_cconv2d_bwd_weight_gauss(const float* x, int Cx, int ci_off, const float* dy, int Cout, int Cin_total, int transposed,
                                 int tshift, int Fin, int B, int Tp, int Jp_x, int Jp_dy, float* work, long long work_floats,
                                 float* dw_re, float* dw_im, void* stream);
int idv_cconv2d_bwd_bias(const double* stats_dy, int Cout, float* db_re, float* db_im, void* stream);

long long idv_pw_wgrad_work_floats(int M, int K, int J);
int idv_pw_bwd_weight(const float* dout, int M, int Jp_d, const float* x, int K, int Jp_x, int J, int shift, float* work,
                      long long work_floats, float* dw, int ldw, int rowmap, int H, int accumulate, void* stream);
int idv_pw_bwd_weight_bf16x3(const float* dout, int M, int Jp_d, const float* x, int K, int Jp_x, int J, int shift, float* work,
                             long long work_floats, float* dw, int ldw, int rowmap, int H, int accumulate, void* stream);
int idv_planar_rowsum(const float* x, int M, int Jp, int J, int accumulate, float* out, void* stream);

int idv_cbn_apply_prelu_to(const float* y, const float* fold, const float* prelu_slope, int C, int F, int B, int Tp, int Jp,
                           int t_valid, float* out, void* stream);
int idv_cbn_bwd_reduce(const float* dz, const float* y, const float* fold, const float* prelu_slope, int C, int F, int B,
                       int Tp, int Jp, int t_valid, double* sums, void* stream);
int idv_cbn_bwd_finalize(const double* sums, double count, const float* moments, const float* gamma_rr, const float* gamma_ri,
                         const float* gamma_ii, int C, float* coef, float* dgamma_rr, float* dgamma_ri, float* dgamma_ii,
                         float* dbeta_r, float* dbeta_i, float* dslope, float param_grad_scale, void* stream);
int idv_cbn_bwd_apply(const float* dz, const float* y, const float* fold, const float* coef, const float* prelu_slope, int C,
                      int F, int B, int Tp, int Jp, int t_valid, float* dy, void* stream);
int idv_cbn_apply_prelu_to_img(const float* y, const float* fold, const float* prelu_slope, int C, int F, int B, int Tp, int Jp,
                               int t_valid, float* out, void* img, long long lo_off_elems, void* stream);
int idv_cbn_bwd_apply_img(const float* dz, const float* y, const float* fold, const float* coef, const float* prelu_slope, int C,
                          int F, int B, int Tp, int Jp, int t_valid, float* dy, void* img, long long lo_off_elems, void* stream);

int idv_mask_apply_bwd(const float* mask, const float* X, int x_div, int JpX, const float* dpred, const float* dpred_c, int F,
                       int B, int T, int Tp, int Jp, float* dmask, float* dX, void* stream);
int idv_repeat_batch_bwd(const float* drep, int n, int rows, int B, int Tp, int Jp_rep, int Jp, float* dx, void* stream);
int idv_complex_to_planar(const float* in_c, float* act, int F, int B, int T, int Tp, int Jp, void* stream);
int idv_istft_ola_bwd(const float* dy, const float* env_inv, int B, int n_fft, int win, int hop, int T, int Tp, int Jp,
                      float* dframes, void* stream);
int idv_stft_frames_bwd(const float* dframes, int B, int L, int n_fft, int win, int hop, int T, int Tp, int Jp, float* dx,
                        void* stream);
int idv_reparam_bwd(const float* lat, int Hl, int off_miu, int off_ls, int off_dl, int zdim, const float* eps_r,
                    const float* eps_i, int ns, int B, int T, int Tp, int Jp, const float* dz, int Jpz, float* dlat, void* stream);

int idv_sisnr_bwd(const float* source, int src_ld, int src_div, const float* est, int est_ld, int B, int L, const double* work,
                  const float* grad_out, float* dest, void* stream);
int idv_recon_loss_bwd(const float* pred_c, const float* ori, long long sb, long long sf, long long st, long long sr,
                       int ori_div, int B, int F, int T, const float* g_cpx, const float* g_mag, float* dpred_c, void* stream);
int idv_ckl_bwd(const float* q1, int H1, int Jp1, int o1_miu, int o1_ls, int o1_dl, const float* q2, int H2, int Jp2,
                int o2_miu, int o2_ls, int o2_dl, int zdim, float eps, int B, int T, int Tp, const float* grad_out, float* dq1,
                void* stream);
int idv_miu_dist_bwd(const float* q1, int H1, int Jp1, int off1, const float* q2, int H2, int Jp2, int off2, int zdim, int B,
                     int T, int Tp, const float* grad_out, const float* loss_value, float* dq1, float* dq2, void* stream);

int idv_lstm_uncombine(const float* dout, int H, int B, int T, int Tp, int Jp, float* dh, void* stream);
int idv_pack_lstm_hh_bwd(const float* w_hh_re, const float* w_hh_im, int H, float* whhT, void* stream);
long long idv_lstm_bptt_work_floats(int H, int B);
int idv_lstm_bptt(float* gates, long long g_run_z, long long g_run_s, int ldg, const float* cstates, const float* dhout,
                  const float* whhT, int H, int B, int T, float* work, void* stream);
int idv_lstm_bptt_coop_supported(int H, int B);
int idv_lstm_bptt_stack2_supported(int H, int B);
long long idv_lstm_bptt_stack2_work_bytes(int H, int B);
int idv_lstm_bptt_stack2(float* g1, float* g0, long long g0_run_z, long long g0_run_s, int ldg0, const float* c1, const float* c0,
                         const float* dhout1, const float* whhT1, const float* wihT1, const float* whhT0, int H, int B, int T,
                         void* work, void* stream);
long long idv_lstm_bptt_coop_work_bytes(int H, int B);
int idv_lstm_bptt_coop(float* gates, long long g_run_z, long long g_run_s, int ldg, const float* cstates, const float* dhout,
                       const float* whhT, int H, int B, int T, void* work, void* stream);
int idv_rows_to_planar(const float* src, long long ld, int c0, int ncol, int B, int T, int Tp, int Jp, float* dst, void* stream);
int idv_lstm_bias_grad(const float* dGp, int H, int Jp, int J, int accumulate, float* db, void* stream);

int idv_bucket_gather(const long long* table, int n, long long total, float* flat, void* stream);
int idv_bucket_scatter(const long long* table, int n, long long total, const float* flat, float scale, void* stream);
int idv_bucket_adam(const long long* ptable, const long long* gtable, const float* gflat, float* exp_avg, float* exp_avg_sq,
                    int n, long long total, float lr, double beta1, double beta2, float eps, float weight_decay,
                    float bias_correction1, float bias_correction2_sqrt, float grad_scale, void* stream);

int idv_cconv_wino_supported(int transposed, int C0, int C1, int Cout, int Fin);
long long idv_cconv_wino_wfrag_floats(int transposed, int Cout, int cin_used);
int idv_cconv_wino_config(int transposed, int Cin, int Cout);
int idv_pack_cconv_wino(const float* w_re, const float* w_im, int Cout, int Cin_total, int Cin_used, int transposed, int conj,
                        float* wfrag, void* stream);
int idv_cconv2d_wino_fwd(const float* x0, int C0, const float* x1, int C1, const float* wfrag, const float* epi, int has_fold,
                         const float* prelu_slope, float* out, double* stats, double* stats_work, int stats_rep, int transposed,
                         int tshift, int Cout, int Fin, int B, int Tp, int Jp, int t_valid_out, const float* addend,
                         int addend_div, int addend_Jp, void* stream);

int idv_cconv_tw_supported(int C0, int C1, int Cout, int Fin);
long long idv_cconv_tw_wfrag_floats(int Cout, int cin_used);
int idv_pack_cconv_tw(const float* wino_frag, int Cout, int cin_used, float* tw_frag, void* stream);
int idv_ctconv2d_tw_fwd(const float* x0, int C0, const float* x1, int C1, const float* wfrag, const float* epi, int has_fold,
                        const float* prelu_slope, float* out, double* stats, double* stats_work, int stats_rep, int tshift,
                        int Cout, int Fin, int B, int Tp, int Jp, int t_valid_out, const float* addend, int addend_div,
                        int addend_Jp, void* stream);

int idv_cconv_tw2_supported(int Cin, int Cout, int Fin);
long long idv_cconv_tw2_wfrag_floats(int Cout, int cin_used);
int idv_pack_cconv_tw2(const float* wino_frag, int Cout, int cin_used, float* tw_frag, void* stream);
int idv_cconv2d_tw_fwd(const float* x0, int Cin, const float* wfrag, const float* epi, int has_fold, const float* prelu_slope,
                       float* out, double* stats, double* stats_work, int stats_rep, int tshift, int Cout, int Fin, int B, int Tp,
                       int Jp, int t_valid_out, void* stream);

long long idv_stream_cconv_wfloats(int Cin, int Cout);
int idv_stream_pack_cconv(const float* w_re, const float* w_im, const float* b_re, const float* b_im, int Cin, int Cout,
                          int transposed, float* w, float* bias, void* stream);
int idv_stream_cconv_splits(int transposed, int Cin, int Cout, int Fin, int B);
int idv_stream_cconv(const float* x0, const float* h0, int C0, const float* x1, const float* h1, int C1, const float* w,
                     const float* bias, const float* fold, const float* prelu_slope, float* out, float* hist_out, float* x0hist_out,
                     float* work, int nsplit, int transposed, int Cout, int Fin, int B, int k, int Tp, int Jp, void* stream);
int idv_stream_lstm_supported(int H);
int idv_stream_clstm(const float* G, const float* wt, const float* b1, float* state, float* hout, float* out, int H, int B, int k,
                     int Tp, int Jp, void* stream);
int idv_stream_frames(const float* ring, int R, const float* x, long long ldx, int n_new, long long n_prev, long long L_end, int B,
                      int n_fft, int win, int hop, long long t0, int k, float* frames, int Tp, int Jp, void* stream);
int idv_stream_ring(float* ring, int R, const float* x, long long ldx, int n_new, long long n_prev, int B, void* stream);
int idv_stream_ola(const float* frames, int Tp, int Jp, const float* carry_in, int carry_in_len, float* carry_out, int cap, int B,
                   int n_fft, int win, int hop, long long t0, int k, long long T_total, long long e0, long long e1, long long p_end,
                   float* y, int ldy, long long y_off, void* stream);

int idv_stft_frames_ragged(const float* x, long long ldx, const int* lens, int B, int n_fft, int win, int hop, int Tmax, float* frames,
                           int Tp, int Jp, void* stream);
int idv_stft_frames_kimage_ragged(const float* x, long long ldx, const int* lens, int B, int n_fft, int win, int hop, int Tmax, void* img,
                                  long long lo_off_elems, int Tp, int Jp, void* stream);
int idv_istft_ola_ragged(const float* frames, const int* lens, int len_div, int B, int n_fft, int win, int hop, int Tmax, int Tp, int Jp,
                         float* y, long long ldy, void* stream);
int idv_sisdr_ragged(const float* ref, int ref_ld, const float* est, int est_ld, const int* lens, int B, double* work, float* out,
                     void* stream);

#ifdef __cplusplus
}
#endif
#endif
```

Measured before the change: 907.4 utterances/sec.

## Pair two output-channel tiles per 512-thread workgroup in Winograd conv kernels

Adds an NCT=2 variant of the tw/tw2 complex conv kernels in which one 512-thread workgroup computes two adjacent Cout tiles, so the staged input patch in LDS is shared by both and the grid shrinks by half. Waves 4..7 can be staggered by one k-step when staging, to spread LDS and global traffic, and each co tile gets its own epilogue exchange area. This cuts the redundant patch loading and staging done per co tile, at the cost of occupancy dropping to one workgroup per CU and a larger LDS footprint. It also caches hipFuncSetAttribute calls for the winograd launcher and adds a runtime mask and launch counter to control pairing.

Result: faster. 957.6 utterances/sec, median of 6 (+5.5%).

```diff
diff --git a/i-dccrn-vae_amd/csrc/cgemm_tw.hip b/i-dccrn-vae_amd/csrc/cgemm_tw.hip
--- a/i-dccrn-vae_amd/csrc/cgemm_tw.hip
+++ b/i-dccrn-vae_amd/csrc/cgemm_tw.hip
@@ -1,5 +1,7 @@
+#include <atomic>
 #include <cstdint>
 #include <cstdlib>
+#include <type_traits>
 #include "cgemm.hpp"
 #include "../../include/idccrn_hip.h"
 
@@ -25,6 +27,8 @@
     int add_div, add_Jp;
     int jtiles, ftiles;
     int xcd_split;
+    int cgroups;
+    int stagger;
 };
 
 constexpr int TW_PACK_CI = 8;
@@ -52,8 +56,8 @@
 }
 template <int PH> constexpr int tw_wslots() { return PH == 0 ? 9 : 8; }
 
-template <int PH, int CIK, bool LEFT, int DBG = 0, int RDW = 2, bool WVEC = true, bool STATS = false>
-__global__ __launch_bounds__(256, 2) void cconv_tw_kernel(const TwArgs a) {
+template <int PH, int CIK, bool LEFT, int DBG = 0, int RDW = 2, bool WVEC = true, bool STATS = false, int NCT = 1>
+__global__ __launch_bounds__(256 * NCT, NCT == 1 ? 2 : 1) void cconv_tw_kernel(const TwArgs a) {
     constexpr int NR = tw_nr<PH>(), NT = tw_nt<PH>(), NTP = tw_ntp<PH>(), NTW = tw_ntw<PH>();
     constexpr int NRAW = PH == 0 ? 4 : 3, ROW0 = PH == 0 ? 0 : 1;
     constexpr int KS = CIK / 2;
@@ -61,33 +65,38 @@
     constexpr int NE = CIK * RT;
     constexpr int NBUF = 2;
     constexpr int NITEM = CIK * NRAW * 16;
-    constexpr int NLD = (NITEM + 255) / 256;
+    constexpr int NTHR = 256 * NCT;
+    constexpr int NLD = (NITEM + NTHR - 1) / NTHR;
+    static_assert(NCT == 1 || NCT == 2, "one or two co tiles per workgroup");
     static_assert(KS % RDW == 0 && NLD <= 2, "weight ring slots are compile-time; at most two staging items per thread");
-    static_assert(NT * 4 * 64 <= NBUF * NE, "the epilogue exchange fits the patch buffers");
+    static_assert(NLD + NCT - 1 < KS, "the staging k-steps (from 1 on, waves 4 .. 7 one later) end before the barrier's k-step");
+    static_assert(NCT * NT * 4 * 64 <= NBUF * NE, "the epilogue exchange (one area per co tile) fits the patch buffers");
 
     extern __shared__ __attribute__((aligned(16))) float smem[];
 
     const int tid = threadIdx.x;
     const int lane = tid & 63;
     const int wave = __builtin_amdgcn_readfirstlane(tid >> 6);
+    const int w4 = NCT == 1 ? wave : wave & 3, cth = NCT == 1 ? 0 : wave >> 2;
     const int half = lane >> 5, l31 = lane & 31;
 
     const int bid = blockIdx.x;
     const int xcd = bid & 7, slot = bid >> 3;
     int jt, ft, ct;
     if (a.xcd_split) {
-        const int G = 8 / a.cotiles;
-        ct = xcd % a.cotiles;
-        jt = (slot / a.ftiles) * G + xcd / a.cotiles;
+        const int G = 8 / a.cgroups;
+        ct = xcd % a.cgroups;
+        jt = (slot / a.ftiles) * G + xcd / a.cgroups;
         ft = slot - (slot / a.ftiles) * a.ftiles;
     } else {
-        const int per = a.cotiles * a.ftiles;
+        const int per = a.cgroups * a.ftiles;
         jt = (slot / per) * 8 + xcd;
         const int rem = slot - (slot / per) * per;
-        ft = rem / a.cotiles;
-        ct = rem - ft * a.cotiles;
+        ft = rem / a.cgroups;
+        ct = rem - ft * a.cgroups;
     }
     if (jt >= a.jtiles) return;
+    ct = NCT * ct + cth;
     const int j0 = jt * 64;
     const int m0 = 2 * ft;
     const int rbase = m0 - 1 + ROW0;
@@ -105,13 +114,13 @@
     int offA[UNI ? 1 : NPAIR + 1], offB[UNI ? 1 : NPAIR + 1];
     float cbj[UNI ? 1 : NPAIR + 1];
     if (UNI) {
-        cbj[0] = tw_cb<PH>(wave);
-        offA[0] = (tw_ra<PH>(wave) - ROW0) * 288;
-        offB[0] = (tw_rb<PH>(wave) - ROW0) * 288;
+        cbj[0] = tw_cb<PH>(w4);
+        offA[0] = (tw_ra<PH>(w4) - ROW0) * 288;
+        offB[0] = (tw_rb<PH>(w4) - ROW0) * 288;
     } else {
 #pragma unroll
         for (int j = 0; j <= NPAIR; ++j) {
-            int t = tw_tile(PH, wave, j < NPAIR ? 2 * j : NTW - 1);
+            int t = tw_tile(PH, w4, j < NPAIR ? 2 * j : NTW - 1);
             t = t < 0 ? 0 : t;
             const int r = t / 9, plane = t - r * 9;
             cbj[j] = tw_cb<PH>(r);
@@ -129,7 +138,7 @@
     bool interior[NLD];
 #pragma unroll
     for (int i = 0; i < NLD; ++i) {
-        const int e = tid + i * 256;
+        const int e = tid + i * NTHR;
         const int c8 = e & 15;
         const int rl = (e >> 4) % NRAW, cl = e / (16 * NRAW);
         item_cl[i] = cl;
@@ -201,7 +210,7 @@
         const float xd_ = g == 0 ? fr[q0 + 2] + fi[q0 + 2] : (g == 1 ? fr[q0 + 2] : fi[q0 + 2]);
         return tau == 0 ? xa_ - xb_ : (tau == 1 ? xb_ : xb_ - xd_);
     };
-    auto item_exists = [&](int i) -> bool { return NITEM >= (i + 1) * 256 || wave * 64 + i * 256 < NITEM; };
+    auto item_exists = [&](int i) -> bool { return NITEM >= (i + 1) * NTHR || wave * 64 + i * NTHR < NITEM; };
     auto stage_plane2 = [&](float* dst, int i, int j) {
         if (!item_exists(i)) return;
         if (j < 4) {
@@ -219,7 +228,7 @@
 
     constexpr int WS = tw_wslots<PH>();
     const float* wbase = a.wfrag + ((size_t)(PH == 1 ? (size_t)a.cotiles * a.UP * tw_ntp<0>() : 0) + (size_t)ct * a.UP * NTP) * 64 +
-                         (size_t)wave * WS * 64;
+                         (size_t)w4 * WS * 64;
     const int total_ks = nchunk * KS;
     float a_w[RDW][NTW];
     auto load_w = [&](int g, float (&dst)[NTW]) {
@@ -266,42 +275,49 @@
     __syncthreads();
 
     load_raw_all(smem + (size_t)half * RT);
-    for (int chunk = 0; chunk < nchunk; ++chunk) {
-        const float* P = smem + (chunk & 1) * NE;
-        float* Pn = smem + ((chunk + 1) & 1) * NE;
-        const int nxt = chunk + 1 < nchunk ? chunk + 1 : chunk, nxt2 = chunk + 2 < nchunk ? chunk + 2 : nchunk - 1;
-#pragma unroll
-        for (int ul = 0; ul < KS; ++ul) {
-            const float* bnext = ul + 1 < KS ? P + (size_t)(2 * (ul + 1) + half) * RT : Pn + (size_t)half * RT;
-            const int si = ul - 1;
-            const bool staging = !(DBG & 1) && si >= 0 && si < NLD;
-#pragma unroll
-            for (int k = 0; k < NTW; ++k) {
-                const float b = xa[k] + cbj[UNI ? 0 : (k >> 1 < NPAIR ? k >> 1 : NPAIR)] * xb[k];
-                acc[k] = __builtin_amdgcn_mfma_f32_32x32x2f32(a_w[ul % RDW][k], b, acc[k], 0, 0, 0);
-                if (ul == KS - 1 && k == 0) {
+    auto run = [&](auto late_) {
+        constexpr bool LATE = decltype(late_)::value;
+        for (int chunk = 0; chunk < nchunk; ++chunk) {
+            const float* P = smem + (chunk & 1) * NE;
+            float* Pn = smem + ((chunk + 1) & 1) * NE;
+            const int nxt = chunk + 1 < nchunk ? chunk + 1 : chunk, nxt2 = chunk + 2 < nchunk ? chunk + 2 : nchunk - 1;
+#pragma unroll
+            for (int ul = 0; ul < KS; ++ul) {
+                const float* bnext = ul + 1 < KS ? P + (size_t)(2 * (ul + 1) + half) * RT : Pn + (size_t)half * RT;
+                const int si = ul - 1 - (LATE ? 1 : 0);
+                const bool staging = !(DBG & 1) && si >= 0 && si < NLD;
+#pragma unroll
+                for (int k = 0; k < NTW; ++k) {
+                    const float b = xa[k] + cbj[UNI ? 0 : (k >> 1 < NPAIR ? k >> 1 : NPAIR)] * xb[k];
+                    acc[k] = __builtin_amdgcn_mfma_f32_32x32x2f32(a_w[ul % RDW][k], b, acc[k], 0, 0, 0);
+                    if (ul == KS - 1 && k == 0) {
+                        __builtin_amdgcn_sched_barrier(0);
+                        __syncthreads();
+                    }
+                    if ((k & 1) && (k >> 1) < NPAIR) load_raw2(bnext, k >> 1);
+                    if (k == NTW - 1) load_raw2(bnext, NPAIR);
+                    if (staging) {
+                        if (k == 0) stage_window(nxt, si);
+                        if ((k & 1) && k < 6) stage_plane2(Pn, si, k >> 1);
+                        if (k == (NTW == 9 ? 7 : 6)) stage_plane2(Pn, si, 3);
+                        if (k == NTW - 1) stage_plane2(Pn, si, 4);
+                        if (k == NTW - 1) stage_load(nxt2, si);
+                    }
                     __builtin_amdgcn_sched_barrier(0);
-                    __syncthreads();
                 }
-                if ((k & 1) && (k >> 1) < NPAIR) load_raw2(bnext, k >> 1);
-                if (k == NTW - 1) load_raw2(bnext, NPAIR);
-                if (staging) {
-                    if (k == 0) stage_window(nxt, si);
-                    if ((k & 1) && k < 6) stage_plane2(Pn, si, k >> 1);
-                    if (k == (NTW == 9 ? 7 : 6)) stage_plane2(Pn, si, 3);
-                    if (k == NTW - 1) stage_plane2(Pn, si, 4);
-                    if (k == NTW - 1) stage_load(nxt2, si);
-                }
-                __builtin_amdgcn_sched_barrier(0);
-            }
-            if (!(DBG & 2)) load_w(chunk * KS + ul + RDW, a_w[ul % RDW]);
-        }
-    }
+                if (!(DBG & 2)) load_w(chunk * KS + ul + RDW, a_w[ul % RDW]);
+            }
+        }
+    };
+    if (NCT == 2 && PH == 1 && a.stagger && cth)
+        run(std::integral_constant<bool, NCT == 2 && PH == 1>{});
+    else
+        run(std::false_type{});
     __syncthreads();
 
     const float slope = a.slope ? *a.slope : 1.0f;
     const bool has_act = a.slope != nullptr;
-    float* E = smem;
+    float* E = smem + cth * (NT * 4 * 64);
     const int jA = j0 + 2 * l31;
     bool keep[2], inb[2];
     int ja[2];
@@ -318,7 +334,7 @@
         if (s > 0) __syncthreads();
 #pragma unroll
         for (int k = 0; k < NTW; ++k) {
-            const int t = tw_tile(PH, wave, k);
+            const int t = tw_tile(PH, w4, k);
             if (t >= 0) {
 #pragma unroll
                 for (int rr = 0; rr < 4; ++rr) E[(t * 4 + rr) * 64 + lane] = acc[k][4 * s + rr];
@@ -327,7 +343,7 @@
         __syncthreads();
         float v[NT];
 #pragma unroll
-        for (int t = 0; t < NT; ++t) v[t] = E[(t * 4 + wave) * 64 + lane];
+        for (int t = 0; t < NT; ++t) v[t] = E[(t * 4 + w4) * 64 + lane];
         float pr[NR][2], pi[NR][2];
 #pragma unroll
         for (int r = 0; r < NR; ++r) {
@@ -344,7 +360,7 @@
                 pi[r][q] = y[0][q] + y[1][q];
             }
         }
-        const int rg = 4 * s + wave;
+        const int rg = 4 * s + w4;
         const int co = ct * 32 + (rg & 3) + 8 * (rg >> 2) + 4 * half;
         const bool cok = co < a.Cout;
         const f32x4 e0 = *(const f32x4*)(a.epi + (size_t)co * 8);
@@ -445,7 +461,7 @@
     }
 }
 
-template <int PH, int CIK, bool LEFT, int DBG, int RDW, bool WVEC = true, bool STATS = false>
+template <int PH, int CIK, bool LEFT, int DBG, int RDW, bool WVEC = true, bool STATS = false, int NCT = 1>
 int launch_tw_ph_l(const TwArgs& a, hipStream_t st);
 inline int tw_wvec_mask() {
     static const int v = [] { const char* e = getenv("IDV_TW_WVEC"); return e ? atoi(e) : 1; }();
@@ -454,6 +470,11 @@
 template <int PH, int CIK, int DBG = 0, int RDW = 2>
 int launch_tw_ph(const TwArgs& a, hipStream_t st) {
     const bool wv = (tw_wvec_mask() >> PH) & 1;
+    if (DBG == 0 && RDW == 2 && wv == (PH == 0) && a.cotiles % 2 == 0 && ((idv_tw_pair(-1) >> PH) & 1)) {
+        constexpr bool WV = PH == 0;
+        if (a.stats) return a.tshift ? launch_tw_ph_l<PH, CIK, true, 0, 2, WV, true, 2>(a, st) : launch_tw_ph_l<PH, CIK, false, 0, 2, WV, true, 2>(a, st);
+        return a.tshift ? launch_tw_ph_l<PH, CIK, true, 0, 2, WV, false, 2>(a, st) : launch_tw_ph_l<PH, CIK, false, 0, 2, WV, false, 2>(a, st);
+    }
     if (DBG == 0 && RDW == 2 && a.stats) {
         constexpr bool WV = PH == 0;
         if (wv != WV) return IDV_EINVAL;
@@ -463,35 +484,56 @@
         return a.tshift ? launch_tw_ph_l<PH, CIK, true, 0, 2, false>(a, st) : launch_tw_ph_l<PH, CIK, false, 0, 2, false>(a, st);
     return a.tshift ? launch_tw_ph_l<PH, CIK, true, DBG, RDW>(a, st) : launch_tw_ph_l<PH, CIK, false, DBG, RDW>(a, st);
 }
-template <int PH, int CIK, bool LEFT, int DBG, int RDW, bool WVEC, bool STATS>
+template <int PH, int CIK, bool LEFT, int DBG, int RDW, bool WVEC, bool STATS, int NCT>
 int launch_tw_ph_l(const TwArgs& a, hipStream_t st) {
     constexpr int NE = CIK * (PH == 0 ? 4 : 3) * 9 * 32;
     constexpr size_t smem = 2 * NE * sizeof(float);
-    static_assert(smem * 2 <= 160 * 1024, "the patch buffers of two workgroups must fit the 160 KB of LDS");
+    static_assert(smem * (NCT == 1 ? 2 : 1) <= 160 * 1024, "the patch buffers of two workgroups (NCT = 2: of one) must fit the 160 KB of LDS");
     TwArgs b = a;
     b.jtiles = (a.J + 63) / 64;
     b.ftiles = PH == 1 ? a.Fin / 2 : (a.Fin + 1) / 2;
     if (b.ftiles == 0) return IDV_OK;
     static const int xsplit = [] { const char* e = getenv("IDV_TW_XCD_SPLIT"); return e ? atoi(e) : 1; }();
-    b.xcd_split = (xsplit && (b.cotiles == 2 || b.cotiles == 4 || b.cotiles == 8)) ? 1 : 0;
-    long long nblk = (long long)((b.jtiles + 7) / 8) * 8 * b.ftiles * b.cotiles;
+    b.cgroups = b.cotiles / NCT;
+    if (b.cgroups * NCT != b.cotiles) return IDV_EINVAL;
+    static const int stag = [] { const char* e = getenv("IDV_TW_PAIR_STAGGER"); return e ? atoi(e) : 1; }();
+    b.stagger = stag;
+    b.xcd_split = (xsplit && (b.cgroups == 2 || b.cgroups == 4 || b.cgroups == 8)) ? 1 : 0;
+    long long nblk = (long long)((b.jtiles + 7) / 8) * 8 * b.ftiles * b.cgroups;
     if (b.xcd_split) {
-        const int G = 8 / b.cotiles;
+        const int G = 8 / b.cgroups;
         nblk = (long long)((b.jtiles + G - 1) / G) * b.ftiles * 8;
     }
     if (nblk > 0x7fffffffLL) return IDV_EINVAL;
-    auto k = cconv_tw_kernel<PH, CIK, LEFT, DBG, RDW, WVEC, STATS>;
-    static bool attr_set[64] = {};
+    auto k = cconv_tw_kernel<PH, CIK, LEFT, DBG, RDW, WVEC, STATS, NCT>;
+    static std::atomic<bool> attr_set[64];
     int dev = 0;
     if (hipGetDevice(&dev) != hipSuccess || dev < 0 || dev >= 64) return IDV_ELAUNCH;
-    if (smem > 64 * 1024 && !attr_set[dev]) {
+    if (smem > 64 * 1024 && !attr_set[dev].load(std::memory_order_acquire)) {
         if (hipFuncSetAttribute((const void*)k, hipFuncAttributeMaxDynamicSharedMemorySize, (int)smem) != hipSuccess) return IDV_ELAUNCH;
-        attr_set[dev] = true;
-    }
-    hipLaunchKernelGGL(k, dim3((unsigned)nblk), dim3(256), smem, st, b);
+        attr_set[dev].store(true, std::memory_order_release);
+    }
+    hipLaunchKernelGGL(k, dim3((unsigned)nblk), dim3(256 * NCT), smem, st, b);
+    if (NCT > 1) idv_tw_pair_note_launch();
     return idv_launch_status();
 }
 
+}
+
+namespace {
+std::atomic<int>& tw_pair_mask() {
+    static std::atomic<int> v{[] { const char* e = getenv("IDV_TW_PAIR"); return e ? atoi(e) & IDV_TW_PAIR_ALL : IDV_TW_PAIR_DEFAULT; }()};
+    return v;
+}
+std::atomic<long long> tw_pair_launches{0};
+}
+void idv_tw_pair_note_launch() { tw_pair_launches.fetch_add(1, std::memory_order_relaxed); }
+extern "C" int idv_tw_pair(int mask) {
+    if (mask < 0) return tw_pair_mask().load(std::memory_order_relaxed);
+    return tw_pair_mask().exchange(mask & IDV_TW_PAIR_ALL, std::memory_order_relaxed);
+}
+extern "C" long long idv_tw_pair_launches(int reset) {
+    return reset ? tw_pair_launches.exchange(0, std::memory_order_relaxed) : tw_pair_launches.load(std::memory_order_relaxed);
 }
 
 extern "C" int idv_cconv_tw_supported(int C0, int C1, int Cout, int Fin) {
diff --git a/i-dccrn-vae_amd/csrc/cgemm_tw2.hip b/i-dccrn-vae_amd/csrc/cgemm_tw2.hip
--- a/i-dccrn-vae_amd/csrc/cgemm_tw2.hip
+++ b/i-dccrn-vae_amd/csrc/cgemm_tw2.hip
@@ -1,3 +1,4 @@
+#include <atomic>
 #include <cstdint>
 #include <cstdlib>
 #include <type_traits>
@@ -23,6 +24,8 @@
     int stats_rep;
     int jtiles, ftiles;
     int xcd_split;
+    int cgroups;
+    int stagger;
 };
 
 constexpr int TW2_PACK_CI = 8;
@@ -50,39 +53,48 @@
 
 __device__ __forceinline__ int tw2_poff(int p, int l31) { return p < 8 ? (p >> 1) * 64 + 2 * l31 + (p & 1) : 256 + l31; }
 
-template <bool LEFT, bool STATS, int DBG = 0>
-__global__ __launch_bounds__(256, 2) void cconv_tw2_kernel(const Tw2Args a) {
+constexpr int tw2_smem_floats(int nct) {
+    return nct == 1 ? 2 * 4 * 7 * 288 : (2 * (4 * 7 * 288 + 288) > 2 * 36 * 4 * 64 ? 2 * (4 * 7 * 288 + 288) : 2 * 36 * 4 * 64);
+}
+template <bool LEFT, bool STATS, int DBG = 0, int NCT = 1>
+__global__ __launch_bounds__(256 * NCT, NCT == 1 ? 2 : 1) void cconv_tw2_kernel(const Tw2Args a) {
     constexpr int NT = 36, NACC = 9, NSLOT = 16;
     constexpr int NRAW = 7, CIK = 4, KS = 2;
     constexpr int RT = NRAW * 288;
     constexpr int NE = CIK * RT;
+    constexpr int NEB = NCT == 1 ? NE : NE + 288;
     constexpr int NITEM = CIK * NRAW * 16;
-    constexpr int NLD = 2;
-    static_assert(NT * 4 * 64 <= 2 * NE, "the epilogue exchange fits the patch buffers");
+    constexpr int NTHR = 256 * NCT;
+    constexpr int NLD = (NITEM + NTHR - 1) / NTHR;
+    static_assert(NCT == 1 || NCT == 2, "one or two co tiles per workgroup");
+    static_assert(2 * NEB <= tw2_smem_floats(NCT) && NCT * NT * 4 * 64 <= tw2_smem_floats(NCT),
+                  "the patch buffers and the epilogue exchange (one area per co tile) fit the allocation");
 
     extern __shared__ __attribute__((aligned(16))) float smem[];
 
     const int tid = threadIdx.x;
     const int lane = tid & 63;
     const int wave = __builtin_amdgcn_readfirstlane(tid >> 6);
+    const int w4 = NCT == 1 ? wave : wave & 3, cth = NCT == 1 ? 0 : wave >> 2;
     const int half = lane >> 5, l31 = lane & 31;
 
     const int bid = blockIdx.x;
     const int xcd = bid & 7, slot = bid >> 3;
     int jt, ft, ct;
     if (a.xcd_split) {
-        const int G = 8 / a.cotiles;
-        ct = xcd % a.cotiles;
-        jt = (slot / a.ftiles) * G + xcd / a.cotiles;
+        const int G = 8 / a.cgroups;
+        ct = xcd % a.cgroups;
+        jt = (slot / a.ftiles) * G + xcd / a.cgroups;
         ft = slot - (slot / a.ftiles) * a.ftiles;
     } else {
-        const int per = a.cotiles * a.ftiles;
+        const int per = a.cgroups * a.ftiles;
         jt = (slot / per) * 8 + xcd;
         const int rem = slot - (slot / per) * per;
-        ft = rem / a.cotiles;
-        ct = rem - ft * a.cotiles;
+        ft = rem / a.cgroups;
+        ct = rem - ft * a.cgroups;
     }
     if (jt >= a.jtiles) return;
+    ct = NCT * ct + cth;
     const int j0 = jt * 64;
     const int m0 = 2 * ft;
     const int rbase = 2 * m0 - 2;
@@ -101,12 +113,12 @@
     unsigned off_v[NLD], ldsoff[NLD];
     unsigned okmask[NLD];
     bool interior[NLD];
-    auto item_cl = [&](int i) -> int { return (tid + i * 256) / (16 * NRAW); };
+    auto item_cl = [&](int i) -> int { return (tid + i * NTHR) / (16 * NRAW); };
 #pragma unroll
     for (int i = 0; i < NLD; ++i) {
-        const int e = tid + i * 256;
+        const int e = tid + i * NTHR;
         const int c8 = e & 15;
-        const int rl = (e >> 4) % NRAW, cl = e / (16 * NRAW);
+        const int cl = e / (16 * NRAW), rl = (NCT == 2 && e >= NITEM) ? 0 : (e >> 4) % NRAW;
         const int f = rbase + rl;
         const int jc = j0 + 4 * c8;
         const int je = LEFT ? jc - 1 : jc + 4;
@@ -187,7 +199,7 @@
         for (int j = 0; j < 5; ++j) stage_plane2(dst, i, j);
     };
 
-    const float* wbase = a.wfrag + (((size_t)ct * a.UP) * 4 + wave) * 1024 + lane * 4;
+    const float* wbase = a.wfrag + (((size_t)ct * a.UP) * 4 + w4) * 1024 + lane * 4;
     const int total_ks = nchunk * KS;
     float a_w[NSLOT];
     auto load_wg = [&](int g, int grp) {
@@ -197,11 +209,11 @@
         for (int k = 0; k < 4; ++k) a_w[grp * 4 + k] = w4[k];
     };
 
-    const int am = tw2_main_acc(wave < 3 ? wave : 0);
+    const int am = tw2_main_acc(w4 < 3 ? w4 : 0);
     const int qxm = tw2_qx(am), qym = tw2_qy(am);
     const int rxa = tw2_ra(qxm) * 288, rxb = tw2_rb(qxm) * 288, rya = tw2_ra(qym) * 288, ryb = tw2_rb(qym) * 288;
     const float cbx = tw2_cb(qxm), cby = tw2_cb(qym);
-    const int r2a = tw2_ra(2) * 288 + wave * 64, r2b = tw2_rb(2) * 288 + wave * 64;
+    const int r2a = tw2_ra(2) * 288 + w4 * 64, r2b = tw2_rb(2) * 288 + w4 * 64;
     float xa[2][4], xb[2][4];
     auto load_grp_a = [&](const float* base, int g, float (&oa)[4], float (&ob)[4]) {
         if (g < 3) {
@@ -236,16 +248,16 @@
 #pragma unroll
     for (int i = 0; i < NLD; ++i) stage_load(nchunk > 1 ? 1 : 0, i);
     __syncthreads();
-    if (wave < 3)
+    if (w4 < 3)
         load_grp_a(smem + (size_t)half * RT, 0, xa[0], xb[0]);
     else
         load_grp_b(smem + (size_t)half * RT, 0, xa[0], xb[0]);
 
-    auto run = [&](auto role) {
+    auto run = [&](auto role, auto late_) {
         constexpr bool ROLE_B = decltype(role)::value;
         for (int chunk = 0; chunk < nchunk; ++chunk) {
-            const float* P = smem + (chunk & 1) * NE;
-            float* Pn = smem + ((chunk + 1) & 1) * NE;
+            const float* P = smem + (chunk & 1) * NEB;
+            float* Pn = smem + ((chunk + 1) & 1) * NEB;
             const int nxt = chunk + 1 < nchunk ? chunk + 1 : chunk, nxt2 = chunk + 2 < nchunk ? chunk + 2 : nchunk - 1;
 #pragma unroll
             for (int ul = 0; ul < KS; ++ul) {
@@ -283,7 +295,20 @@
                         else load_grp_a(bnext, 0, xa[0], xb[0]);
                     }
                     if (((k & 3) == 3 || (ROLE_B && k == NSLOT - 2)) && !(DBG & 2)) load_wg(chunk * KS + ul + 1, k >> 2);
-                    if (staging) {
+                    if constexpr (NCT == 2) if (staging) {
+                        constexpr bool late = decltype(late_)::value;
+                        if (k <= 5 && !late) {
+                            if (k == 0) stage_window(nxt, 0);
+                            if (k >= 1) stage_plane2(Pn, 0, k - 1);
+                            if (k == 5) stage_load(nxt2, 0);
+                        }
+                        if (k >= 8 && k <= 13 && late) {
+                            if (k == 8) stage_window(nxt, 0);
+                            if (k >= 9) stage_plane2(Pn, 0, k - 9);
+                            if (k == 13) stage_load(nxt2, 0);
+                        }
+                    }
+                    if constexpr (NCT == 1) if (staging) {
                         if (k == 0) stage_window(nxt, 0);
                         if (k >= 1 && k <= 5) stage_plane2(Pn, 0, k - 1);
                         if (k == 5) stage_load(nxt2, 0);
@@ -298,15 +323,20 @@
             }
         }
     };
-    if (wave < 3)
-        run(std::false_type{});
+    if (NCT == 2 && a.stagger && cth) {
+        if (w4 < 3)
+            run(std::false_type{}, std::integral_constant<bool, NCT == 2>{});
+        else
+            run(std::true_type{}, std::integral_constant<bool, NCT == 2>{});
+    } else if (w4 < 3)
+        run(std::false_type{}, std::false_type{});
     else
-        run(std::true_type{});
+        run(std::true_type{}, std::false_type{});
     __syncthreads();
 
     const float slope = a.slope ? *a.slope : 1.0f;
     const bool has_act = a.slope != nullptr;
-    float* E = smem;
+    float* E = smem + cth * (NT * 4 * 64);
     const int jA = j0 + 2 * l31;
     bool keep[2], inb[2];
 #pragma unroll
@@ -321,14 +351,14 @@
         if (s > 0) __syncthreads();
 #pragma unroll
         for (int k = 0; k < NACC; ++k) {
-            const int t = tw2_acc_tile(wave, k);
+            const int t = tw2_acc_tile(w4, k);
 #pragma unroll
             for (int rr = 0; rr < 4; ++rr) E[(t * 4 + rr) * 64 + lane] = acc[k][4 * s + rr];
         }
         __syncthreads();
         float v[NT];
 #pragma unroll
-        for (int t = 0; t < NT; ++t) v[t] = E[(t * 4 + wave) * 64 + lane];
+        for (int t = 0; t < NT; ++t) v[t] = E[(t * 4 + w4) * 64 + lane];
         float pr[4][2], pi[4][2];
 #pragma unroll
         for (int r = 0; r < 4; ++r) {
@@ -345,7 +375,7 @@
                 pi[r][q] = y[0][q] + y[1][q];
             }
         }
-        const int rg = 4 * s + wave;
+        const int rg = 4 * s + w4;
         const int co = ct * 32 + (rg & 3) + 8 * (rg >> 2) + 4 * half;
         const bool cok = co < a.Cout;
         const f32x4 e0 = *(const f32x4*)(a.epi + (size_t)co * 8);
@@ -427,30 +457,35 @@
     }
 }
 
-template <bool LEFT, bool STATS, int DBG>
+template <bool LEFT, bool STATS, int DBG, int NCT = 1>
 int launch_tw2(const Tw2Args& a, hipStream_t st) {
-    constexpr size_t smem = 2 * 4 * 7 * 288 * sizeof(float);
-    static_assert(smem * 2 <= 160 * 1024, "the patch buffers of two workgroups must fit the 160 KB of LDS");
+    constexpr size_t smem = tw2_smem_floats(NCT) * sizeof(float);
+    static_assert(smem * (NCT == 1 ? 2 : 1) <= 160 * 1024, "the patch buffers of two workgroups (NCT = 2: of one) must fit the 160 KB of LDS");
     Tw2Args b = a;
     b.jtiles = (a.J + 63) / 64;
     b.ftiles = (a.Fout + 1) / 2;
     static const int xsplit = [] { const char* e = getenv("IDV_TW_XCD_SPLIT"); return e ? atoi(e) : 1; }();
-    b.xcd_split = (xsplit && (b.cotiles == 2 || b.cotiles == 4 || b.cotiles == 8)) ? 1 : 0;
-    long long nblk = (long long)((b.jtiles + 7) / 8) * 8 * b.ftiles * b.cotiles;
+    b.cgroups = b.cotiles / NCT;
+    if (b.cgroups * NCT != b.cotiles) return IDV_EINVAL;
+    static const int stag = [] { const char* e = getenv("IDV_TW_PAIR_STAGGER"); return e ? atoi(e) : 1; }();
+    b.stagger = stag;
+    b.xcd_split = (xsplit && (b.cgroups == 2 || b.cgroups == 4 || b.cgroups == 8)) ? 1 : 0;
+    long long nblk = (long long)((b.jtiles + 7) / 8) * 8 * b.ftiles * b.cgroups;
     if (b.xcd_split) {
-        const int G = 8 / b.cotiles;
+        const int G = 8 / b.cgroups;
         nblk = (long long)((b.jtiles + G - 1) / G) * b.ftiles * 8;
     }
     if (nblk > 0x7fffffffLL) return IDV_EINVAL;
-    auto k = cconv_tw2_kernel<LEFT, STATS, DBG>;
-    static bool attr_set[64] = {};
+    auto k = cconv_tw2_kernel<LEFT, STATS, DBG, NCT>;
+    static std::atomic<bool> attr_set[64];
     int dev = 0;
     if (hipGetDevice(&dev) != hipSuccess || dev < 0 || dev >= 64) return IDV_ELAUNCH;
-    if (smem > 64 * 1024 && !attr_set[dev]) {
+    if (smem > 64 * 1024 && !attr_set[dev].load(std::memory_order_acquire)) {
         if (hipFuncSetAttribute((const void*)k, hipFuncAttributeMaxDynamicSharedMemorySize, (int)smem) != hipSuccess) return IDV_ELAUNCH;
-        attr_set[dev] = true;
-    }
-    hipLaunchKernelGGL(k, dim3((unsigned)nblk), dim3(256), smem, st, b);
+        attr_set[dev].store(true, std::memory_order_release);
+    }
+    hipLaunchKernelGGL(k, dim3((unsigned)nblk), dim3(256 * NCT), smem, st, b);
+    if (NCT > 1) idv_tw_pair_note_launch();
     return idv_launch_status();
 }
 
@@ -507,8 +542,13 @@
     if (!stats && dbg == 2) return tshift ? launch_tw2<true, false, 2>(a, st) : launch_tw2<false, false, 2>(a, st);
     if (!stats && dbg == 3) return tshift ? launch_tw2<true, false, 3>(a, st) : launch_tw2<false, false, 3>(a, st);
 #endif
-    if (stats)
+    const bool pair = a.cotiles % 2 == 0 && (idv_tw_pair(-1) & IDV_TW_PAIR_CONV);
+    if (stats && pair)
+        rc = tshift ? launch_tw2<true, true, 0, 2>(a, st) : launch_tw2<false, true, 0, 2>(a, st);
+    else if (stats)
         rc = tshift ? launch_tw2<true, true, 0>(a, st) : launch_tw2<false, true, 0>(a, st);
+    else if (pair)
+        rc = tshift ? launch_tw2<true, false, 0, 2>(a, st) : launch_tw2<false, false, 0, 2>(a, st);
     else
         rc = tshift ? launch_tw2<true, false, 0>(a, st) : launch_tw2<false, false, 0>(a, st);
     if (rc || !(stats && stats_work)) return rc;
diff --git a/i-dccrn-vae_amd/csrc/cgemm_wino.hip b/i-dccrn-vae_amd/csrc/cgemm_wino.hip
--- a/i-dccrn-vae_amd/csrc/cgemm_wino.hip
+++ b/i-dccrn-vae_amd/csrc/cgemm_wino.hip
@@ -1,3 +1,4 @@
+#include <atomic>
 #include <cstdlib>
 #include "cgemm.hpp"
 #include "../../include/idccrn_hip.h"
@@ -398,8 +399,13 @@
     if (nblk > 0x7fffffffLL) return IDV_EINVAL;
     auto k = cconv_wino_kernel<PH, WM, WN, CIK, NBUF, STATS, OCC, RD>;
     const size_t smem_req = OCC == 1 ? (smem > 84 * 1024 ? smem : 84 * 1024) : smem;
-    if (smem_req > 64 * 1024 &&
-        hipFuncSetAttribute((const void*)k, hipFuncAttributeMaxDynamicSharedMemorySize, (int)smem_req) != hipSuccess) return IDV_ELAUNCH;
+    static std::atomic<bool> attr_set[64];
+    int dev = 0;
+    if (hipGetDevice(&dev) != hipSuccess || dev < 0 || dev >= 64) return IDV_ELAUNCH;
+    if (smem_req > 64 * 1024 && !attr_set[dev].load(std::memory_order_acquire)) {
+        if (hipFuncSetAttribute((const void*)k, hipFuncAttributeMaxDynamicSharedMemorySize, (int)smem_req) != hipSuccess) return IDV_ELAUNCH;
+        attr_set[dev].store(true, std::memory_order_release);
+    }
     hipLaunchKernelGGL(k, dim3((unsigned)nblk), dim3(WM * WN * 64), smem_req, st, b);
     return idv_launch_status();
 }
diff --git a/i-dccrn-vae_amd/csrc/common.hpp b/i-dccrn-vae_amd/csrc/common.hpp
--- a/i-dccrn-vae_amd/csrc/common.hpp
+++ b/i-dccrn-vae_amd/csrc/common.hpp
@@ -35,3 +35,4 @@
 }
 
 int idv_launch_stats_collapse(const double* work, int rep, int n, double* stats, hipStream_t st);
+void idv_tw_pair_note_launch();
diff --git a/i-dccrn-vae_amd/ops.py b/i-dccrn-vae_amd/ops.py
--- a/i-dccrn-vae_amd/ops.py
+++ b/i-dccrn-vae_amd/ops.py
@@ -247,6 +247,23 @@
 TW = os.environ.get("IDV_TW", "1") != "0"
 TW_CONV = os.environ.get("IDV_TW_CONV", "1") != "0"
 TW_CFG = 5000000
+TW_PAIR = None
+_tw_pair_lib = None
+_tw_pair_pushed = None
+
+
+def _sync_tw_pair():
+    global _tw_pair_lib, _tw_pair_pushed
+    if TW_PAIR == _tw_pair_pushed:
+        return
+    if _tw_pair_lib is None:
+        _tw_pair_lib = int(L.lib().idv_tw_pair(-1))
+    L.lib().idv_tw_pair(_tw_pair_lib if TW_PAIR is None else int(TW_PAIR))
+    _tw_pair_pushed = TW_PAIR
+
+
+def tw_pair_launches(reset: bool = False) -> int:
+    return int(L.lib().idv_tw_pair_launches(1 if reset else 0))
 
 
 def _pack_wino_tw(w_re, w_im, cout: int, cin_total: int, cin_used: int, transposed: bool, conj: int):
@@ -489,6 +506,7 @@
         if LAUNCH_LOG is not None:
             cfg = TW_CFG + (1 if tshift else 0)
         swork = _stats_work(stats, cout)
+        _sync_tw_pair()
         call("idv_ctconv2d_tw_fwd", x.ptr(), i(x.C), skip.ptr() if skip is not None else p(None), i(c1), p(gauss[4]), p(gauss[1]),
              i(gauss[2]), p(slope), out.ptr(), p(stats), p(swork), i(STATS_REP), i(tshift), i(cout), i(x.F), i(x.B), i(x.Tp), i(x.Jp),
              i(t_out), addend.ptr() if addend is not None else p(None), i(addend_div), i(addend.Jp if addend is not None else 0),
@@ -497,6 +515,7 @@
         if LAUNCH_LOG is not None:
             cfg = TW_CFG + 2 + (1 if tshift else 0)
         swork = _stats_work(stats, cout)
+        _sync_tw_pair()
         call("idv_cconv2d_tw_fwd", x.ptr(), i(x.C), p(gauss[4]), p(gauss[1]), i(gauss[2]), p(slope), out.ptr(), p(stats), p(swork),
              i(STATS_REP), i(tshift), i(cout), i(x.F), i(x.B), i(x.Tp), i(x.Jp), i(t_out), stream_ptr())
     elif skip_div == 1 and _wino_ok(gauss, transposed, x, c1, cout, skip.Jp if skip is not None else None):
@@ -1003,11 +1022,13 @@
     if wfrag_bf16 is None and adj_transposed and _tw_ok(gauss, dy, 0, cout_adj, None):
         if LAUNCH_LOG is not None:
             cfg = TW_CFG + (1 if tshift_adj else 0)
+        _sync_tw_pair()
         call("idv_ctconv2d_tw_fwd", dy.ptr(), i(dy.C), p(None), i(0), p(gauss[4]), p(gauss[1]), i(0), p(None), out.ptr(), p(None), p(None),
              i(0), i(tshift_adj), i(cout_adj), i(dy.F), i(dy.B), i(dy.Tp), i(dy.Jp), i(t_out), p(None), i(1), i(0), stream_ptr())
     elif wfrag_bf16 is None and not adj_transposed and _tw2_ok(gauss, dy, 0, cout_adj):
         if LAUNCH_LOG is not None:
             cfg = TW_CFG + 2 + (1 if tshift_adj else 0)
+        _sync_tw_pair()
         call("idv_cconv2d_tw_fwd", dy.ptr(), i(dy.C), p(gauss[4]), p(gauss[1]), i(0), p(None), out.ptr(), p(None), p(None), i(0),
              i(tshift_adj), i(cout_adj), i(dy.F), i(dy.B), i(dy.Tp), i(dy.Jp), i(t_out), stream_ptr())
     elif wfrag_bf16 is None and _wino_ok(gauss, adj_transposed, dy, 0, cout_adj, None):
diff --git a/include/idccrn_hip.h b/include/idccrn_hip.h
--- a/include/idccrn_hip.h
+++ b/include/idccrn_hip.h
@@ -320,6 +320,14 @@
 int idv_sisdr_ragged(const float* ref, int ref_ld, const float* est, int est_ld, const int* lens, int B, double* work, float* out,
                      void* stream);
 
+#define IDV_TW_PAIR_T_EVEN 1
+#define IDV_TW_PAIR_T_ODD 2
+#define IDV_TW_PAIR_CONV 4
+#define IDV_TW_PAIR_ALL 7
+#define IDV_TW_PAIR_DEFAULT 7
+int idv_tw_pair(int mask);
+long long idv_tw_pair_launches(int reset);
+
 #ifdef __cplusplus
 }
 #endif
```
